# jaswon/osu-dreamer

Measured on AMD Instinct MI355X. Metric: denoiser train-steps/sec + 50-step sample latents/sec, 1/2/4/8 MI355X, higher is better.
Workload: dtype bf16

## Files before the change

### include/osu_dreamer_hip.h

```cpp
#ifndef OSU_DREAMER_HIP_H
#define OSU_DREAMER_HIP_H

#ifdef __cplusplus
extern "C" {
#endif

enum { OD_F32 = 0, OD_BF16 = 1,
       OD_F32X3 = 2,
       OD_F32X3W = 3,
       OD_F16 = 4 };
enum { OD_EPI_NONE = 0, OD_EPI_SILU = 1 };
enum { OD_ACT_NONE = 0, OD_ACT_SILU = 1 };
enum { OD_ERR_ARG = -1, OD_ERR_ALIGN = -2, OD_ERR_UNSUPPORTED = -3, OD_ERR_COMM = -4 };

int od_version(void);
const char* od_build_source_sha(void);
const char* od_error_string(int code);

int od_gemm_nt(int dtype, const void* A, int lda, const void* W, int ldw, const float* bias, void* C, int ldc,
               int M, int N, int K, int epilogue, int accumulate, void* stream);
int od_gemm_nt_qkrope(int dtype, const void* A, int lda, const void* W, int ldw, const float* bias, void* C, int ldc, int M,
                      int N, int K, const float* wq, const float* wk, const float* table, int L, int H, int hd, float eps,
                      float q_scale, void* stream);
int od_gemm_nt_qkrope_split(int dtype, const void* A, int lda, const void* W, int ldw, const float* bias, void* C, int ldc,
                            void* qk_out, int ldqk, int qk_dtype, int M, int N, int K, const float* wq, const float* wk, const float* table,
                            int L, int H, int hd, float eps, float q_scale, void* stream);
int od_gemm_tn(int dtype, const void* G, int ldg, const void* A, int lda, float* dW, int lddw, float* dbias, int M, int N,
               int K, void* stream);
int od_gemm_tn_blocks(int dtype, const void* G, int ldg, const void* A, int lda, float* dW, int lddw, float* dbias, int M, int N,
                      int K, int n_block, int n_valid, void* stream);
int od_colsum(int dtype, const void* G, int ldg, float* out, int M, int N, void* stream);
int od_pack_weight(int dtype, const float* src, int N, int K, void* dst, int Np, int Kp, int transpose,
                   const int* row_map, void* stream);

int od_linear_small(const float* x, const float* W, const float* b, float* out, float* pre, int B, int N, int K, int act,
                    void* stream);
int od_linear_small_bwd(const float* x, const float* W, const float* pre, const float* dout, float* dpre, float* dW,
                        float* db, float* dx, int accumulate_dx, int B, int N, int K, int act, void* stream);

int od_cl_to_frames(int dtype, const float* src, void* dst, int ldd, int B, int C, int L, void* stream);
int od_feed_gather(const float* store, long store_elems, const long* base, const long* cstride, const int* lens, float* out,
                   int N, int C, int Lpad, void* stream);
int od_feed_gather_quant(const void* store, long store_bytes, int elem_size, const long* base, const long* cstride, const int* lens,
                         const double* scale, const double* offset, const int* flip, float* out, int N, int C, int c0, int Ctot,
                         int Lpad, void* stream);
int od_replicate_tail(float* x, const int* lens, const int* plens, int N, int C, int Lpad, void* stream);
int od_proj_in(int dtype, const float* xt, const float* W, const float* bias, void* x, int ldx, int B, int E, int L,
               int D, void* stream);
int od_proj_in_bwd(int dtype, const float* xt, const void* dx, int ldx, float* dW, float* db, int B, int E, int L, int D,
                   void* stream);
int od_silu(int dtype, const void* x, void* y, long n, void* stream);
int od_silu_bwd(int dtype, const void* x, const void* dy, void* dx, long n, void* stream);

int od_rmsnorm_film(int dtype, const void* x, int ldx, const float* ssg, const void* cl, int ldcl, int cl_bcast,
                    void* h, int ldh, float* inv_rms, int B, int L, int C, float eps, void* stream);
int od_rmsnorm_film_bwd(int dtype, const void* x, int ldx, const float* inv_rms, const float* ssg, const void* dh,
                        int lddh, void* dres, int lddres, float* dssg, int B, int L, int C, void* stream);
int od_rmsnorm_gate_residual(int dtype, const void* x, int ldx, const void* h, int ldh, const float* ssg, void* xo,
                             int ldxo, float* inv_rms, int B, int L, int C, float eps, void* stream);
int od_rmsnorm_gate_residual_film(int dtype, const void* x, int ldx, const void* h, int ldh, const float* ssg_a, void* xo, int ldxo,
                                  float* inv_a, const float* ssg_b, const void* cl, int ldcl, int cl_bcast, void* h2, int ldh2,
                                  float* inv_b, int B, int L, int C, float eps, void* stream);
int od_rmsnorm_gate_residual_film_dwconv(int dtype, const void* x, int ldx, const void* h, int ldh, const float* ssg_a, void* xo, int ldxo,
                                         float* inv_a, const float* ssg_b, void* h2, int ldh2, float* inv_b, const float* conv_w,
                                         const float* conv_b, void* y, int ldy, int B, int L, int C, int ksize, float eps, void* stream);
int od_rmsnorm_gate_residual_bwd(int dtype, const void* h, int ldh, const float* inv_rms, const float* ssg,
                                 const void* dy, int lddy, void* dh, int lddh, float* dssg, int B, int L, int C,
                                 void* stream);

int od_rope_table(float* table, int L, int hd, void* stream);
int od_qk_norm_rope(int dtype, const void* qkv, int ldqkv, const float* wq, const float* wk, const float* table,
                    void* qk_out, int ldo, int B, int L, int H, int hd, float eps, float q_scale, void* stream);
int od_qk_norm_rope_bwd(int dtype, const void* qkv, int ldqkv, const float* wq, const float* wk, const float* table,
                        const void* dqk, int lddqk, void* dqkv, int lddqkv, float* dwq, float* dwk, int B, int L,
                        int H, int hd, float eps, float q_scale, void* stream);
int od_flash_attn_fwd(int dtype, const void* q, int ldq, const void* k, int ldk, const void* v, int ldv, void* o, int ldo,
                      float* lse, int B, int H, int L, int hd, float scale, int q_prescaled, void* stream);
int od_flash_attn_fwd_varlen(int dtype, const void* q, int ldq, const void* k, int ldk, const void* v, int ldv, void* o, int ldo,
                             float* lse, const int* lens, int B, int H, int L, int hd, float scale, int q_prescaled, void* stream);
int od_flash_attn_bwd(int dtype, const void* q, int ldq, const void* k, int ldk, const void* v, int ldv, const void* o,
                      int ldo, const void* dout, int lddo, const float* lse, float* delta, void* dq, int lddq, void* dk,
                      int lddk, void* dv, int lddv, int B, int H, int L, int hd, float scale, int q_prescaled, void* stream);
int od_attn_aux_create(void** aux_out);
int od_attn_aux_destroy(void* aux);
int od_flash_attn_bwd_aux(int dtype, const void* q, int ldq, const void* k, int ldk, const void* v, int ldv, const void* o,
                          int ldo, const void* dout, int lddo, const float* lse, float* delta, void* dq, int lddq, void* dk,
                          int lddk, void* dv, int lddv, int B, int H, int L, int hd, float scale, int q_prescaled, void* aux, void* stream);
int od_flash_attn_bwd_varlen(int dtype, const void* q, int ldq, const void* k, int ldk, const void* v, int ldv, const void* o,
                             int ldo, const void* dout, int lddo, const float* lse, float* delta, void* dq, int lddq, void* dk,
                             int lddk, void* dv, int lddv, const int* lens, int B, int H, int L, int hd, float scale, int q_prescaled,
                             void* aux, void* stream);
int od_flash_attn_bwd_fused_ws_bytes(int dtype, int B, int H, int L, long* total_out, long* zero_out);
int od_flash_attn_bwd_fused(int dtype, const void* q, int ldq, const void* k, int ldk, const void* v, int ldv, const void* o, int ldo,
                            const void* dout, int lddo, const float* lse, void* dq, int lddq, void* dk, int lddk, void* dv, int lddv,
                            int B, int H, int L, int hd, float scale, int q_prescaled, void* ws, long ws_bytes, void* stream);
int od_flash_attn_bwd_fused_status(const void* ws, int* err_out, void* stream);
int od_flash_attn_bwd_fused_err_offset(void);
int od_flash_attn_bwd_fused_passes(void);
int od_flash_attn_bwd_fused_prof(void* ws, long* out16);
int od_flash_attn_bwd_passes(void);

int od_dwconv(int dtype, const void* x, int ldx, const float* w, const float* bias, void* y, int ldy, int B, int L,
              int C, int ksize, void* stream);
int od_dwconv_varlen(int dtype, const void* x, int ldx, const float* w, const float* bias, void* y, int ldy, const int* lens,
                     int B, int L, int C, int ksize, void* stream);
int od_dwconv_bwd(int dtype, const void* x, int ldx, const float* w, const void* dy, int lddy, void* dx, int lddx,
                  float* dw, float* db, int B, int L, int C, int ksize, void* stream);
int od_dwconv_bwd_varlen(int dtype, const void* x, int ldx, const float* w, const void* dy, int lddy, void* dx, int lddx,
                         float* dw, float* db, const int* lens, int B, int L, int C, int ksize, void* stream);
int od_scale_channels(int dtype, void* x, int ldx, const float* scale, int B, int L, int C, void* stream);
int od_swiglu_rmsnorm(int dtype, const void* vg, int ldvg, void* hh, int ldhh, float* inv_rms, int M, int Hf, int Hp,
                      float eps, void* stream);
int od_swiglu_rmsnorm_bwd(int dtype, const void* vg, int ldvg, const float* inv_rms, const void* dhh, int lddhh,
                          void* dvg, int lddvg, int M, int Hf, int Hp, void* stream);

int od_final_norm_proj_out(int dtype, const void* x, int ldx, const float* W, const float* bias, float* v,
                           float* inv_rms, int B, int L, int C, int E, float eps, void* stream);
int od_final_norm_proj_out_bwd(int dtype, const void* x, int ldx, const float* inv_rms, const float* W, const float* dv,
                               void* dx, int lddx, float* dW, float* db, int B, int L, int C, int E, void* stream);
int od_uhead_fwd(const float* xt, const float* w0, const float* b0, const float* w1, const float* b1, const float* w3,
                 const float* b3, const float* w4, const float* b4, float* fsum, int B, int E, int L, int U,
                 void* stream);
int od_uhead_fwd_varlen(const float* xt, const float* w0, const float* b0, const float* w1, const float* b1, const float* w3,
                        const float* b3, const float* w4, const float* b4, float* fsum, const int* lens, int B, int E, int L,
                        int U, void* stream);
int od_uhead_bwd(const float* xt, const float* w0, const float* b0, const float* w1, const float* b1, const float* w3,
                 const float* b3, const float* w4, const float* b4, const float* dfm, float* dw0, float* db0, float* dw1,
                 float* db1, float* dw3, float* db3, float* dw4, float* db4, int B, int E, int L, int U, void* stream);
int od_uhead_bwd_varlen(const float* xt, const float* w0, const float* b0, const float* w1, const float* b1, const float* w3,
                        const float* b3, const float* w4, const float* b4, const float* dfm, float* dw0, float* db0, float* dw1,
                        float* db1, float* dw3, float* db3, float* dw4, float* db4, const int* lens, int B, int E, int L, int U,
                        void* stream);
int od_uhead_tail(const float* fsum, const float* mod, const float* w_out, const float* b_out, float* u, int B, int U,
                  int L, float u_scale, void* stream);
int od_uhead_tail_varlen(const float* fsum, const float* mod, const float* w_out, const float* b_out, float* u, const int* lens,
                         int B, int U, int L, float u_scale, void* stream);
int od_uhead_tail_bwd(const float* fsum, const float* mod, const float* w_out, const float* b_out, const float* du,
                      float* dfm, float* dmod, float* dw_out, float* db_out, int B, int U, int L, float u_scale,
                      void* stream);
int od_uhead_tail_bwd_varlen(const float* fsum, const float* mod, const float* w_out, const float* b_out, const float* du,
                             float* dfm, float* dmod, float* dw_out, float* db_out, const int* lens, int B, int U, int L,
                             float u_scale, void* stream);

int od_make_xt(const float* x0, const float* x1, const float* t, float* xt, float* dsq, int B, int E, int L, void* stream);
int od_make_xt_varlen(const float* x0, const float* x1, const float* t, float* xt, float* dsq, const int* lens, int B, int E, int L,
                      void* stream);
int od_loss_grad(const float* xt, const float* x1, const float* u, const float* v, const float* dsq, float* dv,
                 float* sums, int B, int E, int L, float c0, float osl_w, float del_w, void* stream);
int od_loss_grad_varlen(const float* xt, const float* x1, const float* u, const float* v, const float* dsq, float* dv,
                        float* sums, const int* lens, int B, int E, int L, float c0, float osl_w, float del_w, void* stream);
int od_loss_finalize(const float* sums, const float* dsq, const float* u, float* out, float* du, int B, float c0,
                     float osl_w, float del_w, void* stream);
int od_sampler_step(float* x, const float* u, const float* v, const float* eta, int B, int E, int L, void* stream);
int od_sampler_eta(const float* u, float* eta, int B, float c0, int num_steps, void* stream);
int od_sampler_eta_groups(const float* u, const int* offs, float* eta, int G, float c0, int num_steps, void* stream);
int od_sampler_step_varlen(float* x, const float* u, const float* v, const float* eta, const int* lens, const int* offs, int G,
                           int B, int E, int L, void* stream);

int od_det_clear(void);
int od_det_register(const float* base, long count, void* shadow_i64);
int od_det_enable(void* table_dev, void* stream);
int od_det_table_bytes(void);
int od_det_flush(float* dst, long count, void* stream);

int od_sqnorm(const float* g, long n, float* out, const int* status, void* stream);
int od_adamw_ema(float* p, const float* g, float* m, float* v, float* ema, long n, float lr, float beta1, float beta2,
                 float eps, float weight_decay, int step, float ema_decay, int ema_mode, const float* gnorm_sq,
                 float max_norm, const int* status, void* stream);

int od_ema_update(float* ema, const float* p, long n, float ema_decay, int ema_mode, void* stream);

int od_style_conditioning(const float* labels, const float* rff_w, const float* rff_b, const float* cond_w,
                          const float* cond_b, const float* null_labels, float* c, int B, int NL, int F, int H,
                          void* stream);
int od_rmsnorm_rows(const float* x, const float* gamma, float* y, int M, int C, float eps, void* stream);

int od_style_conditioning_bwd(const float* labels, const float* rff_w, const float* rff_b, const float* dc, float* dcond_w,
                              float* dcond_b, float* dnull_labels, int B, int NL, int F, int H, void* stream);
int od_rmsnorm_rows_bwd(const float* x, const float* gamma, const float* dy, float* dx, float* dgamma, int M, int C, float eps,
                        int accumulate_dx, void* stream);
int od_cast_rows(int src_dtype, const void* src, int dst_dtype, void* dst, long n, void* stream);

int od_spec_features_conv(int dtype, const float* audio, const float* w1, const float* b1, const float* g1, const float* w2,
                          const float* b2, const float* g2, void* out, int ldo, int B, int F, int L, float eps, void* stream);
int od_rmsnorm_affine_film(int dtype, const void* x, int ldx, const float* gamma, const float* ssg, void* y, int ldy, int B,
                           int L, int C, float eps, int act, void* stream);
int od_rmsnorm_affine_gate_residual(int dtype, const void* x, int ldx, const void* h, int ldh, const float* gamma,
                                    const float* ssg, void* xo, int ldxo, int B, int L, int C, float eps, void* stream);
int od_unet_mixer(int dtype, const void* x, int ldx, const void* p, int ldp, int p_bcast, const void* gx, int ldg,
                  const float* gamma, void* xo, int ldxo, int B, int L, int C, float eps, void* stream);
int od_unet_down(int dtype, const void* x, int ldx, const float* w, const float* bias, void* y, int ldy, int B, int Lo, int C,
                 int stride, void* stream);
int od_unet_up(int dtype, const void* x, int ldx, const float* w, const float* bias, void* y, int ldy, int B, int Li, int C,
               int stride, void* stream);
int od_chart_head(int dtype, const void* x, int ldx, const float* W, const float* bias, float* out, int B, int L, int C, int N,
                  int n_sigmoid, int rms, float eps, void* stream);
int od_attn_pool(int dtype, const void* scores, int lds, const void* values, int ldv, float* out, int B, int L, int Hh, int hd,
                 void* stream);
int od_latent_bwd_block_frames(int C);
int od_rmsnorm_affine_film_bwd(int dtype, const void* x, int ldx, const float* gamma, const float* ssg, const void* dy, int lddy, void* dx,
                               int lddx, int accumulate_dx, float* dgamma, float* dssg, float* ws, long ws_floats, int B, int L, int C,
                               float eps, int act, void* stream);
int od_rmsnorm_affine_gate_residual_bwd(int dtype, const void* h, int ldh, const float* gamma, const float* ssg, const void* dxo, int lddxo,
                                        void* dh, int lddh, float* dgamma, float* dssg, float* ws, long ws_floats, int B, int L, int C,
                                        float eps, void* stream);
int od_unet_mixer_bwd(int dtype, const void* p, int ldp, int p_bcast, const void* gx, int ldg, const float* gamma, const void* dxo,
                      int lddxo, void* dp, int lddp, void* dgx, int lddg, float* dgamma, float* ws, long ws_floats, int B, int L, int C,
                      float eps, void* stream);
int od_unet_down_bwd(int dtype, const void* x, int ldx, const float* w, const void* dy, int lddy, void* dx, int lddx, float* dw, float* db,
                     float* ws, long ws_floats, int B, int Lo, int C, int stride, void* stream);
int od_unet_up_bwd(int dtype, const void* x, int ldx, const float* w, const void* dy, int lddy, void* dx, int lddx, float* dw, float* db,
                   float* ws, long ws_floats, int B, int Li, int C, int stride, void* stream);
int od_chart_head_bwd(int dtype, const void* x, int ldx, const float* W, const float* bias, const float* dout, void* dx, int lddx,
                      float* dW, float* db, float* ws, long ws_floats, int B, int L, int C, int N, int rms, float eps, void* stream);
int od_attn_pool_bwd(int dtype, const void* scores, int lds, const void* values, int ldv, const float* dout, void* dscores, int ldds,
                     void* dvalues, int lddv, int B, int L, int Hh, int hd, void* stream);
int od_spec_features_conv_bwd(int dtype, const float* audio, const float* w1, const float* b1, const float* g1, const float* w2,
                              const float* b2, const float* g2, const void* dout, int ldo, float* dw1, float* db1, float* dg1, float* dw2,
                              float* db2, float* dg2, float* ws, long ws_floats, int B, int F, int L, float eps, void* stream);
int od_add_rows(int dtype, const void* x, void* y, long n, void* stream);
int od_proj_in_bwd_input(int dtype, const void* dx, int ldx, const float* W, float* dxt, int B, int E, int L, int D, void* stream);

int od_mmd_imq(const float* z, const float* prior, float* out, float* dz, float* ws, long ws_floats, int N, int D, void* stream);
int od_scale_by(const float* x, const float* g, float* y, long n, void* stream);
int od_latent_perturb(const float* z, long zsb, long zse, long zsl, const float* s, const float* eps_z, const float* eps_s,
                      const float* u_s, const float* repl, const float* u_span, const float* u_start, float* z_out, float* s_out,
                      void* masked, void* start_span, int B2, int E, int l, int S, float s_noise, float z_noise, float s_mask_frac,
                      float z_mask_frac, int training, void* stream);
int od_latent_perturb_bwd(const float* dz_out, const float* ds_out, const void* masked, const int* start_span, float* dz, float* ds,
                          int B2, int E, int l, int S, void* stream);
int od_latent_loss_block_frames(void);
int od_latent_loss_ws_floats(int B2, int L);
int od_latent_loss(const float* logits, const float* chart, const float* pred_labels, const float* true_labels, const void* masked,
                   const float* s_reg, float* loss_ema, void* ema_init, float* out, float* coef, float* ws, long ws_floats, int B2, int L,
                   float s_reg_weight, int training, void* stream);
int od_latent_loss_bwd(const float* logits, const float* chart, const float* pred_labels, const float* true_labels, const void* masked,
                       const float* coef, const float* g, float* dlogits, float* dlabels, float* ds_reg, int B2, int L,
                       float s_reg_weight, void* stream);

int od_mmd_imq_pairs(const float* s, const float* prior, float* out, float* ws, long ws_floats, int G, int S, void* stream);
int od_latent_loss_maps(const float* logits, const float* chart, const int* hlens, const float* pred_labels, const float* true_labels,
                        const float* s_reg, int s_reg_stride, const float* loss_ema, float* out, float* ws, long ws_floats, int G,
                        int Hmax, float s_reg_weight, void* stream);
int od_latent_eval_maps_ws_floats(int G, int Pmax);
int od_latent_eval_maps(const float* chart, const float* pred_chart, const int* plens, const float* z, const int* zlens,
                        const float* pred_labels, const float* true_labels, float* out, float* ws, long ws_floats, int G, int Pmax, int E,
                        int lmax, void* stream);

int od_spec_features_conv_varlen(int dtype, const float* audio, const float* w1, const float* b1, const float* g1, const float* w2,
                                 const float* b2, const float* g2, void* out, int ldo, const int* lens, int B, int F, int L, float eps,
                                 void* stream);
int od_rmsnorm_affine_film_varlen(int dtype, const void* x, int ldx, const float* gamma, const float* ssg, void* y, int ldy,
                                  const int* lens, int B, int L, int C, float eps, int act, void* stream);
int od_unet_mixer_varlen(int dtype, const void* x, int ldx, const void* p, int ldp, const int* prow, const void* gx, int ldg,
                         const float* gamma, void* xo, int ldxo, int B, int L, int C, float eps, void* stream);
int od_unet_down_varlen(int dtype, const void* x, int ldx, const float* w, const float* bias, void* y, int ldy, const int* lens,
                        int B, int Lo, int C, int stride, void* stream);
int od_unet_up_varlen(int dtype, const void* x, int ldx, const float* w, const float* bias, void* y, int ldy, const int* lens,
                      int B, int Li, int C, int stride, void* stream);
int od_chart_head_varlen(int dtype, const void* x, int ldx, const float* W, const float* bias, float* out, const int* lens, int B,
                         int L, int C, int N, int n_sigmoid, int rms, float eps, void* stream);
int od_attn_pool_varlen(int dtype, const void* scores, int lds, const void* values, int ldv, float* out, const int* lens, int B,
                        int L, int Hh, int hd, void* stream);

int od_comm_load(const char* path);
int od_comm_version(void);
int od_comm_unique_id(void* out, int nbytes);
int od_comm_init(void** comm_out, int nranks, int rank, const void* unique_id, int nbytes);
int od_comm_destroy(void* comm);
int od_comm_abort(void* comm);
int od_comm_count(void* comm);
int od_comm_ring_standin(float* buf, long count, int channels, int threads, int rounds, void* stream);
int od_allreduce_grads(void* comm, float* grads, long count, int average, void* stream);
int od_broadcast_f32(void* comm, float* buf, long count, int root, void* stream);

int od_graph_begin(void* stream);
int od_graph_end(void* stream, void** graph_exec_out);
int od_graph_launch(void* graph_exec, void* stream);
int od_graph_destroy(void* graph_exec);

int od_mfma_calibrate(float* scratch, int iters, double* flops_out, void* stream);

#ifdef __cplusplus
}
#endif
#endif
```

### osu_dreamer_amd/csrc/heads.hip

```cpp
#include "od_common.h"
#include "od_api_internal.h"

namespace {

constexpr int UW = 32;
constexpr int UOWN = 30;
constexpr int UWPB = 4;
constexpr int MAXU = 64, MAXE = 8;

__device__ __forceinline__ float red32(float v) {
#pragma unroll
    for (int m = 16; m >= 1; m >>= 1) v += __shfl_xor(v, m);
    return v;
}

struct UHeadW {
    const float *w0, *b0, *w1, *b1, *w3, *b3, *w4, *b4;
};

struct UHeadSmem {
    float xts[MAXE][UW + 4];
    float z0s[MAXE][UW + 2];
    float z1s[MAXU][UW + 2];
    float a1s[MAXU][UW + 2];
    float z3s[MAXU][UW + 1];
    float g4s[MAXU][UW + 1];
    float w4s[MAXU][MAXU + 1];
};

__device__ __forceinline__ void uhead_window_fwd(UHeadSmem& S, const float* __restrict__ xt, const UHeadW& P, int b, int l0,
                                                 int E, int L, int U, int Lv) {
    const int t = threadIdx.x;
    for (int idx = t; idx < E * (UW + 4); idx += 256) {
        const int e = idx / (UW + 4), ix = idx % (UW + 4);
        const int f = l0 - 3 + ix;
        S.xts[e][ix] = (f >= 0 && f < Lv) ? xt[((size_t)b * E + e) * L + f] : 0.f;
    }
    __syncthreads();
    for (int idx = t; idx < E * (UW + 2); idx += 256) {
        const int e = idx / (UW + 2), i2 = idx % (UW + 2);
        S.z0s[e][i2] = P.b0[e] + P.w0[e * 3 + 0] * S.xts[e][i2] + P.w0[e * 3 + 1] * S.xts[e][i2 + 1] + P.w0[e * 3 + 2] * S.xts[e][i2 + 2];
    }
    __syncthreads();
    for (int idx = t; idx < U * (UW + 2); idx += 256) {
        const int c = idx / (UW + 2), i2 = idx % (UW + 2);
        const int f = l0 - 2 + i2;
        float z = P.b1[c];
        for (int e = 0; e < E; e++) z += P.w1[c * E + e] * S.z0s[e][i2];
        S.z1s[c][i2] = z;
        S.a1s[c][i2] = (f >= 0 && f < Lv) ? od_silu(z) : 0.f;
    }
    __syncthreads();
    for (int idx = t; idx < U * UW; idx += 256) {
        const int c = idx / UW, i = idx % UW;
        S.z3s[c][i] = P.b3[c] + P.w3[c * 3 + 0] * S.a1s[c][i] + P.w3[c * 3 + 1] * S.a1s[c][i + 1] + P.w3[c * 3 + 2] * S.a1s[c][i + 2];
    }
    __syncthreads();
}

__device__ __forceinline__ void uhead_load_w4(UHeadSmem& S, const UHeadW& P, int U) {
    for (int idx = threadIdx.x; idx < U * U; idx += 256) S.w4s[idx / U][idx % U] = P.w4[idx];
    __syncthreads();
}

template <bool VL = false>
__global__ __launch_bounds__(256) void uhead_fwd_kernel(const float* __restrict__ xt, UHeadW P, float* __restrict__ fsum,
                                                        int E, int L, int U, int nwin, int wpb, const OdDetTable* __restrict__ det,
                                                        const int* __restrict__ lens = nullptr) {
    __shared__ UHeadSmem S;
    const int b = blockIdx.y, t = threadIdx.x;
    const int Lb = VL ? od_uniform(lens[b]) : L;
    const int i = t & 31, grp = t >> 5, cpg = U / 8;
    uhead_load_w4(S, P, U);
    float acc[MAXU / 8];
#pragma unroll
    for (int q = 0; q < MAXU / 8; q++) acc[q] = 0.f;
    for (int wi = 0; wi < wpb; wi++) {
        const int win = blockIdx.x * wpb + wi;
        if (win >= nwin) break;
        const int l0 = win * UOWN;
        if (VL && l0 >= Lb) break;
        uhead_window_fwd(S, xt, P, b, l0, E, L, U, Lb);
        const int f = l0 - 1 + i;
        const bool own = (i >= 1 && i < UW - 1 && f < Lb);
#pragma unroll
        for (int q = 0; q < MAXU / 8; q++) {
            if (q < cpg) {
                const int c = grp * cpg + q;
                float z = P.b4[c];
                for (int cc = 0; cc < U; cc++) z += S.w4s[c][cc] * S.z3s[cc][i];
                if (own) acc[q] += od_silu(z);
            }
        }
        __syncthreads();
    }
#pragma unroll
    for (int q = 0; q < MAXU / 8; q++) {
        const float s = red32(acc[q]);
        if (q < cpg && i == 0) od_red_add(det, fsum + (size_t)b * U + grp * cpg + q, s);
    }
}

struct UHeadG {
    float *dw0, *db0, *dw1, *db1, *dw3, *db3, *dw4, *db4;
};

template <bool VL>
__device__ __forceinline__ void uhead_bwd_body(const float* __restrict__ xt, const UHeadW& P, const float* __restrict__ dfm,
                                               const UHeadG& G, int E, int L, int U, int nwin, const OdDetTable* __restrict__ det,
                                               const int* __restrict__ lens) {
    __shared__ UHeadSmem S;
    __shared__ float sdw3[MAXU][3], sdb3[MAXU], sdb4[MAXU], sdw1[MAXU][MAXE], sdb1[MAXU], sdw0[MAXE][3], sdb0[MAXE];
    const int b = blockIdx.y, t = threadIdx.x;
    const int i = t & 31, grp = t >> 5, cpg = U / 8;
    const int Lb = VL ? od_uniform(lens[b]) : L;
    for (int idx = t; idx < MAXU; idx += 256) {
        sdb3[idx] = 0.f; sdb4[idx] = 0.f; sdb1[idx] = 0.f;
        for (int j = 0; j < 3; j++) sdw3[idx][j] = 0.f;
        for (int e = 0; e < MAXE; e++) sdw1[idx][e] = 0.f;
    }
    if (t < MAXE) { sdb0[t] = 0.f; for (int j = 0; j < 3; j++) sdw0[t][j] = 0.f; }
    uhead_load_w4(S, P, U);
    float adw4[16];
#pragma unroll
    for (int q = 0; q < 16; q++) adw4[q] = 0.f;
    const float invL = 1.0f / (float)Lb;

    for (int wi = 0; wi < UWPB; wi++) {
        const int win = blockIdx.x * UWPB + wi;
        if (win >= nwin) break;
        const int l0 = win * UOWN;
        if (VL && l0 >= Lb) break;
        uhead_window_fwd(S, xt, P, b, l0, E, L, U, Lb);
        const int f = l0 - 1 + i;
        const bool inr = (f >= 0 && f < Lb);
        const bool own = (i >= 1 && i < UW - 1 && f < Lb);
#pragma unroll
        for (int q = 0; q < MAXU / 8; q++) {
            if (q < cpg) {
                const int c = grp * cpg + q;
                float z = P.b4[c];
                for (int cc = 0; cc < U; cc++) z += S.w4s[c][cc] * S.z3s[cc][i];
                const float g = inr ? dfm[(size_t)b * U + c] * invL * od_silu_grad(z) : 0.f;
                S.g4s[c][i] = g;
                const float s = red32(own ? g : 0.f);
                if (i == 0) atomicAdd(&sdb4[c], s);
            }
        }
        __syncthreads();
        {
            const int iend = (Lb - (l0 - 1)) < (UW - 1) ? (Lb - (l0 - 1)) : (UW - 1);
#pragma unroll
            for (int q = 0; q < 16; q++) {
                const int o = t + 256 * q;
                if (o < U * U) {
                    const int c = o / U, cc = o % U;
                    float s = 0.f;
                    for (int ii = 1; ii < iend; ii++) s += S.g4s[c][ii] * S.z3s[cc][ii];
                    adw4[q] += s;
                }
            }
        }
        __syncthreads();
        float dz3v[MAXU / 8];
#pragma unroll
        for (int q = 0; q < MAXU / 8; q++) {
            dz3v[q] = 0.f;
            if (q < cpg) {
                const int cc = grp * cpg + q;
                float s = 0.f;
                for (int c = 0; c < U; c++) s += S.w4s[c][cc] * S.g4s[c][i];
                dz3v[q] = s;
            }
        }
        __syncthreads();
#pragma unroll
        for (int q = 0; q < MAXU / 8; q++)
            if (q < cpg) S.z3s[grp * cpg + q][i] = dz3v[q];
        __syncthreads();
#pragma unroll
        for (int q = 0; q < MAXU / 8; q++) {
            if (q < cpg) {
                const int c = grp * cpg + q;
                const float g = own ? S.z3s[c][i] : 0.f;
                float s = red32(g);
                if (i == 0) atomicAdd(&sdb3[c], s);
                for (int j = 0; j < 3; j++) {
                    s = red32(g * S.a1s[c][i + j]);
                    if (i == 0) atomicAdd(&sdw3[c][j], s);
                }
                float dz1 = 0.f;
                if (own) {
                    float da1 = 0.f;
                    for (int j = 0; j < 3; j++) da1 += P.w3[c * 3 + j] * S.z3s[c][i - j + 1];
                    dz1 = da1 * od_silu_grad(S.z1s[c][i + 1]);
                }
                S.g4s[c][i] = dz1;
                s = red32(dz1);
                if (i == 0) atomicAdd(&sdb1[c], s);
                for (int e = 0; e < E; e++) {
                    s = red32(dz1 * S.z0s[e][i + 1]);
                    if (i == 0) atomicAdd(&sdw1[c][e], s);
                }
            }
        }
        __syncthreads();
        {
            const bool ev = grp < E;
            const int e = ev ? grp : 0;
            float dz0 = 0.f;
            if (ev)
                for (int c = 0; c < U; c++) dz0 += P.w1[c * E + e] * S.g4s[c][i];
            float s = red32(dz0);
            if (ev && i == 0) atomicAdd(&sdb0[e], s);
            for (int j = 0; j < 3; j++) {
                s = red32(dz0 * S.xts[e][i + 1 + j]);
                if (ev && i == 0) atomicAdd(&sdw0[e][j], s);
            }
        }
        __syncthreads();
    }
#pragma unroll
    for (int q = 0; q < 16; q++) {
        const int o = t + 256 * q;
        if (o < U * U) od_red_add(det, G.dw4 + o, adw4[q]);
    }
    __syncthreads();
    for (int c = t; c < U; c += 256) {
        od_red_add(det, G.db4 + c, sdb4[c]);
        od_red_add(det, G.db3 + c, sdb3[c]);
        od_red_add(det, G.db1 + c, sdb1[c]);
        for (int j = 0; j < 3; j++) od_red_add(det, G.dw3 + c * 3 + j, sdw3[c][j]);
        for (int e = 0; e < E; e++) od_red_add(det, G.dw1 + c * E + e, sdw1[c][e]);
    }
    if (t < E) {
        od_red_add(det, G.db0 + t, sdb0[t]);
        for (int j = 0; j < 3; j++) od_red_add(det, G.dw0 + t * 3 + j, sdw0[t][j]);
    }
}

__global__ __launch_bounds__(256) void uhead_bwd_kernel(const float* __restrict__ xt, UHeadW P, const float* __restrict__ dfm,
                                                        UHeadG G, int E, int L, int U, int nwin, const OdDetTable* __restrict__ det) {
    uhead_bwd_body<false>(xt, P, dfm, G, E, L, U, nwin, det, nullptr);
}
__global__ __launch_bounds__(256) void uhead_bwd_varlen_kernel(const float* __restrict__ xt, UHeadW P, const float* __restrict__ dfm,
                                                               UHeadG G, int E, int L, int U, int nwin, const OdDetTable* __restrict__ det,
                                                               const int* __restrict__ lens) {
    uhead_bwd_body<true>(xt, P, dfm, G, E, L, U, nwin, det, lens);
}

template <bool VL = false>
__global__ void uhead_tail_kernel(const float* __restrict__ fsum, const float* __restrict__ mod, const float* __restrict__ w,
                                  const float* __restrict__ bo, float* __restrict__ u, int B, int U, int L, float u_scale,
                                  const int* __restrict__ lens = nullptr) {
    const int b = blockIdx.x, lane = threadIdx.x;
    const float Lf = (float)(VL ? od_uniform(lens[b]) : L);
    float s = 0.f;
    for (int c = lane; c < U; c += 64) {
        const float f = fsum[(size_t)b * U + c] / Lf;
        s += w[c] * (f * (1.f + mod[(size_t)b * 2 * U + c]) + mod[(size_t)b * 2 * U + U + c]);
    }
    s = od_wave_sum(s);
    if (lane == 0) {
        const float y = s + bo[0];
        const float sp = y > 20.f ? y : log1pf(__expf(y));
        u[b] = u_scale * sp;
    }
}
template <bool VL = false>
__global__ void uhead_tail_bwd_kernel(const float* __restrict__ fsum, const float* __restrict__ mod, const float* __restrict__ w,
                                      const float* __restrict__ bo, const float* __restrict__ du, float* __restrict__ dfm,
                                      float* __restrict__ dmod, float* __restrict__ dw, float* __restrict__ dbo,
                                      int B, int U, int L, float u_scale, const OdDetTable* __restrict__ det,
                                      const int* __restrict__ lens = nullptr) {
    const int b = blockIdx.x, lane = threadIdx.x;
    const float Lf = (float)(VL ? od_uniform(lens[b]) : L);
    float s = 0.f;
    for (int c = lane; c < U; c += 64) {
        const float f = fsum[(size_t)b * U + c] / Lf;
        s += w[c] * (f * (1.f + mod[(size_t)b * 2 * U + c]) + mod[(size_t)b * 2 * U + U + c]);
    }
    s = od_wave_sum(s);
    const float y = s + bo[0];
    const float dy = du[b] * u_scale * od_sigmoid(y);
    for (int c = lane; c < U; c += 64) {
        const float f = fsum[(size_t)b * U + c] / Lf;
        const float sc = mod[(size_t)b * 2 * U + c], sh = mod[(size_t)b * 2 * U + U + c];
        const float fm = f * (1.f + sc) + sh;
        od_red_add(det, dw + c, dy * fm);
        const float dfmv = dy * w[c];
        dfm[(size_t)b * U + c] = dfmv * (1.f + sc);
        dmod[(size_t)b * 2 * U + c] = dfmv * f;
        dmod[(size_t)b * 2 * U + U + c] = dfmv;
    }
    if (lane == 0) od_red_add(det, dbo, dy);
}

__device__ __forceinline__ float block_sum_256(float v, float* sh) {
    v = od_wave_sum(v);
    __syncthreads();
    if ((threadIdx.x & 63) == 0) sh[threadIdx.x >> 6] = v;
    __syncthreads();
    return sh[0] + sh[1] + sh[2] + sh[3];
}

template <bool VL = false>
__global__ __launch_bounds__(256) void make_xt_kernel(const float* __restrict__ x0, const float* __restrict__ x1,
                                                      const float* __restrict__ t, float* __restrict__ xt,
                                                      float* __restrict__ dsq, int EL, int L, const OdDetTable* __restrict__ det,
                                                      const int* __restrict__ lens = nullptr) {
    __shared__ float sh[4];
    const int b = blockIdx.y;
    const int Lb = VL ? od_uniform(lens[b]) : L;
    const float w = t[b];
    float acc = 0.f;
    for (int i = blockIdx.x * 256 + threadIdx.x; i < EL; i += gridDim.x * 256) {
        const size_t o = (size_t)b * EL + i;
        if (VL && (i % L) >= Lb) { xt[o] = 0.f; continue; }
        const float a = x0[o], e = x1[o];
        const float v = w < 0.5f ? a + w * (e - a) : e - (e - a) * (1.f - w);
        xt[o] = v;
        const float d = v - e;
        acc += d * d;
    }
    acc = block_sum_256(acc, sh);
    if (threadIdx.x == 0) od_red_add(det, dsq + b, acc / (float)Lb);
}

template <bool VL = false>
__global__ __launch_bounds__(256) void loss_grad_kernel(const float* __restrict__ xt, const float* __restrict__ x1,
                                                        const float* __restrict__ u, const float* __restrict__ v,
                                                        const float* __restrict__ dsq, float* __restrict__ dv,
                                                        float* __restrict__ sums, int B, int EL, int L, float c0,
                                                        float osl_w, float del_w, const OdDetTable* __restrict__ det,
                                                        const int* __restrict__ lens = nullptr) {
    __shared__ float sh[4];
    const int b = blockIdx.y;
    const int Lb = VL ? od_uniform(lens[b]) : L;
    const float ub = u[b], den = dsq[b] + c0, ut = sqrtf(den);
    const float k1 = osl_w / ((float)B * den), k2 = del_w / (float)B, invL2 = 2.f / (float)Lb;
    float s1 = 0.f, s2 = 0.f, s3 = 0.f;
    for (int i = blockIdx.x * 256 + threadIdx.x; i < EL; i += gridDim.x * 256) {
        const size_t o = (size_t)b * EL + i;
        if (VL && (i % L) >= Lb) { dv[o] = 0.f; continue; }
        const float xv = xt[o], e = x1[o], vv = v[o];
        const float r1 = xv - ub * vv - e;
        const float r2 = vv - (xv - e) / ut;
        s1 += r1 * r1; s2 += r2 * r2; s3 += r1 * (-vv);
        dv[o] = k1 * invL2 * r1 * (-ub) + k2 * invL2 * r2;
    }
    s1 = block_sum_256(s1, sh); s2 = block_sum_256(s2, sh); s3 = block_sum_256(s3, sh);
    if (threadIdx.x == 0) {
        od_red_add(det, sums + b * 3 + 0, s1 / (float)Lb);
        od_red_add(det, sums + b * 3 + 1, s2 / (float)Lb);
        od_red_add(det, sums + b * 3 + 2, s3 * invL2);
    }
}

__global__ void loss_finalize_kernel(const float* __restrict__ sums, const float* __restrict__ dsq, const float* __restrict__ u,
                                     float* __restrict__ out, float* __restrict__ du, int B, float c0, float osl_w, float del_w) {
    const int lane = threadIdx.x;
    float osl = 0.f, del = 0.f, mape = 0.f;
    for (int b = lane; b < B; b += 64) {
        const float den = dsq[b] + c0, ut = sqrtf(den);
        osl += sums[b * 3 + 0] / den;
        del += sums[b * 3 + 1];
        mape += fabsf((u[b] - ut) / ut);
        du[b] = osl_w / ((float)B * den) * sums[b * 3 + 2];
    }
    osl = od_wave_sum(osl) / (float)B; del = od_wave_sum(del) / (float)B; mape = od_wave_sum(mape) / (float)B;
    if (lane == 0) { out[0] = osl_w * osl + del_w * del; out[1] = osl; out[2] = del; out[3] = mape; }
}

__global__ __launch_bounds__(256) void sampler_step_kernel(float* __restrict__ x, const float* __restrict__ u,
                                                           const float* __restrict__ v, const float* __restrict__ eta, int EL) {
    const int b = blockIdx.y;
    const float k = eta[0] * u[b];
    for (int i = blockIdx.x * 256 + threadIdx.x; i < EL; i += gridDim.x * 256) {
        const size_t o = (size_t)b * EL + i;
        x[o] = x[o] - k * v[o];
    }
}

__global__ void sampler_eta_kernel(const float* __restrict__ u, float* __restrict__ eta, int B, float c0, int num_steps) {
    const int lane = threadIdx.x;
    float s = 0.f;
    for (int b = lane; b < B; b += 64) s += u[b];
    s = od_wave_sum(s) / (float)B;
    if (lane == 0) {
        const float r = sqrtf(c0);
        const float u0 = s > r + 1e-6f ? s : r + 1e-6f;
        eta[0] = 1.f - powf(r / u0, 1.f / (float)num_steps);
        eta[1] = s;
    }
}

__global__ void sampler_eta_groups_kernel(const float* __restrict__ u, const int* __restrict__ offs, float* __restrict__ eta, float c0,
                                          int num_steps) {
    const int g = blockIdx.x, lane = threadIdx.x;
    const int r0 = od_uniform(offs[g]), n = od_uniform(offs[g + 1]) - r0;
    float s = 0.f;
    for (int b = lane; b < n; b += 64) s += u[r0 + b];
    s = od_wave_sum(s) / (float)n;
    if (lane == 0) {
        const float r = sqrtf(c0);
        const float u0 = s > r + 1e-6f ? s : r + 1e-6f;
        eta[2 * g] = 1.f - powf(r / u0, 1.f / (float)num_steps);
        eta[2 * g + 1] = s;
    }
}

__global__ __launch_bounds__(256) void sampler_step_varlen_kernel(float* __restrict__ x, const float* __restrict__ u, const float* __restrict__ v,
                                                                  const float* __restrict__ eta, const int* __restrict__ lens,
                                                                  const int* __restrict__ offs, int G, int EL, int L) {
    const int b = blockIdx.y;
    int g = 0;
    while (g + 1 < G && od_uniform(offs[g + 1]) <= b) g++;
    const int Lb = od_uniform(lens[b]);
    const float k = eta[2 * g] * u[b];
    for (int i = blockIdx.x * 256 + threadIdx.x; i < EL; i += gridDim.x * 256) {
        const size_t o = (size_t)b * EL + i;
        x[o] = (i % L) < Lb ? x[o] - k * v[o] : 0.f;
    }
}

}

extern "C" int od_uhead_fwd(const float* xt, const float* w0, const float* b0, const float* w1, const float* b1, const float* w3,
                            const float* b3, const float* w4, const float* b4, float* fsum, int B, int E, int L, int U,
                            void* stream) {
    if (U > MAXU || U % 8 || E > MAXE) return OD_ERR_UNSUPPORTED;
    const int nwin = (L + UOWN - 1) / UOWN;
    UHeadW P{w0, b0, w1, b1, w3, b3, w4, b4};
    int wpb = (int)((long)nwin * B / 512);
    wpb = wpb < 1 ? 1 : (wpb > UWPB ? UWPB : wpb);
    OD_LAUNCH(uhead_fwd_kernel<>, dim3((nwin + wpb - 1) / wpb, B), dim3(256), 0, (hipStream_t)stream, xt, P, fsum, E, L, U, nwin, wpb, od_det_active());
    OD_CHECK_LAUNCH();
    return 0;
}

extern "C" int od_uhead_fwd_varlen(const float* xt, const float* w0, const float* b0, const float* w1, const float* b1, const float* w3,
                                   const float* b3, const float* w4, const float* b4, float* fsum, const int* lens, int B, int E, int L,
                                   int U, void* stream) {
    if (U > MAXU || U % 8 || E > MAXE) return OD_ERR_UNSUPPORTED;
    if (!lens) return OD_ERR_ARG;
    const int nwin = (L + UOWN - 1) / UOWN;
    UHeadW P{w0, b0, w1, b1, w3, b3, w4, b4};
    int wpb = (int)((long)nwin * B / 512);
    wpb = wpb < 1 ? 1 : (wpb > UWPB ? UWPB : wpb);
    OD_LAUNCH(uhead_fwd_kernel<true>, dim3((nwin + wpb - 1) / wpb, B), dim3(256), 0, (hipStream_t)stream, xt, P, fsum, E, L, U, nwin, wpb,
              od_det_active(), lens);
    OD_CHECK_LAUNCH();
    return 0;
}

extern "C" int od_uhead_bwd(const float* xt, const float* w0, const float* b0, const float* w1, const float* b1, const float* w3,
                            const float* b3, const float* w4, const float* b4, const float* dfm, float* dw0, float* db0,
                            float* dw1, float* db1, float* dw3, float* db3, float* dw4, float* db4, int B, int E, int L, int U,
                            void* stream) {
    if (U > MAXU || U % 8 || E > MAXE) return OD_ERR_UNSUPPORTED;
    const int nwin = (L + UOWN - 1) / UOWN;
    UHeadW P{w0, b0, w1, b1, w3, b3, w4, b4};
    UHeadG G{dw0, db0, dw1, db1, dw3, db3, dw4, db4};
    OD_LAUNCH(uhead_bwd_kernel, dim3((nwin + UWPB - 1) / UWPB, B), dim3(256), 0, (hipStream_t)stream, xt, P, dfm, G, E, L, U, nwin, od_det_active());
    OD_CHECK_LAUNCH();
    return 0;
}

extern "C" int od_uhead_bwd_varlen(const float* xt, const float* w0, const float* b0, const float* w1, const float* b1, const float* w3,
                                   const float* b3, const float* w4, const float* b4, const float* dfm, float* dw0, float* db0,
                                   float* dw1, float* db1, float* dw3, float* db3, float* dw4, float* db4, const int* lens, int B, int E,
                                   int L, int U, void* stream) {
    if (U > MAXU || U % 8 || E > MAXE) return OD_ERR_UNSUPPORTED;
    if (!lens) return OD_ERR_ARG;
    const int nwin = (L + UOWN - 1) / UOWN;
    UHeadW P{w0, b0, w1, b1, w3, b3, w4, b4};
    UHeadG G{dw0, db0, dw1, db1, dw3, db3, dw4, db4};
    OD_LAUNCH(uhead_bwd_varlen_kernel, dim3((nwin + UWPB - 1) / UWPB, B), dim3(256), 0, (hipStream_t)stream, xt, P, dfm, G, E, L, U, nwin,
              od_det_active(), lens);
    OD_CHECK_LAUNCH();
    return 0;
}

extern "C" int od_uhead_tail(const float* fsum, const float* mod, const float* w_out, const float* b_out, float* u, int B, int U,
                             int L, float u_scale, void* stream) {
    OD_LAUNCH(uhead_tail_kernel<>, dim3(B), dim3(64), 0, (hipStream_t)stream, fsum, mod, w_out, b_out, u, B, U, L, u_scale);
    OD_CHECK_LAUNCH();
    return 0;
}

extern "C" int od_uhead_tail_varlen(const float* fsum, const float* mod, const float* w_out, const float* b_out, float* u, const int* lens,
                                    int B, int U, int L, float u_scale, void* stream) {
    if (!lens) return OD_ERR_ARG;
    OD_LAUNCH(uhead_tail_kernel<true>, dim3(B), dim3(64), 0, (hipStream_t)stream, fsum, mod, w_out, b_out, u, B, U, L, u_scale, lens);
    OD_CHECK_LAUNCH();
    return 0;
}

extern "C" int od_uhead_tail_bwd(const float* fsum, const float* mod, const float* w_out, const float* b_out, const float* du,
                                 float* dfm, float* dmod, float* dw_out, float* db_out, int B, int U, int L, float u_scale,
                                 void* stream) {
    OD_LAUNCH(uhead_tail_bwd_kernel<>, dim3(B), dim3(64), 0, (hipStream_t)stream, fsum, mod, w_out, b_out, du, dfm, dmod, dw_out,
              db_out, B, U, L, u_scale, od_det_active());
    OD_CHECK_LAUNCH();
    return 0;
}

extern "C" int od_uhead_tail_bwd_varlen(const float* fsum, const float* mod, const float* w_out, const float* b_out, const float* du,
                                        float* dfm, float* dmod, float* dw_out, float* db_out, const int* lens, int B, int U, int L,
                                        float u_scale, void* stream) {
    if (!lens) return OD_ERR_ARG;
    OD_LAUNCH(uhead_tail_bwd_kernel<true>, dim3(B), dim3(64), 0, (hipStream_t)stream, fsum, mod, w_out, b_out, du, dfm, dmod, dw_out,
              db_out, B, U, L, u_scale, od_det_active(), lens);
    OD_CHECK_LAUNCH();
    return 0;
}

extern "C" int od_make_xt(const float* x0, const float* x1, const float* t, float* xt, float* dsq, int B, int E, int L, void* stream) {
    const int EL = E * L;
    int gx = (EL + 255) / 256; if (gx > 256) gx = 256;
    OD_LAUNCH(make_xt_kernel<>, dim3(gx, B), dim3(256), 0, (hipStream_t)stream, x0, x1, t, xt, dsq, EL, L, od_det_active());
    OD_CHECK_LAUNCH();
    return 0;
}

static inline int loss_grid_x(int EL) { const int g = (EL + 255) / 256; return g > 256 ? 256 : g; }

extern "C" int od_make_xt_varlen(const float* x0, const float* x1, const float* t, float* xt, float* dsq, const int* lens, int B, int E,
                                 int L, void* stream) {
    if (!lens) return OD_ERR_ARG;
    const int EL = E * L, gx = loss_grid_x(EL);
    OD_LAUNCH(make_xt_kernel<true>, dim3(gx, B), dim3(256), 0, (hipStream_t)stream, x0, x1, t, xt, dsq, EL, L, od_det_active(), lens);
    OD_CHECK_LAUNCH();
    return 0;
}

extern "C" int od_loss_grad(const float* xt, const float* x1, const float* u, const float* v, const float* dsq, float* dv,
                            float* sums, int B, int E, int L, float c0, float osl_w, float del_w, void* stream) {
    const int EL = E * L;
    int gx = (EL + 255) / 256; if (gx > 256) gx = 256;
    OD_LAUNCH(loss_grad_kernel<>, dim3(gx, B), dim3(256), 0, (hipStream_t)stream, xt, x1, u, v, dsq, dv, sums, B, EL, L, c0, osl_w, del_w, od_det_active());
    OD_CHECK_LAUNCH();
    return 0;
}

extern "C" int od_loss_grad_varlen(const float* xt, const float* x1, const float* u, const float* v, const float* dsq, float* dv,
                                   float* sums, const int* lens, int B, int E, int L, float c0, float osl_w, float del_w, void* stream) {
    if (!lens) return OD_ERR_ARG;
    const int EL = E * L, gx = loss_grid_x(EL);
    OD_LAUNCH(loss_grad_kernel<true>, dim3(gx, B), dim3(256), 0, (hipStream_t)stream, xt, x1, u, v, dsq, dv, sums, B, EL, L, c0, osl_w, del_w,
              od_det_active(), lens);
    OD_CHECK_LAUNCH();
    return 0;
}

extern "C" int od_loss_finalize(const float* sums, const float* dsq, const float* u, float* out, float* du, int B, float c0,
                                float osl_w, float del_w, void* stream) {
    OD_LAUNCH(loss_finalize_kernel, dim3(1), dim3(64), 0, (hipStream_t)stream, sums, dsq, u, out, du, B, c0, osl_w, del_w);
    OD_CHECK_LAUNCH();
    return 0;
}

extern "C" int od_sampler_step(float* x, const float* u, const float* v, const float* eta, int B, int E, int L, void* stream) {
    const int EL = E * L;
    int gx = (EL + 255) / 256; if (gx > 256) gx = 256;
    OD_LAUNCH(sampler_step_kernel, dim3(gx, B), dim3(256), 0, (hipStream_t)stream, x, u, v, eta, EL);
    OD_CHECK_LAUNCH();
    return 0;
}

extern "C" int od_sampler_eta(const float* u, float* eta, int B, float c0, int num_steps, void* stream) {
    OD_LAUNCH(sampler_eta_kernel, dim3(1), dim3(64), 0, (hipStream_t)stream, u, eta, B, c0, num_steps);
    OD_CHECK_LAUNCH();
    return 0;
}

extern "C" int od_sampler_eta_groups(const float* u, const int* offs, float* eta, int G, float c0, int num_steps, void* stream) {
    if (!offs || G < 1) return OD_ERR_ARG;
    OD_LAUNCH(sampler_eta_groups_kernel, dim3(G), dim3(64), 0, (hipStream_t)stream, u, offs, eta, c0, num_steps);
    OD_CHECK_LAUNCH();
    return 0;
}

extern "C" int od_sampler_step_varlen(float* x, const float* u, const float* v, const float* eta, const int* lens, const int* offs, int G,
                                      int B, int E, int L, void* stream) {
    if (!lens || !offs || G < 1) return OD_ERR_ARG;
    const int EL = E * L;
    int gx = (EL + 255) / 256; if (gx > 256) gx = 256;
    OD_LAUNCH(sampler_step_varlen_kernel, dim3(gx, B), dim3(256), 0, (hipStream_t)stream, x, u, v, eta, lens, offs, G, EL, L);
    OD_CHECK_LAUNCH();
    return 0;
}
```

### osu_dreamer_amd/csrc/misc.hip

```cpp
#include "od_common.h"
#include "od_api_internal.h"
#include <type_traits>

namespace {

template <class T>
__global__ __launch_bounds__(256) void cl_to_frames_kernel(const float* __restrict__ src, T* __restrict__ dst, int ldd, int C, int L) {
    __shared__ float tile[64][65];
    const int b = blockIdx.z, l0 = blockIdx.x * 64, c0 = blockIdx.y * 64;
    const int tx = threadIdx.x & 63, ty = threadIdx.x >> 6;
    for (int i = ty; i < 64; i += 4) {
        const int c = c0 + i, l = l0 + tx;
        tile[i][tx] = (c < C && l < L) ? src[((size_t)b * C + c) * L + l] : 0.f;
    }
    __syncthreads();
    for (int i = ty; i < 64; i += 4) {
        const int l = l0 + i, c = c0 + tx;
        if (l < L && c < C) od_t<T>::st(dst + ((size_t)b * L + l) * ldd + c, tile[tx][i]);
    }
}

constexpr int FG_SEG = 1024;
__device__ __forceinline__ bool feed_row(long store_elems, const long* __restrict__ base, const long* __restrict__ cstride,
                                         const int* __restrict__ lens, int C, int Lpad, int nseg, long items, int& n, int& c, int& l0, int& l1,
                                         long& s0, int& len, float& fill) {
    const long w = (long)blockIdx.x * 4 + od_uniform((int)(threadIdx.x >> 6));
    if (w >= items) return false;
    const long row = w / nseg;
    const int seg = (int)(w - row * nseg);
    n = (int)(row / C);
    c = (int)(row - (long)n * C);
    const long b0 = base[n], cs = cstride[n];
    len = lens[n];
    const bool sane = len >= 1 && len <= Lpad && b0 >= 0 && cs >= 0 && b0 <= store_elems && cs <= store_elems;
    s0 = sane ? b0 + (long)c * cs : 0;
    const bool ok = sane && s0 >= 0 && s0 <= store_elems - len;
    fill = ok ? 0.f : __builtin_nanf("");
    if (!ok) len = 0;
    l0 = seg * FG_SEG;
    l1 = l0 + FG_SEG < Lpad ? l0 + FG_SEG : Lpad;
    return true;
}

__global__ __launch_bounds__(256) void feed_gather_kernel(const float* __restrict__ store, long store_elems, const long* __restrict__ base,
                                                          const long* __restrict__ cstride, const int* __restrict__ lens,
                                                          float* __restrict__ out, int C, int Lpad, int nseg, long items) {
    const int lane = threadIdx.x & 63;
    int n, c, l0, l1, len;
    long s0;
    float fill;
    if (!feed_row(store_elems, base, cstride, lens, C, Lpad, nseg, items, n, c, l0, l1, s0, len, fill)) return;
    const float* src = store + s0;
    float* dst = out + ((long)n * C + c) * Lpad;
    if ((Lpad & 3) == 0 && ((((size_t)src) | ((size_t)dst)) & 15) == 0) {
        for (int l = l0 + lane * 4; l < l1; l += 256) {
            f32x4 v;
            if (l + 4 <= len) v = *(const f32x4*)(src + l);
            else {
#pragma unroll
                for (int e = 0; e < 4; e++) v[e] = l + e < len ? src[l + e] : fill;
            }
            *(f32x4*)(dst + l) = v;
        }
    } else {
        for (int l = l0 + lane; l < l1; l += 256) {
            float v[4];
#pragma unroll
            for (int e = 0; e < 4; e++) v[e] = l + 64 * e < len ? src[l + 64 * e] : fill;
#pragma unroll
            for (int e = 0; e < 4; e++)
                if (l + 64 * e < l1) dst[l + 64 * e] = v[e];
        }
    }
}

__device__ __forceinline__ float fq_value(unsigned q, double qmax, bool affine, double sc, double of, bool flip) {
#pragma clang fp contract(off)
    double v = (double)q / qmax;
    if (affine) {
        v = v * sc;
        v = v + of;
    }
    const float f = (float)v;
    return flip ? 1.0f - f : f;
}

template <int ES>
__global__ __launch_bounds__(256) void feed_gather_quant_kernel(const unsigned char* __restrict__ store, long store_bytes, const long* __restrict__ base,
                                                                const long* __restrict__ cstride, const int* __restrict__ lens,
                                                                const double* __restrict__ scale, const double* __restrict__ offset,
                                                                const int* __restrict__ flipmask, float* __restrict__ out, int C, int c0, int Ctot,
                                                                int Lpad, int nseg, long items) {
    typedef typename std::conditional<ES == 1, unsigned char, unsigned short>::type Q;
    const int lane = threadIdx.x & 63;
    int n, c, l0, l1, len;
    long s0;
    float fill;
    if (!feed_row(store_bytes / ES, base, cstride, lens, C, Lpad, nseg, items, n, c, l0, l1, s0, len, fill)) return;
    const double qmax = ES == 1 ? 255.0 : 65535.0;
    const bool affine = scale != nullptr;
    const double sc = affine ? scale[(long)n * C + c] : 1.0, of = affine ? offset[(long)n * C + c] : 0.0;
    const bool flip = flipmask != nullptr && ((flipmask[n] >> c) & 1);
    const Q* src = (const Q*)store + s0;
    float* dst = out + ((long)n * Ctot + c0 + c) * Lpad;
    if ((Lpad & 3) == 0 && (((size_t)dst) & 15) == 0 && (((size_t)store) & 3) == 0) {
        const unsigned* s32 = (const unsigned*)store;
        const long sbyte = s0 * ES;
        const int sh = 8 * (int)(sbyte & 3);
        const long last = (store_bytes >> 2) - (sh ? ES + 1 : ES);
        for (int l = l0 + lane * 4; l < l1; l += 256) {
            unsigned q[4];
            const long a = (sbyte + (long)l * ES) >> 2;
            if (l + 4 <= len && a <= last) {
                unsigned d[ES + 1];
#pragma unroll
                for (int i = 0; i < ES; i++) d[i] = s32[a + i];
                d[ES] = sh ? s32[a + ES] : 0u;
#pragma unroll
                for (int i = 0; i < ES; i++) d[i] = (unsigned)((((unsigned long)d[i + 1] << 32) | d[i]) >> sh);
#pragma unroll
                for (int e = 0; e < 4; e++) q[e] = ES == 1 ? (d[0] >> (8 * e)) & 255u : (d[e >> 1] >> (16 * (e & 1))) & 65535u;
            } else {
#pragma unroll
                for (int e = 0; e < 4; e++) q[e] = l + e < len ? (unsigned)src[l + e] : 0u;
            }
            f32x4 v;
#pragma unroll
            for (int e = 0; e < 4; e++) v[e] = l + e < len ? fq_value(q[e], qmax, affine, sc, of, flip) : fill;
            *(f32x4*)(dst + l) = v;
        }
    } else {
        for (int l = l0 + lane; l < l1; l += 256) {
            unsigned q[4];
#pragma unroll
            for (int e = 0; e < 4; e++) q[e] = l + 64 * e < len ? (unsigned)src[l + 64 * e] : 0u;
#pragma unroll
            for (int e = 0; e < 4; e++)
                if (l + 64 * e < l1) dst[l + 64 * e] = l + 64 * e < len ? fq_value(q[e], qmax, affine, sc, of, flip) : fill;
        }
    }
}

__global__ __launch_bounds__(256) void replicate_tail_kernel(float* __restrict__ x, const int* __restrict__ lens, const int* __restrict__ plens,
                                                             int C, int Lpad, long rows) {
    const int lane = threadIdx.x & 63;
    const long row = (long)blockIdx.x * 4 + od_uniform((int)(threadIdx.x >> 6));
    if (row >= rows) return;
    const int n = (int)(row / C);
    const int len = lens[n], plen = plens[n];
    float* dst = x + row * Lpad;
    if (len < 1 || plen > Lpad) {
        for (int l = lane; l < Lpad; l += 64) dst[l] = __builtin_nanf("");
        return;
    }
    if (plen <= len) return;
    const float v = dst[len - 1];
    for (int l = len + lane; l < plen; l += 64) dst[l] = v;
}

template <class T>
__global__ __launch_bounds__(256) void proj_in_kernel(const float* __restrict__ xt, const float* __restrict__ W,
                                                      const float* __restrict__ bias, T* __restrict__ x, int ldx,
                                                      int B, int E, int L, int D) {
    const int lane = threadIdx.x & 63;
    const long M = (long)B * L;
    const long nw = (long)gridDim.x * 4, w0 = (long)blockIdx.x * 4 + (threadIdx.x >> 6);
    for (int c = lane * 8; c < D; c += 512) {
        float wv[8][8], bv[8];
        od_ld8(bias + c, bv);
        if (E == 6) {
            float flat[48];
#pragma unroll
            for (int q = 0; q < 6; q++) od_ld8(W + (size_t)c * 6 + q * 8, *(float(*)[8])&flat[q * 8]);
#pragma unroll
            for (int k = 0; k < 8; k++)
#pragma unroll
                for (int e = 0; e < 8; e++) wv[k][e] = e < 6 ? flat[k * 6 + e] : 0.f;
        } else {
#pragma unroll
            for (int k = 0; k < 8; k++)
#pragma unroll
                for (int e = 0; e < 8; e++) wv[k][e] = e < E ? W[(size_t)(c + k) * E + e] : 0.f;
        }
        for (long m = w0; m < M; m += nw) {
            const int b = (int)(m / L), l = (int)(m % L);
            float xe[8];
#pragma unroll
            for (int e = 0; e < 8; e++) xe[e] = e < E ? xt[((size_t)b * E + e) * L + l] : 0.f;
            float o[8];
#pragma unroll
            for (int k = 0; k < 8; k++) {
                float s = bv[k];
#pragma unroll
                for (int e = 0; e < 8; e++) s += wv[k][e] * xe[e];
                o[k] = s;
            }
            od_st8(x + m * ldx + c, o);
        }
    }
}

template <class T>
__global__ __launch_bounds__(256) void proj_in_bwd_kernel(const float* __restrict__ xt, const T* __restrict__ dx, int ldx,
                                                          float* __restrict__ dW, float* __restrict__ db, int B, int E, int L, int D,
                                                          const OdDetTable* __restrict__ det) {
    __shared__ float red[64][73];
    const int lane = threadIdx.x & 63, wave = threadIdx.x >> 6;
    const int M = B * L;
    const int nw = gridDim.x * 4, w0 = blockIdx.x * 4 + wave;
    for (int c0 = 0; c0 < D; c0 += 512) {
        const int c = c0 + lane * 8;
        float aw[8][8], ab[8];
#pragma unroll
        for (int k = 0; k < 8; k++) {
            ab[k] = 0.f;
#pragma unroll
            for (int e = 0; e < 8; e++) aw[k][e] = 0.f;
        }
        if (c < D)
            for (int m = w0; m < M; m += nw) {
                const int b = m / L, l = m - b * L;
                float xe[8], g[8];
#pragma unroll
                for (int e = 0; e < 8; e++) xe[e] = e < E ? xt[((size_t)b * E + e) * L + l] : 0.f;
                od_ld8(dx + (size_t)m * ldx + c, g);
#pragma unroll
                for (int k = 0; k < 8; k++) {
                    ab[k] += g[k];
#pragma unroll
                    for (int e = 0; e < 8; e++) aw[k][e] += g[k] * xe[e];
                }
            }
        for (int w = 0; w < 4; w++) {
            if (wave == w) {
#pragma unroll
                for (int k = 0; k < 8; k++) {
                    red[lane][k * 9 + 8] = (w ? red[lane][k * 9 + 8] : 0.f) + ab[k];
#pragma unroll
                    for (int e = 0; e < 8; e++) red[lane][k * 9 + e] = (w ? red[lane][k * 9 + e] : 0.f) + aw[k][e];
                }
            }
            __syncthreads();
        }
        if (wave == 0 && c < D) {
#pragma unroll
            for (int k = 0; k < 8; k++) {
                od_red_add(det, db + c + k, red[lane][k * 9 + 8]);
#pragma unroll
                for (int e = 0; e < 8; e++)
                    if (e < E) od_red_add(det, dW + (size_t)(c + k) * E + e, red[lane][k * 9 + e]);
            }
        }
        __syncthreads();
    }
}

template <class T>
__global__ __launch_bounds__(256) void silu_kernel(const T* __restrict__ x, T* __restrict__ y, long n8) {
    for (long i = (long)blockIdx.x * 256 + threadIdx.x; i < n8; i += (long)gridDim.x * 256) {
        float v[8]; od_ld8(x + i * 8, v);
#pragma unroll
        for (int e = 0; e < 8; e++) v[e] = od_silu(v[e]);
        od_st8(y + i * 8, v);
    }
}
template <class T>
__global__ __launch_bounds__(256) void silu_bwd_kernel(const T* __restrict__ x, const T* __restrict__ dy, T* __restrict__ dx, long n8) {
    for (long i = (long)blockIdx.x * 256 + threadIdx.x; i < n8; i += (long)gridDim.x * 256) {
        float v[8], g[8]; od_ld8(x + i * 8, v); od_ld8(dy + i * 8, g);
#pragma unroll
        for (int e = 0; e < 8; e++) g[e] *= od_silu_grad(v[e]);
        od_st8(dx + i * 8, g);
    }
}

template <class T, int KS, int DW_RUN, bool VL = false>
__global__ __launch_bounds__(256) void dwconv_kernel(const T* __restrict__ x, int ldx, const float* __restrict__ w,
                                                     const float* __restrict__ bias, T* __restrict__ y, int ldy,
                                                     int L, int C, const int* __restrict__ lens = nullptr) {
    constexpr int R = KS / 2;
    const int cg = C / 8;
    const int b = blockIdx.y;
    const int Lb = VL ? od_uniform(lens[b]) : L;
    const long t = (long)blockIdx.x * 256 + threadIdx.x;
    const int cgi = (int)(t % cg);
    const long run = t / cg;
    const int l0 = (int)(run * DW_RUN);
    if (l0 >= L) return;
    const int c = cgi * 8;
    float wv[8][KS], bv[8];
#pragma unroll
    for (int k = 0; k < 8; k++) {
        bv[k] = bias[c + k];
#pragma unroll
        for (int j = 0; j < KS; j++) wv[k][j] = w[(size_t)(c + k) * KS + j];
    }
    float win[KS][8];
    const T* xb = x + (size_t)b * L * ldx + c;
#pragma unroll
    for (int j = 0; j < KS - 1; j++) {
        const int l = l0 - R + j;
        if (l >= 0 && l < Lb) od_ld8(xb + (size_t)l * ldx, win[j]);
        else {
#pragma unroll
            for (int k = 0; k < 8; k++) win[j][k] = 0.f;
        }
    }
    for (int i = 0; i < DW_RUN; i++) {
        const int l = l0 + i;
        if (l >= L) break;
        const int ln = l + R;
        if (ln < Lb) od_ld8(xb + (size_t)ln * ldx, win[KS - 1]);
        else {
#pragma unroll
            for (int k = 0; k < 8; k++) win[KS - 1][k] = 0.f;
        }
        float o[8];
#pragma unroll
        for (int k = 0; k < 8; k++) {
            float s = bv[k];
#pragma unroll
            for (int j = 0; j < KS; j++) s += wv[k][j] * win[j][k];
            o[k] = (VL && l >= Lb) ? 0.f : s;
        }
        od_st8(y + ((size_t)b * L + l) * ldy + c, o);
#pragma unroll
        for (int j = 0; j < KS - 1; j++)
#pragma unroll
            for (int k = 0; k < 8; k++) win[j][k] = win[j + 1][k];
    }
}

constexpr int DW_RUN_BWD = 64;
template <class T, int KS, bool VL = false>
__global__ __launch_bounds__(256) void dwconv_bwd_kernel(const T* __restrict__ x, int ldx, const float* __restrict__ w,
                                                         const T* __restrict__ dy, int lddy, T* __restrict__ dx, int lddx,
                                                         float* __restrict__ dw, float* __restrict__ db, int L, int C,
                                                         const OdDetTable* __restrict__ det, const int* __restrict__ lens = nullptr) {
    constexpr int R = KS / 2;
    __shared__ long long red[(KS <= 5 ? 1024 : 512) * (KS + 1)];
    __shared__ int s_bad;
    const int cg = C / 8;
    const int b = blockIdx.y;
    const int Lb = VL ? od_uniform(lens[b]) : L;
    const long t = (long)blockIdx.x * 256 + threadIdx.x;
    const int cgi = (int)(t % cg);
    const long run = t / cg;
    const int l0 = (int)(run * DW_RUN_BWD);
    const bool active = l0 < L;
    const int c = cgi * 8;
    for (int i = threadIdx.x; i < C * (KS + 1); i += 256) red[i] = 0;
    if (threadIdx.x == 0) s_bad = 0;
    __syncthreads();
    float wv[8][KS], adw[8][KS], adb[8];
#pragma unroll
    for (int k = 0; k < 8; k++) {
        adb[k] = 0.f;
#pragma unroll
        for (int j = 0; j < KS; j++) { wv[k][j] = w[(size_t)(c + k) * KS + j]; adw[k][j] = 0.f; }
    }
    if (active) {
        float wy[KS][8], wx[KS][8];
        const T* xb = x + (size_t)b * L * ldx + c;
        const T* yb = dy + (size_t)b * L * lddy + c;
#pragma unroll
        for (int j = 0; j < KS - 1; j++) {
            const int l = l0 - R + j;
            if (l >= 0 && l < Lb) { od_ld8(xb + (size_t)l * ldx, wx[j]); od_ld8(yb + (size_t)l * lddy, wy[j]); }
            else {
#pragma unroll
                for (int k = 0; k < 8; k++) { wx[j][k] = 0.f; wy[j][k] = 0.f; }
            }
        }
        constexpr int DW_PF = 2;
        typedef typename std::conditional<sizeof(T) == 2, u32x4, f32x4>::type row_t;
        row_t px[DW_PF][sizeof(T) == 2 ? 1 : 2], py[DW_PF][sizeof(T) == 2 ? 1 : 2];
        auto fetch = [&](int ln, int slot) {
            if (ln < Lb) {
#pragma unroll
                for (int h2 = 0; h2 < (sizeof(T) == 2 ? 1 : 2); h2++) {
                    px[slot][h2] = *(const row_t*)(xb + (size_t)ln * ldx + h2 * 4);
                    py[slot][h2] = *(const row_t*)(yb + (size_t)ln * lddy + h2 * 4);
                }
            } else {
#pragma unroll
                for (int h2 = 0; h2 < (sizeof(T) == 2 ? 1 : 2); h2++) { px[slot][h2] = (row_t)(0); py[slot][h2] = (row_t)(0); }
            }
        };
        auto unpack = [&](const row_t (&r)[sizeof(T) == 2 ? 1 : 2], float (&o8)[8]) {
            if constexpr (sizeof(T) == 2) {
#pragma unroll
                for (int i2 = 0; i2 < 4; i2++) {
                    union { uint32_t u; float f; } lo, hi;
                    lo.u = r[0][i2] << 16; hi.u = r[0][i2] & 0xffff0000u;
                    o8[2 * i2] = lo.f; o8[2 * i2 + 1] = hi.f;
                }
            } else {
#pragma unroll
                for (int i2 = 0; i2 < 4; i2++) { o8[i2] = r[0][i2]; o8[4 + i2] = r[1][i2]; }
            }
        };
#pragma unroll
        for (int pf = 0; pf < DW_PF; pf++) fetch(l0 + R + pf, pf);
        for (int i0 = 0; i0 < DW_RUN_BWD; i0 += DW_PF) {
          if (l0 + i0 >= L) break;
#pragma unroll
          for (int pf = 0; pf < DW_PF; pf++) {
            const int i = i0 + pf;
            const int l = l0 + i;
            if (l >= L) break;
            unpack(px[pf], wx[KS - 1]);
            unpack(py[pf], wy[KS - 1]);
            fetch(l + R + DW_PF, pf);
            float o[8];
#pragma unroll
            for (int k = 0; k < 8; k++) {
                float sacc = 0.f;
#pragma unroll
                for (int jj = 0; jj < KS; jj++) sacc += wv[k][jj] * wy[KS - 1 - jj][k];
                o[k] = (VL && l >= Lb) ? 0.f : sacc;
                const float gy = wy[R][k];
                adb[k] += gy;
#pragma unroll
                for (int jj = 0; jj < KS; jj++) adw[k][jj] += gy * wx[jj][k];
            }
            od_st8(dx + ((size_t)b * L + l) * lddx + c, o);
#pragma unroll
            for (int j = 0; j < KS - 1; j++)
#pragma unroll
                for (int k = 0; k < 8; k++) { wx[j][k] = wx[j + 1][k]; wy[j][k] = wy[j + 1][k]; }
          }
        }
#pragma unroll
        for (int k = 0; k < 8; k++) {
            od_lds_fix_add(&red[(c + k) * (KS + 1) + KS], adb[k], &s_bad);
#pragma unroll
            for (int j = 0; j < KS; j++) od_lds_fix_add(&red[(c + k) * (KS + 1) + j], adw[k][j], &s_bad);
        }
    }
    __syncthreads();
    for (int i = threadIdx.x; i < C * (KS + 1); i += 256) {
        const int ch = i / (KS + 1), j = i % (KS + 1);
        const float v = od_lds_unfix(red[i], s_bad);
        if (v != 0.f) {
            if (j == KS) od_red_add(det, db + ch, v); else od_red_add(det, dw + (size_t)ch * KS + j, v);
        }
    }
}

constexpr int LS_KC = 256, LS_NB = 8;
__global__ __launch_bounds__(256) void linear_small_kernel(const float* __restrict__ x, const float* __restrict__ W,
                                                           const float* __restrict__ bias, float* __restrict__ out,
                                                           float* __restrict__ pre, int B, int N, int K, int act) {
    __shared__ __attribute__((aligned(16))) float xs[32][LS_KC + 4];
    __shared__ __attribute__((aligned(16))) float ws[LS_NB][LS_KC + 4];
    const int b0 = blockIdx.y * 32, n0 = blockIdx.x * LS_NB;
    const int bl = threadIdx.x & 31, nl = threadIdx.x >> 5;
    float acc = 0.f;
    for (int k0 = 0; k0 < K; k0 += LS_KC) {
        const int kc = K - k0 < LS_KC ? K - k0 : LS_KC;
        for (int i = threadIdx.x; i < 32 * LS_KC; i += 256) {
            const int r = i / LS_KC, c = i % LS_KC;
            xs[r][c] = (b0 + r < B && c < kc) ? x[(size_t)(b0 + r) * K + k0 + c] : 0.f;
        }
        for (int i = threadIdx.x; i < LS_NB * LS_KC; i += 256) {
            const int r = i / LS_KC, c = i % LS_KC;
            ws[r][c] = (n0 + r < N && c < kc) ? W[(size_t)(n0 + r) * K + k0 + c] : 0.f;
        }
        __syncthreads();
#pragma unroll 8
        for (int c = 0; c < LS_KC; c += 4) {
            const f32x4 a = *(const f32x4*)&xs[bl][c], w = *(const f32x4*)&ws[nl][c];
            acc += a[0] * w[0]; acc += a[1] * w[1]; acc += a[2] * w[2]; acc += a[3] * w[3];
        }
        __syncthreads();
    }
    const int b = b0 + bl, n = n0 + nl;
    if (b < B && n < N) {
        const float s = acc + (bias ? bias[n] : 0.f);
        if (pre) pre[(size_t)b * N + n] = s;
        out[(size_t)b * N + n] = act == OD_ACT_SILU ? od_silu(s) : s;
    }
}
__global__ __launch_bounds__(256) void linear_small_dpre_kernel(const float* __restrict__ pre, const float* __restrict__ dout,
                                                                float* __restrict__ dpre, long n, int act) {
    const long i = (long)blockIdx.x * 256 + threadIdx.x;
    if (i >= n) return;
    dpre[i] = act == OD_ACT_SILU ? dout[i] * od_silu_grad(pre[i]) : dout[i];
}
__global__ __launch_bounds__(256) void linear_small_dw_kernel(const float* __restrict__ x, const float* __restrict__ dpre,
                                                              float* __restrict__ dW, float* __restrict__ db, int B, int N, int K) {
    const int n = blockIdx.y, k = blockIdx.x * 256 + threadIdx.x;
    if (dW && k < K) {
        float s0 = 0.f, s1 = 0.f, s2 = 0.f, s3 = 0.f;
        int b = 0;
        for (; b + 3 < B; b += 4) {
            s0 += dpre[(size_t)b * N + n] * x[(size_t)b * K + k];
            s1 += dpre[(size_t)(b + 1) * N + n] * x[(size_t)(b + 1) * K + k];
            s2 += dpre[(size_t)(b + 2) * N + n] * x[(size_t)(b + 2) * K + k];
            s3 += dpre[(size_t)(b + 3) * N + n] * x[(size_t)(b + 3) * K + k];
        }
        for (; b < B; b++) s0 += dpre[(size_t)b * N + n] * x[(size_t)b * K + k];
        dW[(size_t)n * K + k] += (s0 + s1) + (s2 + s3);
    }
    if (db && blockIdx.x == 0 && threadIdx.x == 0) {
        float s = 0.f;
        for (int b = 0; b < B; b++) s += dpre[(size_t)b * N + n];
        db[n] += s;
    }
}
constexpr int LS_NR = 32;
__global__ __launch_bounds__(256) void linear_small_dx_kernel(const float* __restrict__ W, const float* __restrict__ dpre,
                                                              float* __restrict__ dx, int B, int N, int K, const OdDetTable* __restrict__ det) {
    __shared__ __attribute__((aligned(16))) float ds[LS_NR][32];
    const int n0 = blockIdx.x * LS_NR, b0 = blockIdx.y * 32, k = blockIdx.z * 256 + threadIdx.x;
    for (int i = threadIdx.x; i < LS_NR * 32; i += 256) {
        const int bl = i / LS_NR, nl = i % LS_NR;
        ds[nl][bl] = (b0 + bl < B && n0 + nl < N) ? dpre[(size_t)(b0 + bl) * N + n0 + nl] : 0.f;
    }
    __syncthreads();
    if (k >= K) return;
    float acc[32];
#pragma unroll
    for (int i = 0; i < 32; i++) acc[i] = 0.f;
    const int nr = N - n0 < LS_NR ? N - n0 : LS_NR;
    for (int nl = 0; nl < nr; nl++) {
        const float w = W[(size_t)(n0 + nl) * K + k];
#pragma unroll
        for (int q4 = 0; q4 < 8; q4++) {
            const f32x4 d = *(const f32x4*)&ds[nl][4 * q4];
            acc[4 * q4] += d[0] * w; acc[4 * q4 + 1] += d[1] * w; acc[4 * q4 + 2] += d[2] * w; acc[4 * q4 + 3] += d[3] * w;
        }
    }
#pragma unroll
    for (int i = 0; i < 32; i++)
        if (b0 + i < B) od_red_add(det, dx + (size_t)(b0 + i) * K + k, acc[i]);
}

__global__ __launch_bounds__(256) void zero_f32_kernel(float* __restrict__ p, long n) {
    const long i = (long)blockIdx.x * 256 + threadIdx.x;
    if (i < n) p[i] = 0.f;
}

template <class T>
__global__ __launch_bounds__(256) void pack_weight_kernel(const float* __restrict__ src, int N, int K, T* __restrict__ dst,
                                                          int Np, int Kp, int transpose, const int* __restrict__ row_map) {
    const long i = (long)blockIdx.x * 256 + threadIdx.x;
    if (i >= (long)Np * Kp) return;
    int n, k;
    if (!transpose) { n = (int)(i / Kp); k = (int)(i % Kp); }
    else { k = (int)(i / Np); n = (int)(i % Np); }
    const int sn = row_map ? row_map[n] : (n < N ? n : -1);
    const float v = (sn >= 0 && k < K) ? src[(size_t)sn * K + k] : 0.f;
    od_t<T>::st(dst + i, v);
}

__global__ __launch_bounds__(256) void pack_weight_split_kernel(const float* __restrict__ src, int N, int K, bf16_t* __restrict__ dst,
                                                                int Np, int Kp, const int* __restrict__ row_map) {
    const long i = (long)blockIdx.x * 256 + threadIdx.x;
    if (i >= (long)Np * Kp) return;
    const int n = (int)(i / Kp), k = (int)(i % Kp);
    const int sn = row_map ? row_map[n] : (n < N ? n : -1);
    const float v = (sn >= 0 && k < K) ? src[(size_t)sn * K + k] : 0.f;
    const bf16_t hi = od_f2bf(v);
    const bf16_t lo = od_f2bf(v - od_bf2f(hi));
    bf16_t* slab = dst + ((size_t)n * Kp + (k & ~31)) * 2;
    slab[k & 31] = hi;
    slab[32 + (k & 31)] = lo;
}

}

#define DISPATCH_T(DT, CALL)                                       \
    do {                                                           \
        if ((DT) == OD_BF16) { typedef bf16_t T_; CALL; }          \
        else if ((DT) == OD_F32) { typedef float T_; CALL; }       \
        else return OD_ERR_ARG;                                    \
    } while (0)

extern "C" int od_cl_to_frames(int dtype, const float* src, void* dst, int ldd, int B, int C, int L, void* stream) {
    dim3 grid((L + 63) / 64, (C + 63) / 64, B);
    DISPATCH_T(dtype, OD_LAUNCH((cl_to_frames_kernel<T_>), grid, dim3(256), 0, (hipStream_t)stream, src, (T_*)dst, ldd, C, L));
    OD_CHECK_LAUNCH();
    return 0;
}

extern "C" int od_feed_gather(const float* store, long store_elems, const long* base, const long* cstride, const int* lens, float* out,
                              int N, int C, int Lpad, void* stream) {
    if (!store || !base || !cstride || !lens || !out || Lpad < 1 || N < 1 || C < 1 || store_elems < 1) return OD_ERR_ARG;
    const int nseg = (Lpad + FG_SEG - 1) / FG_SEG;
    const long items = (long)N * C * nseg, blocks = (items + 3) / 4;
    if (blocks > 0x7fffffffL) return OD_ERR_UNSUPPORTED;
    OD_LAUNCH(feed_gather_kernel, dim3((unsigned)blocks), dim3(256), 0, (hipStream_t)stream, store, store_elems, base, cstride, lens, out, C, Lpad, nseg, items);
    OD_CHECK_LAUNCH();
    return 0;
}

extern "C" int od_feed_gather_quant(const void* store, long store_bytes, int elem_size, const long* base, const long* cstride, const int* lens,
                                    const double* scale, const double* offset, const int* flip, float* out, int N, int C, int c0, int Ctot,
                                    int Lpad, void* stream) {
    if (!store || !base || !cstride || !lens || !out || Lpad < 1 || N < 1 || C < 1 || store_bytes < 1) return OD_ERR_ARG;
    if ((elem_size != 1 && elem_size != 2) || (scale == nullptr) != (offset == nullptr)) return OD_ERR_ARG;
    if (c0 < 0 || C > Ctot - c0 || (flip && C > 32)) return OD_ERR_ARG;
    const int nseg = (Lpad + FG_SEG - 1) / FG_SEG;
    const long items = (long)N * C * nseg, blocks = (items + 3) / 4;
    if (blocks > 0x7fffffffL) return OD_ERR_UNSUPPORTED;
    if (elem_size == 1)
        OD_LAUNCH(feed_gather_quant_kernel<1>, dim3((unsigned)blocks), dim3(256), 0, (hipStream_t)stream, (const unsigned char*)store, store_bytes, base,
                  cstride, lens, scale, offset, flip, out, C, c0, Ctot, Lpad, nseg, items);
    else
        OD_LAUNCH(feed_gather_quant_kernel<2>, dim3((unsigned)blocks), dim3(256), 0, (hipStream_t)stream, (const unsigned char*)store, store_bytes, base,
                  cstride, lens, scale, offset, flip, out, C, c0, Ctot, Lpad, nseg, items);
    OD_CHECK_LAUNCH();
    return 0;
}

extern "C" int od_replicate_tail(float* x, const int* lens, const int* plens, int N, int C, int Lpad, void* stream) {
    if (!x || !lens || !plens || N < 1 || C < 1 || Lpad < 1) return OD_ERR_ARG;
    const long rows = (long)N * C, blocks = (rows + 3) / 4;
    if (blocks > 0x7fffffffL) return OD_ERR_UNSUPPORTED;
    OD_LAUNCH(replicate_tail_kernel, dim3((unsigned)blocks), dim3(256), 0, (hipStream_t)stream, x, lens, plens, C, Lpad, rows);
    OD_CHECK_LAUNCH();
    return 0;
}

extern "C" int od_proj_in(int dtype, const float* xt, const float* W, const float* bias, void* x, int ldx, int B, int E, int L,
                          int D, void* stream) {
    if (E > 8) return OD_ERR_UNSUPPORTED;
    if (D % 8 || ldx % 8) return OD_ERR_ALIGN;
    const long M = (long)B * L;
    int blocks = (int)((M + 15) / 16); if (blocks > 4096) blocks = 4096;
    DISPATCH_T(dtype, OD_LAUNCH((proj_in_kernel<T_>), dim3(blocks), dim3(256), 0, (hipStream_t)stream, xt, W, bias, (T_*)x, ldx, B, E, L, D));
    OD_CHECK_LAUNCH();
    return 0;
}

extern "C" int od_proj_in_bwd(int dtype, const float* xt, const void* dx, int ldx, float* dW, float* db, int B, int E, int L, int D,
                              void* stream) {
    if (E > 8) return OD_ERR_UNSUPPORTED;
    if (D % 8 || ldx % 8) return OD_ERR_ALIGN;
    const long M = (long)B * L;
    if (M > 0x7fffffffL) return OD_ERR_UNSUPPORTED;
    int blocks = (int)((M + 63) / 64); if (blocks > 512) blocks = 512; if (blocks < 1) blocks = 1;
    DISPATCH_T(dtype, OD_LAUNCH((proj_in_bwd_kernel<T_>), dim3(blocks), dim3(256), 0, (hipStream_t)stream, xt, (const T_*)dx, ldx, dW, db, B, E, L, D, od_det_active()));
    OD_CHECK_LAUNCH();
    return 0;
}

extern "C" int od_silu(int dtype, const void* x, void* y, long n, void* stream) {
    if (n % 8) return OD_ERR_ALIGN;
    long n8 = n / 8; int blocks = (int)((n8 + 255) / 256); if (blocks > 4096) blocks = 4096; if (blocks < 1) blocks = 1;
    DISPATCH_T(dtype, OD_LAUNCH((silu_kernel<T_>), dim3(blocks), dim3(256), 0, (hipStream_t)stream, (const T_*)x, (T_*)y, n8));
    OD_CHECK_LAUNCH();
    return 0;
}
extern "C" int od_silu_bwd(int dtype, const void* x, const void* dy, void* dx, long n, void* stream) {
    if (n % 8) return OD_ERR_ALIGN;
    long n8 = n / 8; int blocks = (int)((n8 + 255) / 256); if (blocks > 4096) blocks = 4096; if (blocks < 1) blocks = 1;
    DISPATCH_T(dtype, OD_LAUNCH((silu_bwd_kernel<T_>), dim3(blocks), dim3(256), 0, (hipStream_t)stream, (const T_*)x, (const T_*)dy, (T_*)dx, n8));
    OD_CHECK_LAUNCH();
    return 0;
}

template <class T>
__global__ __launch_bounds__(256) void scale_channels_kernel(T* __restrict__ x, int ldx, const float* __restrict__ scale, long M, int L, int C) {
    const int cg = C / 8;
    const long i = (long)blockIdx.x * 256 + threadIdx.x;
    if (i >= M * cg) return;
    const long m = i / cg;
    const int c = (int)(i % cg) * 8;
    float v[8], f[8];
    od_ld8(x + m * ldx + c, v);
    od_ld8(scale + (m / L) * C + c, f);
#pragma unroll
    for (int e = 0; e < 8; e++) v[e] *= f[e];
    od_st8(x + m * ldx + c, v);
}

extern "C" int od_scale_channels(int dtype, void* x, int ldx, const float* scale, int B, int L, int C, void* stream) {
    if (C % 8 || ldx % 8) return OD_ERR_ALIGN;
    const long M = (long)B * L, n = M * (C / 8);
    if (n == 0) return 0;
    DISPATCH_T(dtype, OD_LAUNCH((scale_channels_kernel<T_>), dim3((unsigned)((n + 255) / 256)), dim3(256), 0, (hipStream_t)stream, (T_*)x, ldx, scale, M, L, C));
    OD_CHECK_LAUNCH();
    return 0;
}

extern "C" int od_dwconv(int dtype, const void* x, int ldx, const float* w, const float* bias, void* y, int ldy, int B, int L,
                         int C, int ksize, void* stream) {
    if (C % 8 || ldx % 8 || ldy % 8) return OD_ERR_ALIGN;
    if (ksize != 3 && ksize != 5 && ksize != 7 && ksize != 9) return OD_ERR_UNSUPPORTED;
#ifndef OD_DW_SMALL_THREADS
#define OD_DW_SMALL_THREADS 131072
#endif
    const bool small = (long)B * (C / 8) * ((L + 31) / 32) < OD_DW_SMALL_THREADS;
    const int run = small ? 4 : 32;
    const long threads = (long)(C / 8) * ((L + run - 1) / run);
    dim3 grid((unsigned)((threads + 255) / 256), B);
#define DW_GO(KS_, RUN_) DISPATCH_T(dtype, OD_LAUNCH((dwconv_kernel<T_, KS_, RUN_>), grid, dim3(256), 0, (hipStream_t)stream, (const T_*)x, ldx, w, bias, (T_*)y, ldy, L, C))
    if (ksize == 5) { if (small) DW_GO(5, 4); else DW_GO(5, 32); }
    else if (ksize == 3) { if (small) DW_GO(3, 4); else DW_GO(3, 32); }
    else if (ksize == 7) { if (small) DW_GO(7, 4); else DW_GO(7, 32); }
    else { if (small) DW_GO(9, 4); else DW_GO(9, 32); }
#undef DW_GO
    OD_CHECK_LAUNCH();
    return 0;
}

extern "C" int od_dwconv_varlen(int dtype, const void* x, int ldx, const float* w, const float* bias, void* y, int ldy, const int* lens,
                                int B, int L, int C, int ksize, void* stream) {
    if (C % 8 || ldx % 8 || ldy % 8) return OD_ERR_ALIGN;
    if (ksize != 3 && ksize != 5 && ksize != 7 && ksize != 9) return OD_ERR_UNSUPPORTED;
    if (!lens) return OD_ERR_ARG;
    const bool small = (long)B * (C / 8) * ((L + 31) / 32) < OD_DW_SMALL_THREADS;
    const int run = small ? 4 : 32;
    const long threads = (long)(C / 8) * ((L + run - 1) / run);
    dim3 grid((unsigned)((threads + 255) / 256), B);
#define DW_GO(KS_, RUN_) DISPATCH_T(dtype, OD_LAUNCH((dwconv_kernel<T_, KS_, RUN_, true>), grid, dim3(256), 0, (hipStream_t)stream, (const T_*)x, ldx, w, bias, (T_*)y, ldy, L, C, lens))
    if (ksize == 5) { if (small) DW_GO(5, 4); else DW_GO(5, 32); }
    else if (ksize == 3) { if (small) DW_GO(3, 4); else DW_GO(3, 32); }
    else if (ksize == 7) { if (small) DW_GO(7, 4); else DW_GO(7, 32); }
    else { if (small) DW_GO(9, 4); else DW_GO(9, 32); }
#undef DW_GO
    OD_CHECK_LAUNCH();
    return 0;
}

extern "C" int od_dwconv_bwd(int dtype, const void* x, int ldx, const float* w, const void* dy, int lddy, void* dx, int lddx,
                             float* dw, float* db, int B, int L, int C, int ksize, void* stream) {
    if (C % 8 || ldx % 8 || lddy % 8 || lddx % 8) return OD_ERR_ALIGN;
    if (C > 1024 || (ksize > 5 && C > 512)) return OD_ERR_UNSUPPORTED;
    const long threads = (long)(C / 8) * ((L + DW_RUN_BWD - 1) / DW_RUN_BWD);
    dim3 grid((unsigned)((threads + 255) / 256), B);
    if (ksize == 5) DISPATCH_T(dtype, OD_LAUNCH((dwconv_bwd_kernel<T_, 5>), grid, dim3(256), 0, (hipStream_t)stream, (const T_*)x, ldx, w, (const T_*)dy, lddy, (T_*)dx, lddx, dw, db, L, C, od_det_active()));
    else if (ksize == 3) DISPATCH_T(dtype, OD_LAUNCH((dwconv_bwd_kernel<T_, 3>), grid, dim3(256), 0, (hipStream_t)stream, (const T_*)x, ldx, w, (const T_*)dy, lddy, (T_*)dx, lddx, dw, db, L, C, od_det_active()));
    else if (ksize == 7 && C <= 512) DISPATCH_T(dtype, OD_LAUNCH((dwconv_bwd_kernel<T_, 7>), grid, dim3(256), 0, (hipStream_t)stream, (const T_*)x, ldx, w, (const T_*)dy, lddy, (T_*)dx, lddx, dw, db, L, C, od_det_active()));
    else if (ksize == 9 && C <= 512) DISPATCH_T(dtype, OD_LAUNCH((dwconv_bwd_kernel<T_, 9>), grid, dim3(256), 0, (hipStream_t)stream, (const T_*)x, ldx, w, (const T_*)dy, lddy, (T_*)dx, lddx, dw, db, L, C, od_det_active()));
    else return OD_ERR_UNSUPPORTED;
    OD_CHECK_LAUNCH();
    return 0;
}

extern "C" int od_dwconv_bwd_varlen(int dtype, const void* x, int ldx, const float* w, const void* dy, int lddy, void* dx, int lddx,
                                    float* dw, float* db, const int* lens, int B, int L, int C, int ksize, void* stream) {
    if (C % 8 || ldx % 8 || lddy % 8 || lddx % 8) return OD_ERR_ALIGN;
    if (C > 1024 || (ksize > 5 && C > 512)) return OD_ERR_UNSUPPORTED;
    if (!lens) return OD_ERR_ARG;
    const long threads = (long)(C / 8) * ((L + DW_RUN_BWD - 1) / DW_RUN_BWD);
    dim3 grid((unsigned)((threads + 255) / 256), B);
#define DWB_GO(KS_) DISPATCH_T(dtype, OD_LAUNCH((dwconv_bwd_kernel<T_, KS_, true>), grid, dim3(256), 0, (hipStream_t)stream, (const T_*)x, ldx, w, (const T_*)dy, lddy, (T_*)dx, lddx, dw, db, L, C, od_det_active(), lens))
    if (ksize == 5) DWB_GO(5);
    else if (ksize == 3) DWB_GO(3);
    else if (ksize == 7) DWB_GO(7);
    else if (ksize == 9) DWB_GO(9);
    else return OD_ERR_UNSUPPORTED;
#undef DWB_GO
    OD_CHECK_LAUNCH();
    return 0;
}

extern "C" int od_linear_small(const float* x, const float* W, const float* b, float* out, float* pre, int B, int N, int K, int act,
                               void* stream) {
    OD_LAUNCH(linear_small_kernel, dim3((N + LS_NB - 1) / LS_NB, (B + 31) / 32), dim3(256), 0, (hipStream_t)stream, x, W, b, out, pre, B, N, K, act);
    OD_CHECK_LAUNCH();
    return 0;
}

extern "C" int od_linear_small_bwd(const float* x, const float* W, const float* pre, const float* dout, float* dpre, float* dW,
                                   float* db, float* dx, int accumulate_dx, int B, int N, int K, int act, void* stream) {
    if (act != OD_ACT_NONE && !pre) return OD_ERR_ARG;
    const long n = (long)B * N;
    OD_LAUNCH(linear_small_dpre_kernel, dim3((unsigned)((n + 255) / 256)), dim3(256), 0, (hipStream_t)stream, pre, dout, dpre, n, act);
    if (dW || db)
        OD_LAUNCH(linear_small_dw_kernel, dim3((K + 255) / 256, N), dim3(256), 0, (hipStream_t)stream, x, (const float*)dpre, dW, db, B, N, K);
    if (dx) {
        if (!accumulate_dx)
            OD_LAUNCH(zero_f32_kernel, dim3((unsigned)(((long)B * K + 255) / 256)), dim3(256), 0, (hipStream_t)stream, dx, (long)B * K);
        OD_LAUNCH(linear_small_dx_kernel, dim3((N + LS_NR - 1) / LS_NR, (B + 31) / 32, (K + 255) / 256), dim3(256), 0, (hipStream_t)stream, W,
                  (const float*)dpre, dx, B, N, K, od_det_active());
    }
    OD_CHECK_LAUNCH();
    return 0;
}

extern "C" int od_pack_weight(int dtype, const float* src, int N, int K, void* dst, int Np, int Kp, int transpose,
                              const int* row_map, void* stream) {
    const long n = (long)Np * Kp;
    if (dtype == OD_F32X3W) {
        if (transpose || Kp % 32) return OD_ERR_UNSUPPORTED;
        OD_LAUNCH(pack_weight_split_kernel, dim3((unsigned)((n + 255) / 256)), dim3(256), 0, (hipStream_t)stream, src, N, K, (bf16_t*)dst, Np, Kp, row_map);
        OD_CHECK_LAUNCH();
        return 0;
    }
    DISPATCH_T(dtype, OD_LAUNCH((pack_weight_kernel<T_>), dim3((unsigned)((n + 255) / 256)), dim3(256), 0, (hipStream_t)stream, src, N, K, (T_*)dst, Np, Kp, transpose, row_map));
    OD_CHECK_LAUNCH();
    return 0;
}
```

### osu_dreamer_amd/engine.py

```python
from __future__ import annotations


import math
import os
from collections import OrderedDict
from typing import Dict, List, Optional

import torch

from . import det, ops
from ._lib import OD_ACT_NONE, OD_ACT_SILU

OD_FUSE_FILM_DWCONV_DEFAULT = "0"

FP32_EPS = float(torch.finfo(torch.float32).eps)

PLAN_CACHE_DEFAULT = 16
PLAN_CACHE_DETERMINISTIC = 2


def _ceil(x: int, m: int) -> int:
    return (x + m - 1) // m * m


class Workspace:

    def __init__(self, device):
        self.device = device
        self.t: Dict[str, torch.Tensor] = {}
        self.bytes = 0

    def get(self, name: str, shape, dtype) -> torch.Tensor:
        t = self.t.get(name)
        if t is None:
            t = torch.zeros(shape, dtype=dtype, device=self.device)
            self.t[name] = t
            self.bytes += t.numel() * t.element_size()
            if name in det.WS_NAMES:
                ctx = det.context(self.device)
                if ctx is not None:
                    ctx.register(t)
        return t


class DenoiserEngine:
    def __init__(self, model):
        self.model = model
        a = model.args
        ba = a.backbone_args
        self.E, self.A, self.S = model.emb_dim, model.a_dim, model.style_dim
        self.Cg, self.D, self.U = a.global_cond_dim, a.backbone_dim, a.u_head_dim
        self.H, self.hd, self.depth = ba.n_heads, ba.head_dim, ba.depth
        self.dh = self.H * self.hd
        self.q_scale = math.log2(math.e) / math.sqrt(self.hd)
        self.radius = ba.radius
        self.ksize = 1 + 2 * ba.radius
        self.Hf = int(self.D * ba.expand * 2 / 3)
        self.Hp = _ceil(self.Hf, 64)
        if ba.radius not in (0, 1, 2, 3, 4):
            raise NotImplementedError("depthwise kernel sizes 3, 5, 7, 9 (radius 1-4) are compiled; radius 0 is the identity")
        if not (0.0 <= ba.dropout < 1.0):
            raise ValueError(f"dropout probability has to be in [0, 1), got {ba.dropout}")
        self.dropout = float(ba.dropout)
        self._packed: Dict[str, torch.Tensor] = {}
        self._packed_key = None
        self._plan_key = None
        self.ws: Optional[Workspace] = None
        self._plans: "OrderedDict[tuple, Workspace]" = OrderedDict()
        self.plan_switches = 0
        self.plan_builds = 0
        self._rowmap = None
        self.generation = 0
        self._attn_aux = None
        self._attn_ws_cache: Dict[tuple, "ops.FusedAttnBwdWorkspace"] = {}
        self._attn_ws = None
        self.varlen = False
        self.attn_f16 = False

    def _det_flush(self, *tensors):
        ctx = det.context(self.model.arena.data.device)
        if ctx is not None:
            for t in tensors:
                ctx.flush(t)

    def _det_flush_segment(self, name: str):
        ctx = det.context(self.model.arena.data.device)
        if ctx is not None:
            s, e = self.model.arena.segments(self.depth)[name]
            ctx.flush(self.model.arena.ensure_grad()[s:e])

    def P(self, name: str) -> torch.Tensor:
        return self.model.arena.view(name)

    def G(self, name: str) -> torch.Tensor:
        return self.model.arena.grad_view(name)

    def _gemm_weights(self) -> List[str]:
        names = ["proj_audio.0"]
        for i in range(self.depth):
            p = f"net.layers.{i}."
            names += [p + "proj_cl", p + "attn.qkv_proj", p + "attn.out_proj", p + "ffn.proj_vg.1", p + "ffn.proj_o"]
        return names

    def pack_weights(self, dtype: torch.dtype, train: bool, x3: bool = False):
        dev = self.model.arena.data.device
        x3 = bool(x3 and dtype == torch.float32 and not train)
        key = (dtype, train, dev, x3)
        if self._packed_key != key:
            self._packed = {}
            self._packed_key = key
            self.generation += 1
            Hf, Hp = self.Hf, self.Hp
            rm = [-1] * (2 * Hp)
            for j in range(Hf):
                rm[j] = j
                rm[Hp + j] = Hf + j
            self._rowmap = torch.tensor(rm, dtype=torch.int32, device=dev)
        pk = self._packed
        for n in self._gemm_weights():
            w = self.P(n + ".weight")
            N, K = w.shape[0], w.shape[1]
            Np, Kp, rmap = N, K, None
            if n.endswith("ffn.proj_vg.1"):
                Np, rmap = 2 * self.Hp, self._rowmap
            if n.endswith("ffn.proj_o"):
                Kp = self.Hp
            if n not in pk:
                pk[n] = torch.empty(Np, Kp, dtype=dtype, device=dev)
                if x3 and Kp % 32 == 0:
                    pk[n] = ops.SplitWeight(pk[n])
                if train:
                    pk[n + ".T"] = torch.empty(Kp, Np, dtype=dtype, device=dev)
                if rmap is not None:
                    pk[n + ".b"] = torch.empty(Np, dtype=torch.float32, device=dev)
            ops.pack_weight(w, pk[n], row_map=rmap)
            if train:
                ops.pack_weight(w, pk[n + ".T"], transpose=True, row_map=rmap)
            if rmap is not None:
                ops.pack_weight(self.P(n + ".bias"), pk[n + ".b"].view(Np, 1), row_map=rmap)

    def W(self, name: str, T: bool = False) -> torch.Tensor:
        return self._packed[name + (".T" if T else "")]

    def plain_gemm(self, A: torch.Tensor, W: torch.Tensor, bias, C: torch.Tensor):
        ops.gemm_nt(A, W, bias, C, x3=self.x3)

    def plan(self, B: int, L: int, Ba: int, dtype: torch.dtype, train: bool, x3: bool = False, lens=None, offs=None):
        dev = self.model.arena.data.device
        assert not (x3 and train), "the f32x3 product exists for the forward kernels only"
        varlen = lens is not None
        x3 = bool(x3 and dtype == torch.float32)
        ngroups = len(offs) - 1 if offs is not None else 0
        key = (B, L, Ba, dtype, train, dev, x3, getattr(self.model, "attn_dtype", None), varlen, ngroups)
        if key != self._plan_key:
            self.plan_switches += 1
            self.ws = self._plans.get(key) if train else None
            if self.ws is None:
                self.plan_builds += 1
                self.ws = Workspace(dev)
                tab = self.ws.get("rope", (L, self.hd // 2, 2), torch.float32)
                ops.rope_table(tab, L, self.hd)
            if train:
                limit = max(1, int(os.environ.get("OD_PLAN_CACHE", PLAN_CACHE_DEFAULT)))
                if det.enabled():
                    limit = min(limit, PLAN_CACHE_DETERMINISTIC)
                self._plans[key] = self.ws
                self._plans.move_to_end(key)
                while len(self._plans) > limit:
                    self._plans.popitem(last=False)
            self._plan_key = key
            self.generation += 1
        self.varlen = varlen
        if varlen:
            lens_t = torch.as_tensor(lens).to("cpu", torch.int32)
            if lens_t.shape != (B,) or int(lens_t.min()) < 1 or int(lens_t.max()) > L:
                raise ValueError(f"lens must hold B = {B} lengths in [1, {L}]")
            self.ws.get("vl.lens", (B,), torch.int32).copy_(lens_t)
            if offs is not None:
                offs_t = torch.as_tensor(offs).to("cpu", torch.int32)
                if int(offs_t[0]) != 0 or int(offs_t[-1]) != B or bool((offs_t[1:] <= offs_t[:-1]).any()):
                    raise ValueError("offs must rise strictly from 0 to B")
                self.ws.get("vl.offs", (ngroups + 1,), torch.int32).copy_(offs_t)
        self.B, self.L, self.Ba, self.dtype, self.train, self.x3 = B, L, Ba, dtype, train, x3
        self.M, self.Ma = B * L, Ba * L
        self.attn_f16 = getattr(self.model, "attn_dtype", None) == torch.float16
        if self.attn_f16 and (dtype != torch.bfloat16 or self.hd != 64):
            if not getattr(self, "_warned_f16_fallback", False):
                import warnings
                warnings.warn(f"attn_dtype = float16 applies to compute_dtype bfloat16 with head_dim 64; this plan (dtype {dtype}, head_dim "
                              f"{self.hd}) runs its attention in {dtype}")
                self._warned_f16_fallback = True
            self.attn_f16 = False
        if varlen and train and self.attn_f16:
            raise NotImplementedError("ragged training has no half-operand attention (attn_dtype = float16 runs the fused backward, which has no "
                                      "varlen form): train ragged batches with attn_dtype = None")
        return self.ws

    def buf(self, name, shape, dtype=None):
        return self.ws.get(name, shape, self.dtype if dtype is None else dtype)

    def lbuf(self, name, i, shape, dtype=None):
        return self.buf(f"{name}.{i}" if self.train else name, shape, dtype)

    def conditioning(self, audio: torch.Tensor, style: torch.Tensor):
        B, Ba, L = self.B, self.Ba, self.L
        D, A, Cg, U = self.D, self.A, self.Cg, self.U
        f32 = torch.float32
        a_t = self.buf("a_t", (self.Ma, A))
        a_pre = self.buf("a_pre", (self.Ma, A))
        a = self.buf("a", (self.Ma, A))
        ops.cl_to_frames(audio, a_t)
        ops.gemm_nt(a_t, self.W("proj_audio.0"), self.P("proj_audio.0.bias"), a_pre, x3=self.x3)
        ops.silu(a_pre, a)
        cg, cg_pre = self.buf("cg", (B, Cg), f32), self.buf("cg_pre", (B, Cg), f32)
        ops.linear_small(style, self.P("proj_style.0.weight"), self.P("proj_style.0.bias"), cg, cg_pre, OD_ACT_SILU)
        for i in range(self.depth):
            p = f"net.layers.{i}."
            for s in ("ssg1", "ssg2"):
                ops.linear_small(cg, self.P(p + s + ".weight"), self.P(p + s + ".bias"),
                                 self.buf(f"{s}.{i}", (B, 3 * D), f32))
            if not self.train:
                ops.gemm_nt(a, self.W(p + "proj_cl"), self.P(p + "proj_cl.bias"), self.buf(f"cl.{i}", (self.Ma, D)), x3=self.x3)
        ops.linear_small(cg, self.P("u_mod.weight"), self.P("u_mod.bias"), self.buf("umod", (B, 2 * U), f32))

    def pred(self, xt: torch.Tensor, u: torch.Tensor, v: torch.Tensor):
        B, L, M, D, dh, Hp = self.B, self.L, self.M, self.D, self.dh, self.Hp
        f32 = torch.float32
        tab = self.ws.t["rope"]
        bcast = self.Ba == 1 and B > 1
        x = self.lbuf("x_in", 0, (M, D))
        ops.proj_in(xt, self.P("proj_in.weight"), self.P("proj_in.bias"), x)

        def cl_of(i):
            if not self.train:
                return self.ws.t[f"cl.{i}"]
            cl = self.buf("cl", (self.Ma, D))
            ops.gemm_nt(self.ws.t["a"], self.W(f"net.layers.{i}.proj_cl"), self.P(f"net.layers.{i}.proj_cl.bias"), cl)
            return cl

        h1 = self.lbuf("h1", 0, (M, D))
        ops.rmsnorm_film(x, self.ws.t["ssg1.0"], cl_of(0), bcast, h1, self.lbuf("inv1", 0, (M,), f32), B, L)
        for i in range(self.depth):
            p = f"net.layers.{i}."
            ssg1, ssg2 = self.ws.t[f"ssg1.{i}"], self.ws.t[f"ssg2.{i}"]
            qkv = self.lbuf("qkv", i, (M, 3 * dh))
            if self.train or self.attn_f16 or self.hd not in (32, 64) or (2 * dh) % 128:
                qk = self.lbuf("qk16" if self.attn_f16 else "qk", i, (M, 2 * dh), torch.float16 if self.attn_f16 else None)
                ops.gemm_nt_qkrope_split(h1, self.W(p + "attn.qkv_proj"), self.P(p + "attn.qkv_proj.bias"), qkv, qk,
                                         self.P(p + "attn.q_norm.weight"), self.P(p + "attn.k_norm.weight"), tab, L, self.H,
                                         self.hd, FP32_EPS, x3=self.x3, q_scale=self.q_scale)
            else:
                ops.gemm_nt_qkrope(h1, self.W(p + "attn.qkv_proj"), self.P(p + "attn.qkv_proj.bias"), qkv,
                                   self.P(p + "attn.q_norm.weight"), self.P(p + "attn.k_norm.weight"), tab, L,
                                   self.H, self.hd, FP32_EPS, x3=self.x3, q_scale=self.q_scale)
                qk = qkv
            y = self.lbuf("y", i, (M, dh))
            lse = self.lbuf("lse", i, (B, self.H, L), f32)
            if self.varlen:
                ops.flash_attn_fwd_varlen(qk[:, :dh], qk[:, dh:], self._v_of(qkv), y, lse, self.ws.t["vl.lens"], B, self.H, L, self.hd,
                                          1.0 / math.sqrt(self.hd), x3=self.x3, q_prescaled=True)
            else:
                ops.flash_attn_fwd(qk[:, :dh], qk[:, dh:], self._v_of(qkv), y, lse, B, self.H, L, self.hd,
                                   1.0 / math.sqrt(self.hd), x3=self.x3, q_prescaled=True)
            ao = self.lbuf("ao", i, (M, D))
            self.plain_gemm(y, self.W(p + "attn.out_proj"), self.P(p + "attn.out_proj.bias"), ao)
            x_mid = self.lbuf("x_mid", i, (M, D))
            h2 = self.lbuf("h2", i, (M, D))
            fuse_dw = (self.radius > 0 and not self.varlen and D <= 512 and x.data_ptr() != x_mid.data_ptr() and x.dtype in (torch.bfloat16, torch.float32)
                       and os.environ.get("OD_FUSE_FILM_DWCONV", OD_FUSE_FILM_DWCONV_DEFAULT) == "1")
            if fuse_dw:
                hdw = self.lbuf("hdw", i, (M, D))
                ops.rmsnorm_gate_residual_film_dwconv(x, ao, ssg1, x_mid, self.lbuf("inv2", i, (M,), f32), ssg2, h2 if self.train else None,
                                                      self.lbuf("inv3", i, (M,), f32),
                                                      self.P(p + "ffn.proj_vg.0.weight"), self.P(p + "ffn.proj_vg.0.bias"), hdw, B, L, self.ksize)
            else:
                ops.rmsnorm_gate_residual_film(x, ao, ssg1, x_mid, self.lbuf("inv2", i, (M,), f32), ssg2, None, False, h2,
                                               self.lbuf("inv3", i, (M,), f32), B, L)
            if fuse_dw:
                pass
            elif self.radius > 0:
                hdw = self.lbuf("hdw", i, (M, D))
                if self.varlen:
                    ops.dwconv_varlen(h2, self.P(p + "ffn.proj_vg.0.weight"), self.P(p + "ffn.proj_vg.0.bias"), hdw, self.ws.t["vl.lens"], B, L,
                                      self.ksize)
                else:
                    ops.dwconv(h2, self.P(p + "ffn.proj_vg.0.weight"), self.P(p + "ffn.proj_vg.0.bias"), hdw, B, L, self.ksize)
            else:
                hdw = h2
            vg = self.lbuf("vg", i, (M, 2 * Hp))
            ops.gemm_nt(hdw, self.W(p + "ffn.proj_vg.1"), self._packed[p + "ffn.proj_vg.1.b"], vg, x3=self.x3)
            hh = self.lbuf("hh", i, (M, Hp))
            ops.swiglu_rmsnorm(vg, hh, self.lbuf("inv4", i, (M,), f32), self.Hf, Hp)
            if self._drop_active():
                ops.scale_channels(hh, self.draw_dropout_mask(i), B, L)
            fo = self.lbuf("fo", i, (M, D))
            self.plain_gemm(hh, self.W(p + "ffn.proj_o"), self.P(p + "ffn.proj_o.bias"), fo)
            x = self.buf(f"x_in.{i + 1}", (M, D)) if self.train else self.buf(f"x_in.{(i + 1) & 1}", (M, D))
            if i + 1 < self.depth:
                h1 = self.lbuf("h1", i + 1, (M, D))
                ops.rmsnorm_gate_residual_film(x_mid, fo, ssg2, x, self.lbuf("inv5", i, (M,), f32),
                                               self.ws.t[f"ssg1.{i + 1}"], cl_of(i + 1), bcast, h1,
                                               self.lbuf("inv1", i + 1, (M,), f32), B, L)
            else:
                ops.rmsnorm_gate_residual(x_mid, fo, ssg2, x, self.lbuf("inv5", i, (M,), f32), B, L)
        self._x_last = x
        ops.final_norm_proj_out(x, self.P("proj_out.weight"), self.P("proj_out.bias"), v,
                                self.buf("invf", (M,), f32), B, L)
        fsum = self.buf("fsum", (B, self.U), f32)
        fsum.zero_()
        if self.varlen:
            ops.uhead_fwd_varlen(xt, self._uhead_w(), fsum, self.ws.t["vl.lens"], self.U)
            self._det_flush(fsum)
            ops.uhead_tail_varlen(fsum, self.ws.t["umod"], self.P("u_out.weight"), self.P("u_out.bias"), u, self.ws.t["vl.lens"], L,
                                  self.model.u_scale)
        else:
            ops.uhead_fwd(xt, self._uhead_w(), fsum, self.U)
            self._det_flush(fsum)
            ops.uhead_tail(fsum, self.ws.t["umod"], self.P("u_out.weight"), self.P("u_out.bias"), u, L, self.model.u_scale)

    def _v_of(self, qkv: torch.Tensor) -> torch.Tensor:
        v = qkv[:, 2 * self.dh:]
        return v.view(torch.float16) if self.attn_f16 else v

    def attn_bwd_passes(self) -> int:
        from . import _lib
        return int(_lib.lib().cdll.od_flash_attn_bwd_fused_passes() if self.fused_attn_bwd() else _lib.lib().cdll.od_flash_attn_bwd_passes())

    def fused_attn_bwd(self) -> bool:
        import os
        if self.dtype != torch.bfloat16 or self.hd != 64 or self.varlen:
            return False
        if self.attn_f16:
            return True
        env = os.environ.get("OD_ATTN_BWD_FUSED", "")
        if env in ("0", "1"):
            return env == "1"
        return self.L >= 2048

    def attn_bwd_launch(self, i: int, dy: torch.Tensor, delta: torch.Tensor, dqkv: torch.Tensor, core_only: bool = False):
        t, dh, p = self.ws.t, self.dh, f"net.layers.{i}."
        qk, qkv, y, lse = t[f"qk16.{i}" if self.attn_f16 else f"qk.{i}"], t[f"qkv.{i}"], t[f"y.{i}"], t[f"lse.{i}"]
        wq, wk = self.P(p + "attn.q_norm.weight"), self.P(p + "attn.k_norm.weight")
        gq, gk = self.G(p + "attn.q_norm.weight"), self.G(p + "attn.k_norm.weight")
        scale = 1.0 / math.sqrt(self.hd)
        dqk = self.buf("d.qk", (self.M, 2 * dh))
        if self.fused_attn_bwd():
            key = (self.B, self.H, self.L, qk.device, qk.dtype)
            ws = self._attn_ws_cache.get(key)
            if ws is None:
                if len(self._attn_ws_cache) >= 4:
                    self._attn_ws_cache.pop(next(iter(self._attn_ws_cache)))
                ws = self._attn_ws_cache[key] = ops.FusedAttnBwdWorkspace(self.B, self.H, self.L, qk.device, qk.dtype)
                ws.checked = False
            self._attn_ws = ws
            ops.flash_attn_bwd_fused(qk[:, :dh], qk[:, dh:], self._v_of(qkv), y, dy, lse, dqk[:, :dh], dqk[:, dh:], dqkv[:, 2 * dh:],
                                     self.B, self.H, self.L, self.hd, scale, self._attn_ws, q_prescaled=True)
        else:
            if (self._attn_aux is None or self._attn_aux.device != qk.device) and qk.is_cuda:
                if self._attn_aux is not None:
                    self._attn_aux.close()
                with torch.cuda.device(qk.device):
                    self._attn_aux = ops.AttnAux()
                self._attn_aux.device = qk.device
            if self.varlen:
                ops.flash_attn_bwd_varlen(qk[:, :dh], qk[:, dh:], qkv[:, 2 * dh:], y, dy, lse, delta, dqk[:, :dh], dqk[:, dh:],
                                          dqkv[:, 2 * dh:], self.ws.t["vl.lens"], self.B, self.H, self.L, self.hd, scale, q_prescaled=True,
                                          aux=self._attn_aux)
            else:
                ops.flash_attn_bwd(qk[:, :dh], qk[:, dh:], qkv[:, 2 * dh:], y, dy, lse, delta, dqk[:, :dh], dqk[:, dh:],
                                   dqkv[:, 2 * dh:], self.B, self.H, self.L, self.hd, scale, q_prescaled=True, aux=self._attn_aux)
        if not core_only:
            ops.qk_norm_rope_bwd(qkv, wq, wk, t["rope"], dqk, dqkv, gq, gk, self.B, self.L, self.H, self.hd, FP32_EPS, q_scale=self.q_scale)

    def _drop_active(self) -> bool:
        return self.dropout > 0.0 and self.model.training

    def _drop_mask(self, i: int) -> torch.Tensor:
        return self.ws.t[f"drop.{i}"]

    def draw_dropout_mask(self, i: int) -> torch.Tensor:
        keep = 1.0 - self.dropout
        m = self.buf(f"drop.{i}", (self.B, self.Hp), torch.float32)
        m.zero_()
        m[:, :self.Hf] = torch.empty(self.B, self.Hf, device=m.device, dtype=torch.float32).bernoulli_(keep) / keep
        return m

    def _uhead_w(self, grads=False):
        f = self.G if grads else self.P
        return [f(f"u_head.{j}.{s}") for j in (0, 1, 3, 4) for s in ("weight", "bias")]

    def backward(self, xt: torch.Tensor, style: torch.Tensor, du: torch.Tensor, dv: torch.Tensor, reducer=None):
        assert self.train
        B, L, M, D, dh, Hf, Hp, A = self.B, self.L, self.M, self.D, self.dh, self.Hf, self.Hp, self.A
        f32 = torch.float32
        dctx = det.context(self.model.arena.data.device)
        if dctx is not None:
            dctx.register(self.model.arena.ensure_grad())
        tab = self.ws.t["rope"]
        cg, a = self.ws.t["cg"], self.ws.t["a"]
        dx = self.buf("d.x", (M, D))
        dbr = self.buf("d.branch", (M, D))
        dtmp = self.buf("d.tmp", (M, D))
        dhh = self.buf("d.hh", (M, Hp))
        dvg = self.buf("d.vg", (M, 2 * Hp))
        dy = self.buf("d.y", (M, dh))
        dqkv = self.buf("d.qkv", (M, 3 * dh))
        da = self.buf("d.a", (self.Ma, A))
        delta = self.buf("d.delta", (B, self.H, L), f32)
        dcg = self.buf("d.cg", (B, self.Cg), f32)
        dssg1, dssg2 = self.buf("d.ssg1", (B, 3 * D), f32), self.buf("d.ssg2", (B, 3 * D), f32)

        ops.final_norm_proj_out_bwd(self._x_last, self.ws.t["invf"], self.P("proj_out.weight"), dv, dx,
                                    self.G("proj_out.weight"), self.G("proj_out.bias"), B, L)
        dfm, dmod = self.buf("d.fm", (B, self.U), f32), self.buf("d.mod", (B, 2 * self.U), f32)
        if self.varlen:
            lens = self.ws.t["vl.lens"]
            ops.uhead_tail_bwd_varlen(self.ws.t["fsum"], self.ws.t["umod"], self.P("u_out.weight"), self.P("u_out.bias"), du,
                                      dfm, dmod, self.G("u_out.weight"), self.G("u_out.bias"), lens, L, self.model.u_scale)
            ops.uhead_bwd_varlen(xt, self._uhead_w(), dfm, self._uhead_w(grads=True), lens, self.U)
        else:
            ops.uhead_tail_bwd(self.ws.t["fsum"], self.ws.t["umod"], self.P("u_out.weight"), self.P("u_out.bias"), du,
                               dfm, dmod, self.G("u_out.weight"), self.G("u_out.bias"), L, self.model.u_scale)
            ops.uhead_bwd(xt, self._uhead_w(), dfm, self._uhead_w(grads=True), self.U)
        ops.linear_small_bwd(cg, self.P("u_mod.weight"), None, dmod, self.buf("d.lin_pre_umod", (B, 2 * self.U), f32),
                             self.G("u_mod.weight"), self.G("u_mod.bias"), dcg, False, OD_ACT_NONE)
        self._det_flush_segment("tail")
        if reducer is not None:
            reducer.segment_done("tail")

        for i in reversed(range(self.depth)):
            p = f"net.layers.{i}."
            t = self.ws.t
            ssg1, ssg2 = t[f"ssg1.{i}"], t[f"ssg2.{i}"]
            dssg1.zero_()
            dssg2.zero_()
            ops.rmsnorm_gate_residual_bwd(t[f"fo.{i}"], t[f"inv5.{i}"], ssg2, dx, dbr, dssg2, B, L)
            ops.gemm_tn(dbr, t[f"hh.{i}"], self.G(p + "ffn.proj_o.weight"), n_cols=D, k_cols=Hf,
                        dbias=self.G(p + "ffn.proj_o.bias"))
            ops.gemm_nt(dbr, self.W(p + "ffn.proj_o", T=True), None, dhh)
            if self._drop_active():
                ops.scale_channels(dhh, self._drop_mask(i), B, L)
            ops.swiglu_rmsnorm_bwd(t[f"vg.{i}"], t[f"inv4.{i}"], dhh, dvg, Hf, Hp)
            gw, gb = self.G(p + "ffn.proj_vg.1.weight"), self.G(p + "ffn.proj_vg.1.bias")
            hdw = t[f"hdw.{i}"] if self.radius > 0 else t[f"h2.{i}"]
            ops.gemm_tn(dvg, hdw, gw, n_cols=2 * Hp, k_cols=D, dbias=gb, n_block=Hp, n_valid=Hf)
            if self.radius > 0:
                self.plain_gemm(dvg, self.W(p + "ffn.proj_vg.1", T=True), None, dtmp)
                if self.varlen:
                    ops.dwconv_bwd_varlen(t[f"h2.{i}"], self.P(p + "ffn.proj_vg.0.weight"), dtmp, dbr, self.G(p + "ffn.proj_vg.0.weight"),
                                          self.G(p + "ffn.proj_vg.0.bias"), self.ws.t["vl.lens"], B, L, self.ksize)
                else:
                    ops.dwconv_bwd(t[f"h2.{i}"], self.P(p + "ffn.proj_vg.0.weight"), dtmp, dbr,
                                   self.G(p + "ffn.proj_vg.0.weight"), self.G(p + "ffn.proj_vg.0.bias"), B, L, self.ksize)
            else:
                self.plain_gemm(dvg, self.W(p + "ffn.proj_vg.1", T=True), None, dbr)
            ops.rmsnorm_film_bwd(t[f"x_mid.{i}"], t[f"inv3.{i}"], ssg2, dbr, dx, dssg2, B, L)
            ops.rmsnorm_gate_residual_bwd(t[f"ao.{i}"], t[f"inv2.{i}"], ssg1, dx, dbr, dssg1, B, L)
            ops.gemm_tn(dbr, t[f"y.{i}"], self.G(p + "attn.out_proj.weight"), dbias=self.G(p + "attn.out_proj.bias"))
            ops.gemm_nt(dbr, self.W(p + "attn.out_proj", T=True), None, dy)
            self.attn_bwd_launch(i, dy, delta, dqkv)
            ops.gemm_tn(dqkv, t[f"h1.{i}"], self.G(p + "attn.qkv_proj.weight"), dbias=self.G(p + "attn.qkv_proj.bias"))
            self.plain_gemm(dqkv, self.W(p + "attn.qkv_proj", T=True), None, dtmp)
            ops.gemm_tn(dtmp, a, self.G(p + "proj_cl.weight"), dbias=self.G(p + "proj_cl.bias"))
            ops.gemm_nt(dtmp, self.W(p + "proj_cl", T=True), None, da, accumulate=(i != self.depth - 1))
            ops.rmsnorm_film_bwd(t[f"x_in.{i}"], t[f"inv1.{i}"], ssg1, dtmp, dx, dssg1, B, L)
            lp = self.buf("d.lin_pre_ssg", (B, 3 * D), f32)
            self._det_flush(dssg1, dssg2)
            ops.linear_small_bwd(cg, self.P(p + "ssg2.weight"), None, dssg2, lp, self.G(p + "ssg2.weight"),
                                 self.G(p + "ssg2.bias"), dcg, True, OD_ACT_NONE)
            ops.linear_small_bwd(cg, self.P(p + "ssg1.weight"), None, dssg1, lp, self.G(p + "ssg1.weight"),
                                 self.G(p + "ssg1.bias"), dcg, True, OD_ACT_NONE)
            self._det_flush_segment(f"layer{i}")
            if reducer is not None:
                reducer.segment_done(f"layer{i}")

        ops.proj_in_bwd(xt, dx, self.G("proj_in.weight"), self.G("proj_in.bias"))
        da_pre = self.buf("d.a_pre", (self.Ma, A))
        ops.silu_bwd(self.ws.t["a_pre"], da, da_pre)
        ops.gemm_tn(da_pre, self.ws.t["a_t"], self.G("proj_audio.0.weight"), dbias=self.G("proj_audio.0.bias"))
        self._det_flush(dcg)
        ops.linear_small_bwd(style, self.P("proj_style.0.weight"), self.ws.t["cg_pre"], dcg,
                             self.buf("d.lin_pre_style", (B, self.Cg), f32), self.G("proj_style.0.weight"),
                             self.G("proj_style.0.bias"), None, False, OD_ACT_SILU)
        self._det_flush_segment("head")
        if reducer is not None:
            reducer.segment_done("head")
        if self.fused_attn_bwd() and self._attn_ws is not None and not self._attn_ws.checked:
            self._attn_ws.checked = True
            self.check_attn_status()

    def attn_status_ptr(self) -> int:
        return self._attn_ws.err_ptr() if self._attn_ws is not None else 0

    def attn_status_view(self) -> torch.Tensor:
        return self._attn_ws.err_view()

    ATTN_STATUS = {1: "a launch left jobs unprocessed (an XCD ran none of its workgroups): gradients incomplete",
                   2: "a launch with another (B, H, L) than the workspace's earlier launches was refused",
                   3: "a chain wait ran out of time (the predecessor's write never came; OD_FB_CHAIN_TIMEOUT_MS): dq is NaN"}

    def check_attn_status(self):
        if self._attn_ws is None:
            return
        code = 0
        for ws in {id(w): w for w in [self._attn_ws, *self._attn_ws_cache.values()]}.values():
            code = code or ws.status()
        if code != 0:
            raise RuntimeError(f"od_flash_attn_bwd_fused status {code}: {self.ATTN_STATUS.get(code, '?')}; the optimizer steps since then "
                               "were skipped.  OD_ATTN_BWD_FUSED=0 selects the two-kernel backward.")
```

### osu_dreamer_amd/ops.py

```python
from __future__ import annotations

import os
from typing import Optional

import torch

from . import _lib
from ._lib import OD_ACT_NONE, OD_ACT_SILU, OD_BF16, OD_EPI_NONE, OD_EPI_SILU, OD_F32, OD_F32X3, OD_F32X3W


def dt_code(dtype: torch.dtype) -> int:
    if dtype == torch.float32:
        return OD_F32
    if dtype == torch.bfloat16:
        return OD_BF16
    if dtype == torch.float16:
        return _lib.OD_F16
    raise TypeError(f"unsupported compute dtype {dtype}")


class SplitWeight:

    def __init__(self, storage: torch.Tensor):
        self.t = storage


def mm_code(dtype: torch.dtype, x3: bool, w=None) -> int:
    if isinstance(w, SplitWeight):
        if not (x3 and dtype == torch.float32):
            raise ValueError("a pre-split weight can only feed the fp32-as-3-x-bf16 product")
        return OD_F32X3W
    return OD_F32X3 if (x3 and dtype == torch.float32) else dt_code(dtype)


def _w(W):
    return W.t if isinstance(W, SplitWeight) else W


def _stream(t: torch.Tensor) -> int:
    return torch.cuda.current_stream(t.device).cuda_stream if t.is_cuda else 0


def _p(t: Optional[torch.Tensor]) -> Optional[int]:
    return None if t is None else t.data_ptr()


def _ld(t: torch.Tensor) -> int:
    assert t.dim() == 2 and t.stride(1) == 1, "need a row-major 2-D view"
    return t.stride(0)


def _f32(*ts):
    for t in ts:
        assert t is None or (t.dtype == torch.float32 and t.is_contiguous()), "expected contiguous fp32"


def _i32(*ts):
    for t in ts:
        assert t.dtype == torch.int32 and t.is_contiguous(), "expected contiguous int32"


def gemm_nt(A, W, bias, C, epilogue=OD_EPI_NONE, accumulate=False, x3=False):
    code, W = mm_code(A.dtype, x3, W), _w(W)
    M, K = A.shape
    N = W.shape[0]
    assert W.shape[1] == K and tuple(C.shape) == (M, N)
    assert A.dtype == W.dtype == C.dtype
    _f32(bias)
    _lib.lib().od_gemm_nt(code, _p(A), _ld(A), _p(W), _ld(W), _p(bias), _p(C), _ld(C), M, N, K,
                          epilogue, int(accumulate), _stream(A))


def gemm_nt_qkrope(A, W, bias, C, wq, wk, table, L, H, hd, eps, x3=False, q_scale=1.0):
    code, W = mm_code(A.dtype, x3, W), _w(W)
    M, K = A.shape
    N = W.shape[0]
    assert W.shape[1] == K and tuple(C.shape) == (M, N) and A.dtype == W.dtype == C.dtype
    _f32(bias, wq, wk, table)
    _lib.lib().od_gemm_nt_qkrope(code, _p(A), _ld(A), _p(W), _ld(W), _p(bias), _p(C), _ld(C), M, N, K,
                                 _p(wq), _p(wk), _p(table), L, H, hd, eps, q_scale, _stream(A))


def gemm_nt_qkrope_split(A, W, bias, C, qk_out, wq, wk, table, L, H, hd, eps, x3=False, q_scale=1.0):
    code, W = mm_code(A.dtype, x3, W), _w(W)
    M, K = A.shape
    N = W.shape[0]
    assert W.shape[1] == K and tuple(C.shape) == (M, N) and tuple(qk_out.shape) == (M, 2 * H * hd)
    assert A.dtype == W.dtype == C.dtype
    assert qk_out.dtype == A.dtype or (qk_out.dtype == torch.float16 and A.dtype == torch.bfloat16)
    _f32(bias, wq, wk, table)
    qk_code = _lib.OD_F16 if qk_out.dtype == torch.float16 else (OD_F32 if A.dtype == torch.float32 else code)
    _lib.lib().od_gemm_nt_qkrope_split(code, _p(A), _ld(A), _p(W), _ld(W), _p(bias), _p(C), _ld(C), _p(qk_out),
                                       _ld(qk_out), qk_code, M, N, K, _p(wq), _p(wk), _p(table), L, H, hd, eps, q_scale, _stream(A))


def gemm_tn(G, A, dW, n_cols=None, k_cols=None, dbias=None, n_block=0, n_valid=0):
    M = G.shape[0]
    N = n_cols if n_cols is not None else G.shape[1]
    K = k_cols if k_cols is not None else A.shape[1]
    rows = N if not n_block else (N // n_block) * n_valid
    assert not n_block or N % n_block == 0
    assert dW.dtype == torch.float32 and dW.is_contiguous() and dW.numel() == rows * K
    _f32(dbias)
    _lib.lib().od_gemm_tn_blocks(dt_code(G.dtype), _p(G), _ld(G), _p(A), _ld(A), _p(dW), K, _p(dbias), M, N, K, n_block, n_valid, _stream(G))


def colsum(G, out, n_cols=None):
    M = G.shape[0]
    N = n_cols if n_cols is not None else G.shape[1]
    _f32(out)
    _lib.lib().od_colsum(dt_code(G.dtype), _p(G), _ld(G), _p(out), M, N, _stream(G))


def pack_weight(src, dst, transpose=False, row_map=None):
    N = src.shape[0]
    K = src.numel() // N
    _f32(src)
    code = OD_F32X3W if isinstance(dst, SplitWeight) else dt_code(_w(dst).dtype)
    dst = _w(dst)
    if transpose:
        Kp, Np = dst.shape
    else:
        Np, Kp = dst.shape
    assert dst.is_contiguous()
    _lib.lib().od_pack_weight(code, _p(src), N, K, _p(dst), Np, Kp, int(transpose), _p(row_map), _stream(src))


def linear_small(x, W, b, out, pre=None, act=OD_ACT_NONE):
    B, K = x.shape
    N = W.shape[0]
    _f32(x, W, b, out, pre)
    _lib.lib().od_linear_small(_p(x), _p(W), _p(b), _p(out), _p(pre), B, N, K, act, _stream(x))


def linear_small_bwd(x, W, pre, dout, dpre, dW, db, dx, accumulate_dx, act=OD_ACT_NONE):
    B, K = x.shape
    N = W.shape[0]
    _f32(x, W, pre, dout, dpre, dW, db, dx)
    _lib.lib().od_linear_small_bwd(_p(x), _p(W), _p(pre), _p(dout), _p(dpre), _p(dW), _p(db), _p(dx),
                                   int(accumulate_dx), B, N, K, act, _stream(x))


def cl_to_frames(src, dst):
    B, C, L = src.shape
    _f32(src)
    _lib.lib().od_cl_to_frames(dt_code(dst.dtype), _p(src), _p(dst), _ld(dst), B, C, L, _stream(src))


def _feed_rows(base, cstride, lens, N):
    assert lens.dtype == torch.int32 and lens.dim() == 1 and lens.shape[0] == N and lens.is_contiguous(), "lens must be a contiguous int32 [B]"
    for t in (base, cstride):
        assert t.dtype == torch.int64 and t.dim() == 1 and t.shape[0] == N and t.is_contiguous(), "base / cstride must be contiguous int64 [N]"


def feed_gather(store, base, cstride, lens, out):
    N, C, Lpad = out.shape
    _f32(store, out)
    _feed_rows(base, cstride, lens, N)
    assert store.device == out.device == base.device == cstride.device == lens.device, "feed_gather: every tensor on one device"
    _lib.lib().od_feed_gather(_p(store), store.numel(), _p(base), _p(cstride), _p(lens), _p(out), N, C, Lpad, _stream(out))


def feed_gather_quant(store, elem_size, base, cstride, lens, out, c0=0, channels=None, scale=None, offset=None, flip=None):
    N, Ctot, Lpad = out.shape
    C = Ctot - c0 if channels is None else channels
    _f32(out)
    _feed_rows(base, cstride, lens, N)
    assert store.dtype == torch.uint8 and store.dim() == 1 and store.is_contiguous(), "the store is a flat uint8 tensor (its bytes)"
    assert (scale is None) == (offset is None), "scale and offset come together"
    for t in (scale, offset):
        assert t is None or (t.dtype == torch.float64 and tuple(t.shape) == (N, C) and t.is_contiguous()), "scale / offset must be contiguous fp64 (N, channels)"
    if flip is not None:
        _lens(flip, N)
    assert all(t is None or t.device == out.device for t in (store, base, cstride, lens, scale, offset, flip)), "feed_gather_quant: every tensor on one device"
    _lib.lib().od_feed_gather_quant(_p(store), store.numel(), elem_size, _p(base), _p(cstride), _p(lens), _p(scale), _p(offset), _p(flip), _p(out),
                                    N, C, c0, Ctot, Lpad, _stream(out))


def replicate_tail(x, lens, plens):
    N, C, Lpad = x.shape
    _f32(x)
    _lens(lens, N)
    _lens(plens, N)
    assert x.device == lens.device == plens.device, "replicate_tail: every tensor on one device"
    _lib.lib().od_replicate_tail(_p(x), _p(lens), _p(plens), N, C, Lpad, _stream(x))


def proj_in(xt, W, bias, x):
    B, E, L = xt.shape
    D = x.shape[1]
    _f32(xt, W, bias)
    _lib.lib().od_proj_in(dt_code(x.dtype), _p(xt), _p(W), _p(bias), _p(x), _ld(x), B, E, L, D, _stream(xt))


def proj_in_bwd(xt, dx, dW, db):
    B, E, L = xt.shape
    D = dx.shape[1]
    _f32(xt, dW, db)
    _lib.lib().od_proj_in_bwd(dt_code(dx.dtype), _p(xt), _p(dx), _ld(dx), _p(dW), _p(db), B, E, L, D, _stream(xt))


def silu(x, y):
    assert x.is_contiguous() and y.is_contiguous()
    _lib.lib().od_silu(dt_code(x.dtype), _p(x), _p(y), x.numel(), _stream(x))


def silu_bwd(x, dy, dx):
    assert x.is_contiguous() and dy.is_contiguous() and dx.is_contiguous()
    _lib.lib().od_silu_bwd(dt_code(x.dtype), _p(x), _p(dy), _p(dx), x.numel(), _stream(x))


def rmsnorm_film(x, ssg, cl, cl_bcast, h, inv_rms, B, L, eps=1e-6):
    C = x.shape[1]
    _f32(ssg, inv_rms)
    _lib.lib().od_rmsnorm_film(dt_code(x.dtype), _p(x), _ld(x), _p(ssg), _p(cl), _ld(cl) if cl is not None else 0,
                               int(cl_bcast), _p(h), _ld(h), _p(inv_rms), B, L, C, eps, _stream(x))


def rmsnorm_film_bwd(x, inv_rms, ssg, dh, dres, dssg, B, L):
    C = x.shape[1]
    _f32(ssg, inv_rms, dssg)
    _lib.lib().od_rmsnorm_film_bwd(dt_code(x.dtype), _p(x), _ld(x), _p(inv_rms), _p(ssg), _p(dh), _ld(dh), _p(dres),
                                   _ld(dres), _p(dssg), B, L, C, _stream(x))


def rmsnorm_gate_residual(x, h, ssg, xo, inv_rms, B, L, eps=1e-6):
    C = x.shape[1]
    _f32(ssg, inv_rms)
    _lib.lib().od_rmsnorm_gate_residual(dt_code(x.dtype), _p(x), _ld(x), _p(h), _ld(h), _p(ssg), _p(xo), _ld(xo),
                                        _p(inv_rms), B, L, C, eps, _stream(x))


def rmsnorm_gate_residual_film(x, h, ssg_a, xo, inv_a, ssg_b, cl, cl_bcast, h2, inv_b, B, L, eps=1e-6):
    _f32(ssg_a, ssg_b, inv_a, inv_b)
    _lib.lib().od_rmsnorm_gate_residual_film(dt_code(x.dtype), _p(x), _ld(x), _p(h), _ld(h), _p(ssg_a), _p(xo), _ld(xo),
                                             _p(inv_a), _p(ssg_b), _p(cl), _ld(cl) if cl is not None else 0, int(cl_bcast),
                                             _p(h2), _ld(h2), _p(inv_b), B, L, x.shape[1], eps, _stream(x))


def rmsnorm_gate_residual_film_dwconv(x, h, ssg_a, xo, inv_a, ssg_b, h2, inv_b, conv_w, conv_b, y, B, L, ksize, eps=1e-6):
    _f32(ssg_a, ssg_b, inv_a, inv_b, conv_w, conv_b)
    assert xo.data_ptr() != x.data_ptr() and xo.data_ptr() != h.data_ptr()
    _lib.lib().od_rmsnorm_gate_residual_film_dwconv(dt_code(x.dtype), _p(x), _ld(x), _p(h), _ld(h), _p(ssg_a), _p(xo), _ld(xo), _p(inv_a),
                                                    _p(ssg_b), _p(h2), _ld(h2) if h2 is not None else 0, _p(inv_b), _p(conv_w), _p(conv_b),
                                                    _p(y), _ld(y), B, L, x.shape[1], ksize, eps, _stream(x))


def rmsnorm_gate_residual_bwd(h, inv_rms, ssg, dy, dh, dssg, B, L):
    C = h.shape[1]
    _f32(ssg, inv_rms, dssg)
    _lib.lib().od_rmsnorm_gate_residual_bwd(dt_code(h.dtype), _p(h), _ld(h), _p(inv_rms), _p(ssg), _p(dy), _ld(dy),
                                            _p(dh), _ld(dh), _p(dssg), B, L, C, _stream(h))


def rope_table(table, L, hd):
    _f32(table)
    _lib.lib().od_rope_table(_p(table), L, hd, _stream(table))


def qk_norm_rope(qkv, wq, wk, table, qk_out, B, L, H, hd, eps, q_scale=1.0):
    _f32(wq, wk, table)
    _lib.lib().od_qk_norm_rope(dt_code(qkv.dtype), _p(qkv), _ld(qkv), _p(wq), _p(wk), _p(table), _p(qk_out),
                               _ld(qk_out), B, L, H, hd, eps, q_scale, _stream(qkv))


def qk_norm_rope_bwd(qkv, wq, wk, table, dqk, dqkv, dwq, dwk, B, L, H, hd, eps, q_scale=1.0):
    _f32(wq, wk, table, dwq, dwk)
    _lib.lib().od_qk_norm_rope_bwd(dt_code(qkv.dtype), _p(qkv), _ld(qkv), _p(wq), _p(wk), _p(table), _p(dqk), _ld(dqk),
                                   _p(dqkv), _ld(dqkv), _p(dwq), _p(dwk), B, L, H, hd, eps, q_scale, _stream(qkv))


def flash_attn_fwd(q, k, v, o, lse, B, H, L, hd, scale, x3=False, q_prescaled=False):
    _f32(lse)
    assert q.dtype == k.dtype == v.dtype and (o.dtype == q.dtype or (q.dtype == torch.float16 and o.dtype == torch.bfloat16))
    _lib.lib().od_flash_attn_fwd(mm_code(q.dtype, x3), _p(q), _ld(q), _p(k), _ld(k), _p(v), _ld(v), _p(o), _ld(o), _p(lse),
                                 B, H, L, hd, scale, int(q_prescaled), _stream(q))


class AttnAux:

    def __init__(self):
        import ctypes
        self.handle = ctypes.c_void_p()
        _lib.lib().od_attn_aux_create(ctypes.byref(self.handle))

    def close(self):
        if self.handle:
            _lib.lib().od_attn_aux_destroy(self.handle)
            self.handle = None

    def __del__(self):
        try:
            self.close()
        except Exception:
            pass


def flash_attn_fwd_varlen(q, k, v, o, lse, lens, B, H, L, hd, scale, x3=False, q_prescaled=False):
    _f32(lse)
    _i32(lens)
    assert q.dtype == k.dtype == v.dtype and (o.dtype == q.dtype or (q.dtype == torch.float16 and o.dtype == torch.bfloat16))
    _lib.lib().od_flash_attn_fwd_varlen(mm_code(q.dtype, x3), _p(q), _ld(q), _p(k), _ld(k), _p(v), _ld(v), _p(o), _ld(o), _p(lse),
                                        _p(lens), B, H, L, hd, scale, int(q_prescaled), _stream(q))


def flash_attn_bwd(q, k, v, o, do, lse, delta, dq, dk, dv, B, H, L, hd, scale, q_prescaled=False, aux=None):
    _f32(lse, delta)
    _lib.lib().od_flash_attn_bwd_aux(dt_code(q.dtype), _p(q), _ld(q), _p(k), _ld(k), _p(v), _ld(v), _p(o), _ld(o), _p(do),
                                     _ld(do), _p(lse), _p(delta), _p(dq), _ld(dq), _p(dk), _ld(dk), _p(dv), _ld(dv),
                                     B, H, L, hd, scale, int(q_prescaled), aux.handle if aux is not None else None, _stream(q))


def flash_attn_bwd_varlen(q, k, v, o, do, lse, delta, dq, dk, dv, lens, B, H, L, hd, scale, q_prescaled=False, aux=None):
    _f32(lse, delta)
    _i32(lens)
    _lib.lib().od_flash_attn_bwd_varlen(dt_code(q.dtype), _p(q), _ld(q), _p(k), _ld(k), _p(v), _ld(v), _p(o), _ld(o), _p(do),
                                        _ld(do), _p(lse), _p(delta), _p(dq), _ld(dq), _p(dk), _ld(dk), _p(dv), _ld(dv), _p(lens),
                                        B, H, L, hd, scale, int(q_prescaled), aux.handle if aux is not None else None, _stream(q))


class FusedAttnBwdWorkspace:

    def __init__(self, B, H, L, device, dtype=torch.bfloat16):
        import ctypes
        total, zero = ctypes.c_long(), ctypes.c_long()
        _lib.lib().od_flash_attn_bwd_fused_ws_bytes(dt_code(dtype), B, H, L, ctypes.byref(total), ctypes.byref(zero))
        self.shape = (B, H, L)
        self.dtype = dtype
        self.bytes = total.value
        assert zero.value <= self.bytes
        self.zero_bytes = zero.value
        self.buf = torch.empty(self.bytes, dtype=torch.uint8, device=device)
        self.reset()

    def reset(self):
        self.buf[:self.zero_bytes].zero_()

    def err_ptr(self) -> int:
        return self.buf.data_ptr() + int(_lib.lib().cdll.od_flash_attn_bwd_fused_err_offset())

    def err_view(self) -> torch.Tensor:
        off = int(_lib.lib().cdll.od_flash_attn_bwd_fused_err_offset())
        return self.buf[off:off + 4].view(torch.int32)

    def status(self) -> int:
        import ctypes
        err = ctypes.c_int(-1)
        _lib.lib().od_flash_attn_bwd_fused_status(_p(self.buf), ctypes.byref(err), _stream(self.buf))
        return err.value


def flash_attn_bwd_fused(q, k, v, o, do, lse, dq, dk, dv, B, H, L, hd, scale, ws: FusedAttnBwdWorkspace, q_prescaled=False):
    _f32(lse)
    assert ws.shape == (B, H, L), (ws.shape, (B, H, L))
    assert q.dtype == k.dtype == v.dtype and o.dtype == do.dtype == dq.dtype == dk.dtype == dv.dtype == torch.bfloat16
    assert q.dtype == torch.bfloat16 or (q.dtype == torch.float16 and ws.dtype == torch.float16)
    _lib.lib().od_flash_attn_bwd_fused(dt_code(q.dtype), _p(q), _ld(q), _p(k), _ld(k), _p(v), _ld(v), _p(o), _ld(o), _p(do), _ld(do),
                                       _p(lse), _p(dq), _ld(dq), _p(dk), _ld(dk), _p(dv), _ld(dv), B, H, L, hd, scale, int(q_prescaled),
                                       _p(ws.buf), ws.bytes, _stream(q))


def dwconv(x, w, bias, y, B, L, ksize):
    C = x.shape[1]
    _f32(w, bias)
    _lib.lib().od_dwconv(dt_code(x.dtype), _p(x), _ld(x), _p(w), _p(bias), _p(y), _ld(y), B, L, C, ksize, _stream(x))


def dwconv_varlen(x, w, bias, y, lens, B, L, ksize):
    C = x.shape[1]
    _f32(w, bias)
    _i32(lens)
    _lib.lib().od_dwconv_varlen(dt_code(x.dtype), _p(x), _ld(x), _p(w), _p(bias), _p(y), _ld(y), _p(lens), B, L, C, ksize, _stream(x))


def dwconv_bwd(x, w, dy, dx, dw, db, B, L, ksize):
    C = x.shape[1]
    _f32(w, dw, db)
    _lib.lib().od_dwconv_bwd(dt_code(x.dtype), _p(x), _ld(x), _p(w), _p(dy), _ld(dy), _p(dx), _ld(dx), _p(dw), _p(db),
                             B, L, C, ksize, _stream(x))


def dwconv_bwd_varlen(x, w, dy, dx, dw, db, lens, B, L, ksize):
    C = x.shape[1]
    _f32(w, dw, db)
    _i32(lens)
    _lib.lib().od_dwconv_bwd_varlen(dt_code(x.dtype), _p(x), _ld(x), _p(w), _p(dy), _ld(dy), _p(dx), _ld(dx), _p(dw), _p(db),
                                    _p(lens), B, L, C, ksize, _stream(x))


def scale_channels(x, scale, B, L):
    _f32(scale)
    assert scale.shape == (B, x.shape[1]) and scale.is_contiguous()
    _lib.lib().od_scale_channels(dt_code(x.dtype), _p(x), _ld(x), _p(scale), B, L, x.shape[1], _stream(x))


def swiglu_rmsnorm(vg, hh, inv_rms, Hf, Hp, eps=1e-6):
    _f32(inv_rms)
    _lib.lib().od_swiglu_rmsnorm(dt_code(vg.dtype), _p(vg), _ld(vg), _p(hh), _ld(hh), _p(inv_rms), vg.shape[0], Hf, Hp,
                                 eps, _stream(vg))


def swiglu_rmsnorm_bwd(vg, inv_rms, dhh, dvg, Hf, Hp):
    _f32(inv_rms)
    _lib.lib().od_swiglu_rmsnorm_bwd(dt_code(vg.dtype), _p(vg), _ld(vg), _p(inv_rms), _p(dhh), _ld(dhh), _p(dvg),
                                     _ld(dvg), vg.shape[0], Hf, Hp, _stream(vg))


def final_norm_proj_out(x, W, bias, v, inv_rms, B, L, eps=1e-6):
    C = x.shape[1]
    E = W.shape[0]
    _f32(W, bias, v, inv_rms)
    _lib.lib().od_final_norm_proj_out(dt_code(x.dtype), _p(x), _ld(x), _p(W), _p(bias), _p(v), _p(inv_rms), B, L, C, E,
                                      eps, _stream(x))


def final_norm_proj_out_bwd(x, inv_rms, W, dv, dx, dW, db, B, L):
    C = x.shape[1]
    E = W.shape[0]
    _f32(W, dv, inv_rms, dW, db)
    _lib.lib().od_final_norm_proj_out_bwd(dt_code(x.dtype), _p(x), _ld(x), _p(inv_rms), _p(W), _p(dv), _p(dx), _ld(dx),
                                          _p(dW), _p(db), B, L, C, E, _stream(x))


def uhead_fwd(xt, w, fsum, U):
    B, E, L = xt.shape
    _f32(xt, fsum, *w)
    _lib.lib().od_uhead_fwd(_p(xt), *[_p(t) for t in w], _p(fsum), B, E, L, U, _stream(xt))


def uhead_fwd_varlen(xt, w, fsum, lens, U):
    B, E, L = xt.shape
    _f32(xt, fsum, *w)
    _i32(lens)
    _lib.lib().od_uhead_fwd_varlen(_p(xt), *[_p(t) for t in w], _p(fsum), _p(lens), B, E, L, U, _stream(xt))


def uhead_bwd(xt, w, dfm, g, U):
    B, E, L = xt.shape
    _f32(xt, dfm, *w, *g)
    _lib.lib().od_uhead_bwd(_p(xt), *[_p(t) for t in w], _p(dfm), *[_p(t) for t in g], B, E, L, U, _stream(xt))


def uhead_bwd_varlen(xt, w, dfm, g, lens, U):
    B, E, L = xt.shape
    _f32(xt, dfm, *w, *g)
    _i32(lens)
    _lib.lib().od_uhead_bwd_varlen(_p(xt), *[_p(t) for t in w], _p(dfm), *[_p(t) for t in g], _p(lens), B, E, L, U, _stream(xt))


def uhead_tail(fsum, mod, w_out, b_out, u, L, u_scale):
    B, U = fsum.shape
    _f32(fsum, mod, w_out, b_out, u)
    _lib.lib().od_uhead_tail(_p(fsum), _p(mod), _p(w_out), _p(b_out), _p(u), B, U, L, u_scale, _stream(fsum))


def uhead_tail_varlen(fsum, mod, w_out, b_out, u, lens, L, u_scale):
    B, U = fsum.shape
    _f32(fsum, mod, w_out, b_out, u)
    _i32(lens)
    _lib.lib().od_uhead_tail_varlen(_p(fsum), _p(mod), _p(w_out), _p(b_out), _p(u), _p(lens), B, U, L, u_scale, _stream(fsum))


def uhead_tail_bwd(fsum, mod, w_out, b_out, du, dfm, dmod, dw_out, db_out, L, u_scale):
    B, U = fsum.shape
    _f32(fsum, mod, w_out, b_out, du, dfm, dmod, dw_out, db_out)
    _lib.lib().od_uhead_tail_bwd(_p(fsum), _p(mod), _p(w_out), _p(b_out), _p(du), _p(dfm), _p(dmod), _p(dw_out),
                                 _p(db_out), B, U, L, u_scale, _stream(fsum))


def uhead_tail_bwd_varlen(fsum, mod, w_out, b_out, du, dfm, dmod, dw_out, db_out, lens, L, u_scale):
    B, U = fsum.shape
    _f32(fsum, mod, w_out, b_out, du, dfm, dmod, dw_out, db_out)
    _i32(lens)
    _lib.lib().od_uhead_tail_bwd_varlen(_p(fsum), _p(mod), _p(w_out), _p(b_out), _p(du), _p(dfm), _p(dmod), _p(dw_out),
                                        _p(db_out), _p(lens), B, U, L, u_scale, _stream(fsum))


def make_xt(x0, x1, t, xt, dsq):
    B, E, L = x0.shape
    _f32(x0, x1, t, xt, dsq)
    _lib.lib().od_make_xt(_p(x0), _p(x1), _p(t), _p(xt), _p(dsq), B, E, L, _stream(x0))


def make_xt_varlen(x0, x1, t, xt, dsq, lens):
    B, E, L = x0.shape
    _f32(x0, x1, t, xt, dsq)
    _i32(lens)
    _lib.lib().od_make_xt_varlen(_p(x0), _p(x1), _p(t), _p(xt), _p(dsq), _p(lens), B, E, L, _stream(x0))


def loss_grad(xt, x1, u, v, dsq, dv, sums, c0, osl_w, del_w):
    B, E, L = xt.shape
    _f32(xt, x1, u, v, dsq, dv, sums)
    _lib.lib().od_loss_grad(_p(xt), _p(x1), _p(u), _p(v), _p(dsq), _p(dv), _p(sums), B, E, L, c0, osl_w, del_w, _stream(xt))


def loss_grad_varlen(xt, x1, u, v, dsq, dv, sums, lens, c0, osl_w, del_w):
    B, E, L = xt.shape
    _f32(xt, x1, u, v, dsq, dv, sums)
    _i32(lens)
    _lib.lib().od_loss_grad_varlen(_p(xt), _p(x1), _p(u), _p(v), _p(dsq), _p(dv), _p(sums), _p(lens), B, E, L, c0, osl_w, del_w,
                                   _stream(xt))


def loss_finalize(sums, dsq, u, out, du, c0, osl_w, del_w):
    B = u.shape[0]
    _f32(sums, dsq, u, out, du)
    _lib.lib().od_loss_finalize(_p(sums), _p(dsq), _p(u), _p(out), _p(du), B, c0, osl_w, del_w, _stream(u))


def sampler_step(x, u, v, eta):
    B, E, L = x.shape
    _f32(x, u, v, eta)
    _lib.lib().od_sampler_step(_p(x), _p(u), _p(v), _p(eta), B, E, L, _stream(x))


def sampler_eta(u, eta, c0, num_steps):
    _f32(u, eta)
    _lib.lib().od_sampler_eta(_p(u), _p(eta), u.shape[0], c0, num_steps, _stream(u))


def sampler_eta_groups(u, offs, eta, c0, num_steps):
    _f32(u, eta)
    _i32(offs)
    G = offs.shape[0] - 1
    assert eta.numel() >= 2 * G
    _lib.lib().od_sampler_eta_groups(_p(u), _p(offs), _p(eta), G, c0, num_steps, _stream(u))


def sampler_step_varlen(x, u, v, eta, lens, offs):
    B, E, L = x.shape
    _f32(x, u, v, eta)
    _i32(lens, offs)
    _lib.lib().od_sampler_step_varlen(_p(x), _p(u), _p(v), _p(eta), _p(lens), _p(offs), offs.shape[0] - 1, B, E, L, _stream(x))


def sqnorm(g, out, status_ptr: int = 0):
    _f32(g, out)
    _lib.lib().od_sqnorm(_p(g), g.numel(), _p(out), status_ptr or None, _stream(g))


def adamw_ema(p, g, m, v, ema, lr, beta1, beta2, eps, weight_decay, step, ema_decay, ema_mode, gnorm_sq, max_norm, status_ptr: int = 0):
    _f32(p, g, m, v, ema, gnorm_sq)
    _lib.lib().od_adamw_ema(_p(p), _p(g), _p(m), _p(v), _p(ema), p.numel(), lr, beta1, beta2, eps, weight_decay, step,
                            ema_decay, ema_mode, _p(gnorm_sq), max_norm, status_ptr or None, _stream(p))


def ema_update(ema, p, decay, mode):
    _f32(ema, p)
    _lib.lib().od_ema_update(_p(ema), _p(p), p.numel(), decay, mode, _stream(p))


def style_conditioning(labels, rff_w, rff_b, cond_w, cond_b, null_labels, c):
    B, NL = labels.shape
    F, H = cond_w.shape[1], cond_w.shape[2]
    _f32(labels, rff_w, rff_b, cond_w, cond_b, null_labels, c)
    _lib.lib().od_style_conditioning(_p(labels), _p(rff_w), _p(rff_b), _p(cond_w), _p(cond_b), _p(null_labels), _p(c),
                                     B, NL, F, H, _stream(labels))


def rmsnorm_rows(x, gamma, y, eps):
    M, C = x.shape
    _f32(x, gamma, y)
    _lib.lib().od_rmsnorm_rows(_p(x), _p(gamma), _p(y), M, C, eps, _stream(x))


def style_conditioning_bwd(labels, rff_w, rff_b, dc, dcond_w, dcond_b, dnull_labels):
    B, NL = labels.shape
    F, H = dcond_w.shape[1], dcond_w.shape[2]
    _f32(labels, rff_w, rff_b, dc, dcond_w, dcond_b, dnull_labels)
    assert tuple(dc.shape) == (B, H) and rff_w.numel() == F and rff_b.numel() == F
    assert tuple(dcond_w.shape) == (NL, F, H) and tuple(dcond_b.shape) == (NL, H) and tuple(dnull_labels.shape) == (NL, H)
    _lib.lib().od_style_conditioning_bwd(_p(labels), _p(rff_w), _p(rff_b), _p(dc), _p(dcond_w), _p(dcond_b), _p(dnull_labels),
                                         B, NL, F, H, _stream(labels))


def rmsnorm_rows_bwd(x, gamma, dy, dx, dgamma, eps, accumulate_dx=False):
    M, C = x.shape
    _f32(x, gamma, dy, dx, dgamma)
    assert dy.shape == x.shape == dx.shape and (gamma is None or gamma.numel() == C) and (dgamma is None or dgamma.numel() == C)
    _lib.lib().od_rmsnorm_rows_bwd(_p(x), _p(gamma), _p(dy), _p(dx), _p(dgamma), M, C, eps, int(accumulate_dx), _stream(x))


def cast_rows(src, dst):
    assert src.is_contiguous() and dst.is_contiguous() and src.numel() == dst.numel()
    _lib.lib().od_cast_rows(dt_code(src.dtype), _p(src), dt_code(dst.dtype), _p(dst), src.numel(), _stream(src))


def spec_features_conv(audio, w1, b1, g1, w2, b2, g2, out, eps=1e-6):
    B, F, L = audio.shape
    _f32(audio, w1, b1, g1, w2, b2, g2)
    _lib.lib().od_spec_features_conv(dt_code(out.dtype), _p(audio), _p(w1), _p(b1), _p(g1), _p(w2), _p(b2), _p(g2),
                                     _p(out), _ld(out), B, F, L, eps, _stream(audio))


def rmsnorm_affine_film(x, gamma, ssg, y, B, L, act=OD_ACT_NONE, eps=1e-6):
    _f32(gamma, ssg)
    _lib.lib().od_rmsnorm_affine_film(dt_code(x.dtype), _p(x), _ld(x), _p(gamma), _p(ssg), _p(y), _ld(y), B, L, x.shape[1],
                                      eps, act, _stream(x))


def rmsnorm_affine_gate_residual(x, h, gamma, ssg, xo, B, L, eps=1e-6):
    _f32(gamma, ssg)
    _lib.lib().od_rmsnorm_affine_gate_residual(dt_code(x.dtype), _p(x), _ld(x), _p(h), _ld(h), _p(gamma), _p(ssg), _p(xo),
                                               _ld(xo), B, L, x.shape[1], eps, _stream(x))


def unet_mixer(x, p, p_bcast, gx, gamma, xo, B, L, eps=1e-6):
    _f32(gamma)
    _lib.lib().od_unet_mixer(dt_code(x.dtype), _p(x), _ld(x), _p(p), _ld(p), int(p_bcast), _p(gx), _ld(gx), _p(gamma),
                             _p(xo), _ld(xo), B, L, x.shape[1], eps, _stream(x))


def unet_down(x, w, bias, y, B, Lo, stride):
    _f32(w, bias)
    _lib.lib().od_unet_down(dt_code(x.dtype), _p(x), _ld(x), _p(w), _p(bias), _p(y), _ld(y), B, Lo, x.shape[1], stride,
                            _stream(x))


def unet_up(x, w, bias, y, B, Li, stride):
    _f32(w, bias)
    _lib.lib().od_unet_up(dt_code(x.dtype), _p(x), _ld(x), _p(w), _p(bias), _p(y), _ld(y), B, Li, x.shape[1], stride,
                          _stream(x))


def chart_head(x, W, bias, out, B, L, n_sigmoid, rms=False, eps=1e-6):
    _f32(W, bias, out)
    N = W.shape[0]
    _lib.lib().od_chart_head(dt_code(x.dtype), _p(x), _ld(x), _p(W), _p(bias), _p(out), B, L, x.shape[1], N, n_sigmoid,
                             int(rms), eps, _stream(x))


def attn_pool(scores, values, out, B, L, heads, hd):
    _f32(out)
    _lib.lib().od_attn_pool(dt_code(scores.dtype), _p(scores), _ld(scores), _p(values), _ld(values), _p(out), B, L, heads, hd,
                            _stream(scores))


def latent_bwd_ws_floats(kind, B, L, C, n=0):
    if kind == "spec":
        return B * -(-L // 32) * 4880
    f = _lib.lib().cdll.od_latent_bwd_block_frames(C)
    assert f > 0, "C must be a power of two in 8..512"
    per_row, flat = -(-L // f), -(-(B * L) // f)
    if kind == "film":
        return B * per_row * 3 * C
    if kind == "gate":
        return B * per_row * 2 * C
    if kind == "mixer":
        return (per_row if n else B * per_row) * C
    if kind in ("down", "up"):
        return flat * (2 * (n // 2) + 2) * C
    if kind == "head":
        return flat * n * (C + 1)
    raise ValueError(kind)


def rmsnorm_affine_film_bwd(x, gamma, ssg, dy, dx, dgamma, dssg, ws, B, L, act=OD_ACT_NONE, accumulate_dx=False, eps=1e-6):
    _f32(gamma, ssg, dgamma, dssg, ws)
    assert x.dtype == dy.dtype == dx.dtype
    _lib.lib().od_rmsnorm_affine_film_bwd(dt_code(x.dtype), _p(x), _ld(x), _p(gamma), _p(ssg), _p(dy), _ld(dy), _p(dx), _ld(dx),
                                          int(accumulate_dx), _p(dgamma), _p(dssg), _p(ws), ws.numel(), B, L, x.shape[1], eps, act,
                                          _stream(x))


def rmsnorm_affine_gate_residual_bwd(h, gamma, ssg, dxo, dh, dgamma, dssg, ws, B, L, eps=1e-6):
    _f32(gamma, ssg, dgamma, dssg, ws)
    assert h.dtype == dxo.dtype == dh.dtype
    _lib.lib().od_rmsnorm_affine_gate_residual_bwd(dt_code(h.dtype), _p(h), _ld(h), _p(gamma), _p(ssg), _p(dxo), _ld(dxo), _p(dh),
                                                   _ld(dh), _p(dgamma), _p(dssg), _p(ws), ws.numel(), B, L, h.shape[1], eps, _stream(h))


def unet_mixer_bwd(p, p_bcast, gx, gamma, dxo, dp, dgx, dgamma, ws, B, L, eps=1e-6):
    _f32(gamma, dgamma, ws)
    assert p.dtype == gx.dtype == dxo.dtype == dgx.dtype and dp.dtype == (torch.float32 if p_bcast else p.dtype)
    _lib.lib().od_unet_mixer_bwd(dt_code(p.dtype), _p(p), _ld(p), int(p_bcast), _p(gx), _ld(gx), _p(gamma), _p(dxo), _ld(dxo), _p(dp),
                                 _ld(dp), _p(dgx), _ld(dgx), _p(dgamma), _p(ws), ws.numel(), B, L, p.shape[1], eps, _stream(p))


def unet_down_bwd(x, w, dy, dx, dw, db, ws, B, Lo, stride):
    _f32(w, dw, db, ws)
    assert x.dtype == dy.dtype == dx.dtype
    _lib.lib().od_unet_down_bwd(dt_code(x.dtype), _p(x), _ld(x), _p(w), _p(dy), _ld(dy), _p(dx), _ld(dx), _p(dw), _p(db), _p(ws),
                                ws.numel(), B, Lo, x.shape[1], stride, _stream(x))


def unet_up_bwd(x, w, dy, dx, dw, db, ws, B, Li, stride):
    _f32(w, dw, db, ws)
    assert x.dtype == dy.dtype == dx.dtype
    _lib.lib().od_unet_up_bwd(dt_code(x.dtype), _p(x), _ld(x), _p(w), _p(dy), _ld(dy), _p(dx), _ld(dx), _p(dw), _p(db), _p(ws),
                              ws.numel(), B, Li, x.shape[1], stride, _stream(x))


def chart_head_bwd(x, W, bias, dout, dx, dW, db, ws, B, L, rms=False, eps=1e-6):
    _f32(W, bias, dout, dW, db, ws)
    N = W.shape[0]
    assert tuple(dout.shape) == (B, N, L) and x.dtype == dx.dtype
    _lib.lib().od_chart_head_bwd(dt_code(x.dtype), _p(x), _ld(x), _p(W), _p(bias), _p(dout), _p(dx), _ld(dx), _p(dW), _p(db), _p(ws),
                                 ws.numel(), B, L, x.shape[1], N, int(rms), eps, _stream(x))


def attn_pool_bwd(scores, values, dout, dscores, dvalues, B, L, heads, hd):
    _f32(dout)
    assert scores.dtype == values.dtype == dscores.dtype == dvalues.dtype
    _lib.lib().od_attn_pool_bwd(dt_code(scores.dtype), _p(scores), _ld(scores), _p(values), _ld(values), _p(dout), _p(dscores),
                                _ld(dscores), _p(dvalues), _ld(dvalues), B, L, heads, hd, _stream(scores))


def spec_features_conv_bwd(audio, w1, b1, g1, w2, b2, g2, dout, dw1, db1, dg1, dw2, db2, dg2, ws, eps=1e-6):
    B, F, L = audio.shape
    _f32(audio, w1, b1, g1, w2, b2, g2, dw1, db1, dg1, dw2, db2, dg2, ws)
    _lib.lib().od_spec_features_conv_bwd(dt_code(dout.dtype), _p(audio), _p(w1), _p(b1), _p(g1), _p(w2), _p(b2), _p(g2), _p(dout),
                                         _ld(dout), _p(dw1), _p(db1), _p(dg1), _p(dw2), _p(db2), _p(dg2), _p(ws), ws.numel(), B, F, L,
                                         eps, _stream(audio))


def add_rows(x, y):
    assert x.dtype == y.dtype and x.shape == y.shape and x.is_contiguous() and y.is_contiguous()
    _lib.lib().od_add_rows(dt_code(x.dtype), _p(x), _p(y), x.numel(), _stream(x))


def proj_in_bwd_input(dx, W, dxt):
    B, E, L = dxt.shape
    _f32(W, dxt)
    _lib.lib().od_proj_in_bwd_input(dt_code(dx.dtype), _p(dx), _ld(dx), _p(W), _p(dxt), B, E, L, dx.shape[1], _stream(dx))


def _lens(lens, B):
    _i32(lens)
    assert lens.dim() == 1 and lens.shape[0] == B and lens.is_contiguous(), "lens must be a contiguous int32 [B]"


def spec_features_conv_varlen(audio, w1, b1, g1, w2, b2, g2, out, lens, eps=1e-6):
    B, F, L = audio.shape
    _f32(audio, w1, b1, g1, w2, b2, g2)
    _lens(lens, B)
    _lib.lib().od_spec_features_conv_varlen(dt_code(out.dtype), _p(audio), _p(w1), _p(b1), _p(g1), _p(w2), _p(b2), _p(g2),
                                            _p(out), _ld(out), _p(lens), B, F, L, eps, _stream(audio))


def rmsnorm_affine_film_varlen(x, gamma, ssg, y, lens, B, L, act=OD_ACT_NONE, eps=1e-6):
    _f32(gamma, ssg)
    _lens(lens, B)
    _lib.lib().od_rmsnorm_affine_film_varlen(dt_code(x.dtype), _p(x), _ld(x), _p(gamma), _p(ssg), _p(y), _ld(y), _p(lens), B, L,
                                             x.shape[1], eps, act, _stream(x))


def unet_mixer_varlen(x, p, prow, gx, gamma, xo, B, L, eps=1e-6):
    _f32(gamma)
    _lens(prow, B)
    _lib.lib().od_unet_mixer_varlen(dt_code(x.dtype), _p(x), _ld(x), _p(p), _ld(p), _p(prow), _p(gx), _ld(gx), _p(gamma),
                                    _p(xo), _ld(xo), B, L, x.shape[1], eps, _stream(x))


def unet_down_varlen(x, w, bias, y, lens, B, Lo, stride):
    _f32(w, bias)
    _lens(lens, B)
    _lib.lib().od_unet_down_varlen(dt_code(x.dtype), _p(x), _ld(x), _p(w), _p(bias), _p(y), _ld(y), _p(lens), B, Lo, x.shape[1],
                                   stride, _stream(x))


def unet_up_varlen(x, w, bias, y, lens, B, Li, stride):
    _f32(w, bias)
    _lens(lens, B)
    _lib.lib().od_unet_up_varlen(dt_code(x.dtype), _p(x), _ld(x), _p(w), _p(bias), _p(y), _ld(y), _p(lens), B, Li, x.shape[1],
                                 stride, _stream(x))


def chart_head_varlen(x, W, bias, out, lens, B, L, n_sigmoid, rms=False, eps=1e-6):
    _f32(W, bias, out)
    _lens(lens, B)
    _lib.lib().od_chart_head_varlen(dt_code(x.dtype), _p(x), _ld(x), _p(W), _p(bias), _p(out), _p(lens), B, L, x.shape[1],
                                    W.shape[0], n_sigmoid, int(rms), eps, _stream(x))


def attn_pool_varlen(scores, values, out, lens, B, L, heads, hd):
    _f32(out)
    _lens(lens, B)
    _lib.lib().od_attn_pool_varlen(dt_code(scores.dtype), _p(scores), _ld(scores), _p(values), _ld(values), _p(out), _p(lens), B, L,
                                   heads, hd, _stream(scores))


def _u8(*ts):
    for t in ts:
        assert t.dtype == torch.uint8 and t.is_contiguous(), "expected contiguous uint8"


def mmd_imq(z, prior, out, dz, ws):
    N, D = z.shape
    _f32(z, prior, out, dz, ws)
    assert prior.shape == z.shape == dz.shape and out.numel() >= 4
    _lib.lib().od_mmd_imq(_p(z), _p(prior), _p(out), _p(dz), _p(ws), ws.numel(), N, D, _stream(z))


def scale_by(x, g, y):
    _f32(x, g, y)
    assert x.shape == y.shape
    _lib.lib().od_scale_by(_p(x), _p(g), _p(y), x.numel(), _stream(x))


def latent_perturb(z, s, eps_z, eps_s, u_s, repl, u_span, u_start, z_out, s_out, masked, start_span, s_noise, z_noise, s_mask_frac,
                   z_mask_frac, training):
    B2, E, l = z.shape
    S = s.shape[1]
    assert z.dtype == torch.float32
    _f32(s, eps_z, eps_s, u_s, repl, u_span, u_start, z_out, s_out)
    _u8(masked)
    _i32(start_span)
    assert tuple(z_out.shape) == (B2, E, l) and tuple(s_out.shape) == (B2, S) and masked.numel() == B2 and start_span.numel() == 2 * B2
    _lib.lib().od_latent_perturb(_p(z), z.stride(0), z.stride(1), z.stride(2), _p(s), _p(eps_z), _p(eps_s), _p(u_s), _p(repl), _p(u_span),
                                 _p(u_start), _p(z_out), _p(s_out), _p(masked), _p(start_span), B2, E, l, S, s_noise, z_noise,
                                 s_mask_frac, z_mask_frac, int(training), _stream(s))


def latent_perturb_bwd(dz_out, ds_out, masked, start_span, dz, ds):
    B2, E, l = dz_out.shape
    _f32(dz_out, ds_out, dz, ds)
    _u8(masked)
    _i32(start_span)
    _lib.lib().od_latent_perturb_bwd(_p(dz_out), _p(ds_out), _p(masked), _p(start_span), _p(dz), _p(ds), B2, E, l, ds_out.shape[1],
                                     _stream(ds))


def latent_loss_block_frames() -> int:
    return _lib.lib().cdll.od_latent_loss_block_frames()


def latent_loss_ws_floats(B2, L) -> int:
    return _lib.lib().cdll.od_latent_loss_ws_floats(B2, L)


def latent_loss(logits, chart, pred_labels, true_labels, masked, s_reg, loss_ema, ema_init, out, coef, ws, s_reg_weight, training):
    B2, C, L = logits.shape
    _f32(logits, chart, pred_labels, true_labels, s_reg, loss_ema, out, coef, ws)
    _u8(masked, ema_init)
    assert C == 9 and chart.shape == logits.shape and tuple(pred_labels.shape) == tuple(true_labels.shape) == (B2, 5)
    assert masked.numel() == B2 and loss_ema.numel() == 11 and out.numel() >= 13 and coef.numel() >= 11
    _lib.lib().od_latent_loss(_p(logits), _p(chart), _p(pred_labels), _p(true_labels), _p(masked), _p(s_reg), _p(loss_ema), _p(ema_init),
                              _p(out), _p(coef), _p(ws), ws.numel(), B2, L, s_reg_weight, int(training), _stream(logits))


def latent_loss_bwd(logits, chart, pred_labels, true_labels, masked, coef, g, dlogits, dlabels, ds_reg, s_reg_weight):
    B2, _, L = logits.shape
    _f32(logits, chart, pred_labels, true_labels, coef, g, dlogits, dlabels, ds_reg)
    _u8(masked)
    assert dlogits.shape == logits.shape and tuple(dlabels.shape) == (B2, 5)
    _lib.lib().od_latent_loss_bwd(_p(logits), _p(chart), _p(pred_labels), _p(true_labels), _p(masked), _p(coef), _p(g), _p(dlogits),
                                  _p(dlabels), _p(ds_reg), B2, L, s_reg_weight, _stream(logits))


def mmd_imq_pairs(s, prior, out, ws):
    N, S = s.shape
    _f32(s, prior, out, ws)
    assert N % 2 == 0 and prior.shape == s.shape and tuple(out.shape) == (N // 2, 4) and ws.numel() >= 3 * N
    _lib.lib().od_mmd_imq_pairs(_p(s), _p(prior), _p(out), _p(ws), ws.numel(), N // 2, S, _stream(s))


def latent_loss_maps(logits, chart, hlens, pred_labels, true_labels, s_reg, loss_ema, out, ws, s_reg_weight):
    B2, C, Hmax = logits.shape
    G = B2 // 2
    _f32(logits, chart, pred_labels, true_labels, loss_ema, out, ws)
    _lens(hlens, B2)
    assert C == 9 and B2 % 2 == 0 and chart.shape == logits.shape and tuple(pred_labels.shape) == tuple(true_labels.shape) == (B2, 5)
    assert s_reg.dtype == torch.float32 and s_reg.dim() == 1 and s_reg.shape[0] == G and (G == 1 or s_reg.stride(0) >= 1)
    assert loss_ema.numel() == 11 and tuple(out.shape) == (G, 13)
    _lib.lib().od_latent_loss_maps(_p(logits), _p(chart), _p(hlens), _p(pred_labels), _p(true_labels), _p(s_reg), max(s_reg.stride(0), 1),
                                   _p(loss_ema), _p(out), _p(ws), ws.numel(), G, Hmax, s_reg_weight, _stream(logits))


def latent_eval_maps_ws_floats(G, Pmax) -> int:
    return _lib.lib().cdll.od_latent_eval_maps_ws_floats(G, Pmax)


def latent_eval_maps(chart, pred_chart, plens, z, zlens, pred_labels, true_labels, out, ws):
    G, C, Pmax = chart.shape
    _f32(chart, pred_chart, z, pred_labels, true_labels, out, ws)
    _lens(plens, G)
    _lens(zlens, G)
    assert C == 9 and pred_chart.shape == chart.shape and z.dim() == 3 and z.shape[0] == G
    assert tuple(pred_labels.shape) == tuple(true_labels.shape) == (G, 5) and tuple(out.shape) == (G, 8)
    _lib.lib().od_latent_eval_maps(_p(chart), _p(pred_chart), _p(plens), _p(z), _p(zlens), _p(pred_labels), _p(true_labels), _p(out), _p(ws),
                                   ws.numel(), G, Pmax, z.shape[1], z.shape[2], _stream(chart))
```

Measured before the change: 3.137.

## Batch weight packing and small linears; restructure u-head kernels and proj_in backward

Replaces the per-weight pack_weight calls with one table-driven batched pack kernel, and replaces the per-layer ssg/u_mod linear_small calls with one grouped launch. This targets per-step launch and host overhead. The u-head forward stages its small weights in shared memory and computes z4 with register blocking. The u-head backward swaps the warp-reduce-plus-shared-atomics accumulation for per-thread register accumulators and adds a U=64 specialisation with a launch-bounds occupancy hint. proj_in_bwd gets a new launch shape; the larger rewrite risks correctness slips in the gradient reductions.

Result: no change. 3.153, median of 6 (+0.5%).

```diff
diff --git a/include/osu_dreamer_hip.h b/include/osu_dreamer_hip.h
--- a/include/osu_dreamer_hip.h
+++ b/include/osu_dreamer_hip.h
@@ -32,9 +32,11 @@
 int od_colsum(int dtype, const void* G, int ldg, float* out, int M, int N, void* stream);
 int od_pack_weight(int dtype, const float* src, int N, int K, void* dst, int Np, int Kp, int transpose,
                    const int* row_map, void* stream);
+int od_pack_weights(int dtype, const long* table, int n, long blocks, void* stream);
 
 int od_linear_small(const float* x, const float* W, const float* b, float* out, float* pre, int B, int N, int K, int act,
                     void* stream);
+int od_linear_small_group(const float* x, const long* descs, int n, int B, int K, void* stream);
 int od_linear_small_bwd(const float* x, const float* W, const float* pre, const float* dout, float* dpre, float* dW,
                         float* db, float* dx, int accumulate_dx, int B, int N, int K, int act, void* stream);
 
diff --git a/osu_dreamer_amd/csrc/heads.hip b/osu_dreamer_amd/csrc/heads.hip
--- a/osu_dreamer_amd/csrc/heads.hip
+++ b/osu_dreamer_amd/csrc/heads.hip
@@ -63,14 +63,42 @@
     __syncthreads();
 }
 
-template <bool VL = false>
+template <int BS = 1>
+__device__ __forceinline__ void uhead_z4(const UHeadSmem& S, const float* __restrict__ b4, int grp, int cpg, int i, int U,
+                                         float (&z)[MAXU / 8]) {
+    int c[MAXU / 8];
+#pragma unroll
+    for (int q = 0; q < MAXU / 8; q++) {
+        c[q] = grp * cpg + (q < cpg ? q : cpg - 1);
+        z[q] = b4[c[q] * BS];
+    }
+#pragma unroll 2
+    for (int cc = 0; cc < U; cc++) {
+        const float zv = S.z3s[cc][i];
+#pragma unroll
+        for (int q = 0; q < MAXU / 8; q++) z[q] += S.w4s[c[q]][cc] * zv;
+    }
+}
+
+template <bool VL = false, int CU = 0>
 __global__ __launch_bounds__(256) void uhead_fwd_kernel(const float* __restrict__ xt, UHeadW P, float* __restrict__ fsum,
-                                                        int E, int L, int U, int nwin, int wpb, const OdDetTable* __restrict__ det,
+                                                        int E, int L, int U_, int nwin, int wpb, const OdDetTable* __restrict__ det,
                                                         const int* __restrict__ lens = nullptr) {
     __shared__ UHeadSmem S;
+    const int U = CU ? CU : U_;
     const int b = blockIdx.y, t = threadIdx.x;
     const int Lb = VL ? od_uniform(lens[b]) : L;
     const int i = t & 31, grp = t >> 5, cpg = U / 8;
+    float* const lw = &S.g4s[0][0];
+    static_assert(sizeof(S.g4s) >= sizeof(float) * (MAXE * 4 + MAXU * (MAXE + 6)), "staged u-head weights");
+    float *const lw0 = lw, *const lb0 = lw0 + MAXE * 3, *const lw1 = lb0 + MAXE, *const lb1 = lw1 + MAXU * MAXE, *const lw3 = lb1 + MAXU,
+          *const lb3 = lw3 + MAXU * 3, *const lb4 = lb3 + MAXU;
+    for (int k = t; k < U * E; k += 256) lw1[k] = P.w1[k];
+    if (t < U * 3) lw3[t] = P.w3[t];
+    if (t < U) { lb1[t] = P.b1[t]; lb3[t] = P.b3[t]; lb4[t] = P.b4[t]; }
+    if (t < E * 3) lw0[t] = P.w0[t];
+    if (t < E) lb0[t] = P.b0[t];
+    P.w0 = lw0; P.b0 = lb0; P.w1 = lw1; P.b1 = lb1; P.w3 = lw3; P.b3 = lb3; P.b4 = lb4;
     uhead_load_w4(S, P, U);
     float acc[MAXU / 8];
 #pragma unroll
@@ -83,15 +111,11 @@
         uhead_window_fwd(S, xt, P, b, l0, E, L, U, Lb);
         const int f = l0 - 1 + i;
         const bool own = (i >= 1 && i < UW - 1 && f < Lb);
-#pragma unroll
-        for (int q = 0; q < MAXU / 8; q++) {
-            if (q < cpg) {
-                const int c = grp * cpg + q;
-                float z = P.b4[c];
-                for (int cc = 0; cc < U; cc++) z += S.w4s[c][cc] * S.z3s[cc][i];
-                if (own) acc[q] += od_silu(z);
-            }
-        }
+        float z[MAXU / 8];
+        uhead_z4(S, P.b4, grp, cpg, i, U, z);
+#pragma unroll
+        for (int q = 0; q < MAXU / 8; q++)
+            if (own) acc[q] += od_silu(z[q]);
         __syncthreads();
     }
 #pragma unroll
@@ -105,27 +129,35 @@
     float *dw0, *db0, *dw1, *db1, *dw3, *db3, *dw4, *db4;
 };
 
-template <bool VL>
+template <bool VL, int CU>
 __device__ __forceinline__ void uhead_bwd_body(const float* __restrict__ xt, const UHeadW& P, const float* __restrict__ dfm,
-                                               const UHeadG& G, int E, int L, int U, int nwin, const OdDetTable* __restrict__ det,
+                                               const UHeadG& G, int E, int L, int U_, int nwin, const OdDetTable* __restrict__ det,
                                                const int* __restrict__ lens) {
+    constexpr int NQ = MAXU / 8;
+    const int U = CU ? CU : U_;
     __shared__ UHeadSmem S;
-    __shared__ float sdw3[MAXU][3], sdb3[MAXU], sdb4[MAXU], sdw1[MAXU][MAXE], sdb1[MAXU], sdw0[MAXE][3], sdb0[MAXE];
+    __shared__ float sw3[MAXU * 3], sdf[MAXU];
+    static_assert(sizeof(UHeadSmem) + sizeof(float) * MAXU * 4 <= 53 * 1024, "three blocks per CU");
     const int b = blockIdx.y, t = threadIdx.x;
     const int i = t & 31, grp = t >> 5, cpg = U / 8;
     const int Lb = VL ? od_uniform(lens[b]) : L;
-    for (int idx = t; idx < MAXU; idx += 256) {
-        sdb3[idx] = 0.f; sdb4[idx] = 0.f; sdb1[idx] = 0.f;
-        for (int j = 0; j < 3; j++) sdw3[idx][j] = 0.f;
-        for (int e = 0; e < MAXE; e++) sdw1[idx][e] = 0.f;
-    }
-    if (t < MAXE) { sdb0[t] = 0.f; for (int j = 0; j < 3; j++) sdw0[t][j] = 0.f; }
+    const float invL = 1.0f / (float)Lb;
+    if (t < U) { S.w4s[t][MAXU] = P.b4[t]; sdf[t] = dfm[(size_t)b * U + t] * invL; }
+    if (t < 3 * U) sw3[t] = P.w3[t];
     uhead_load_w4(S, P, U);
-    float adw4[16];
+    int cq[NQ];
+#pragma unroll
+    for (int q = 0; q < NQ; q++) cq[q] = grp * cpg + (q < cpg ? q : cpg - 1);
+    float adw4[16], adw1[2] = {0.f, 0.f}, adw3 = 0.f;
+    float pb4[NQ], pb1[NQ], pb0 = 0.f, pw0[3] = {0.f, 0.f, 0.f};
 #pragma unroll
     for (int q = 0; q < 16; q++) adw4[q] = 0.f;
-    const float invL = 1.0f / (float)Lb;
-
+#pragma unroll
+    for (int q = 0; q < NQ; q++) { pb4[q] = 0.f; pb1[q] = 0.f; }
+    const bool dw4_shared = (256 % U) == 0;
+    const int UU = U * U, cc4 = t % U, cb4 = t / U, cs4 = 256 / U;
+
+#pragma unroll 1
     for (int wi = 0; wi < UWPB; wi++) {
         const int win = blockIdx.x * UWPB + wi;
         if (win >= nwin) break;
@@ -135,118 +167,171 @@
         const int f = l0 - 1 + i;
         const bool inr = (f >= 0 && f < Lb);
         const bool own = (i >= 1 && i < UW - 1 && f < Lb);
-#pragma unroll
-        for (int q = 0; q < MAXU / 8; q++) {
-            if (q < cpg) {
-                const int c = grp * cpg + q;
-                float z = P.b4[c];
-                for (int cc = 0; cc < U; cc++) z += S.w4s[c][cc] * S.z3s[cc][i];
-                const float g = inr ? dfm[(size_t)b * U + c] * invL * od_silu_grad(z) : 0.f;
-                S.g4s[c][i] = g;
-                const float s = red32(own ? g : 0.f);
-                if (i == 0) atomicAdd(&sdb4[c], s);
+        const int iend = (Lb - (l0 - 1)) < (UW - 1) ? (Lb - (l0 - 1)) : (UW - 1);
+        {
+            float z[NQ];
+            uhead_z4<MAXU + 1>(S, &S.w4s[0][MAXU], grp, cpg, i, U, z);
+#pragma unroll
+            for (int q = 0; q < NQ; q++) {
+                const float g = inr ? sdf[cq[q]] * od_silu_grad(z[q]) : 0.f;
+                S.g4s[cq[q]][i] = g;
+                pb4[q] += own ? g : 0.f;
             }
         }
         __syncthreads();
         {
-            const int iend = (Lb - (l0 - 1)) < (UW - 1) ? (Lb - (l0 - 1)) : (UW - 1);
-#pragma unroll
-            for (int q = 0; q < 16; q++) {
-                const int o = t + 256 * q;
-                if (o < U * U) {
-                    const int c = o / U, cc = o % U;
-                    float s = 0.f;
-                    for (int ii = 1; ii < iend; ii++) s += S.g4s[c][ii] * S.z3s[cc][ii];
-                    adw4[q] += s;
+            if (dw4_shared) {
+                float s[16];
+                int row[16];
+#pragma unroll
+                for (int q = 0; q < 16; q++) {
+                    s[q] = 0.f;
+                    row[q] = cb4 + cs4 * q < MAXU ? cb4 + cs4 * q : MAXU - 1;
+                }
+#pragma unroll 2
+                for (int ii = 1; ii < iend; ii++) {
+                    const float zv = S.z3s[cc4][ii];
+#pragma unroll
+                    for (int q = 0; q < 16; q++) s[q] += S.g4s[row[q]][ii] * zv;
+                }
+#pragma unroll
+                for (int q = 0; q < 16; q++)
+                    if (t + 256 * q < UU) adw4[q] += s[q];
+            } else {
+#pragma unroll
+                for (int q = 0; q < 16; q++) {
+                    const int o = t + 256 * q;
+                    if (o < UU) {
+                        const int c = o / U, cc = o % U;
+                        float s = 0.f;
+                        for (int ii = 1; ii < iend; ii++) s += S.g4s[c][ii] * S.z3s[cc][ii];
+                        adw4[q] += s;
+                    }
                 }
             }
         }
         __syncthreads();
-        float dz3v[MAXU / 8];
-#pragma unroll
-        for (int q = 0; q < MAXU / 8; q++) {
-            dz3v[q] = 0.f;
-            if (q < cpg) {
-                const int cc = grp * cpg + q;
+        float dz3v[NQ];
+#pragma unroll
+        for (int q = 0; q < NQ; q++) dz3v[q] = 0.f;
+#pragma unroll 2
+        for (int c = 0; c < U; c++) {
+            const float gv = S.g4s[c][i];
+#pragma unroll
+            for (int q = 0; q < NQ; q++) dz3v[q] += S.w4s[c][cq[q]] * gv;
+        }
+        __syncthreads();
+#pragma unroll
+        for (int q = 0; q < NQ; q++) S.z3s[cq[q]][i] = dz3v[q];
+        __syncthreads();
+        if (t < 3 * U) {
+            const int c = t / 3, j = t - 3 * c;
+            float s = 0.f;
+#pragma unroll 2
+            for (int ii = 1; ii < iend; ii++) s += S.z3s[c][ii] * S.a1s[c][ii + j];
+            adw3 += s;
+        } else if (t - 3 * U < U) {
+            const int c = t - 3 * U;
+            float s = 0.f;
+#pragma unroll 2
+            for (int ii = 1; ii < iend; ii++) s += S.z3s[c][ii];
+            adw3 += s;
+        }
+#pragma unroll
+        for (int q = 0; q < NQ; q++) {
+            const int c = cq[q];
+            float dz1 = 0.f;
+            if (own) {
+                float da1 = 0.f;
+                for (int j = 0; j < 3; j++) da1 += sw3[c * 3 + j] * S.z3s[c][i - j + 1];
+                dz1 = da1 * od_silu_grad(S.z1s[c][i + 1]);
+            }
+            S.g4s[c][i] = dz1;
+            pb1[q] += dz1;
+        }
+        __syncthreads();
+#pragma unroll
+        for (int k = 0; k < 2; k++) {
+            const int o = t + 256 * k;
+            if (o < U * E) {
+                const int c = o / E, e = o % E;
                 float s = 0.f;
-                for (int c = 0; c < U; c++) s += S.w4s[c][cc] * S.g4s[c][i];
-                dz3v[q] = s;
+#pragma unroll 2
+                for (int ii = 1; ii < UW - 1; ii++) s += S.g4s[c][ii] * S.z0s[e][ii + 1];
+                adw1[k] += s;
             }
         }
-        __syncthreads();
-#pragma unroll
-        for (int q = 0; q < MAXU / 8; q++)
-            if (q < cpg) S.z3s[grp * cpg + q][i] = dz3v[q];
-        __syncthreads();
-#pragma unroll
-        for (int q = 0; q < MAXU / 8; q++) {
-            if (q < cpg) {
-                const int c = grp * cpg + q;
-                const float g = own ? S.z3s[c][i] : 0.f;
-                float s = red32(g);
-                if (i == 0) atomicAdd(&sdb3[c], s);
-                for (int j = 0; j < 3; j++) {
-                    s = red32(g * S.a1s[c][i + j]);
-                    if (i == 0) atomicAdd(&sdw3[c][j], s);
-                }
-                float dz1 = 0.f;
-                if (own) {
-                    float da1 = 0.f;
-                    for (int j = 0; j < 3; j++) da1 += P.w3[c * 3 + j] * S.z3s[c][i - j + 1];
-                    dz1 = da1 * od_silu_grad(S.z1s[c][i + 1]);
-                }
-                S.g4s[c][i] = dz1;
-                s = red32(dz1);
-                if (i == 0) atomicAdd(&sdb1[c], s);
-                for (int e = 0; e < E; e++) {
-                    s = red32(dz1 * S.z0s[e][i + 1]);
-                    if (i == 0) atomicAdd(&sdw1[c][e], s);
-                }
-            }
+        if (grp < E) {
+            const int e = grp;
+            float dz0 = 0.f;
+#pragma unroll 4
+            for (int c = 0; c < U; c++) dz0 += P.w1[c * E + e] * S.g4s[c][i];
+            pb0 += dz0;
+#pragma unroll
+            for (int j = 0; j < 3; j++) pw0[j] += dz0 * S.xts[e][i + 1 + j];
         }
         __syncthreads();
-        {
-            const bool ev = grp < E;
-            const int e = ev ? grp : 0;
-            float dz0 = 0.f;
-            if (ev)
-                for (int c = 0; c < U; c++) dz0 += P.w1[c * E + e] * S.g4s[c][i];
-            float s = red32(dz0);
-            if (ev && i == 0) atomicAdd(&sdb0[e], s);
-            for (int j = 0; j < 3; j++) {
-                s = red32(dz0 * S.xts[e][i + 1 + j]);
-                if (ev && i == 0) atomicAdd(&sdw0[e][j], s);
-            }
-        }
-        __syncthreads();
-    }
+    }
+    float* const st4 = &S.w4s[0][0];
+    float (*const stc)[MAXU] = reinterpret_cast<float (*)[MAXU]>(&S.z1s[0][0]);
+    float (*const st0)[4] = reinterpret_cast<float (*)[4]>(&S.a1s[0][0]);
+    float* const st1 = &S.g4s[0][0];
+    static_assert(sizeof(S.z1s) >= 2 * MAXU * sizeof(float) && sizeof(S.a1s) >= MAXE * 4 * sizeof(float) &&
+                  sizeof(S.g4s) >= MAXU * MAXE * sizeof(float) && sizeof(S.w4s) >= MAXU * MAXU * sizeof(float), "flush staging");
 #pragma unroll
     for (int q = 0; q < 16; q++) {
         const int o = t + 256 * q;
-        if (o < U * U) od_red_add(det, G.dw4 + o, adw4[q]);
-    }
-    __syncthreads();
-    for (int c = t; c < U; c += 256) {
-        od_red_add(det, G.db4 + c, sdb4[c]);
-        od_red_add(det, G.db3 + c, sdb3[c]);
-        od_red_add(det, G.db1 + c, sdb1[c]);
-        for (int j = 0; j < 3; j++) od_red_add(det, G.dw3 + c * 3 + j, sdw3[c][j]);
-        for (int e = 0; e < E; e++) od_red_add(det, G.dw1 + c * E + e, sdw1[c][e]);
-    }
-    if (t < E) {
-        od_red_add(det, G.db0 + t, sdb0[t]);
-        for (int j = 0; j < 3; j++) od_red_add(det, G.dw0 + t * 3 + j, sdw0[t][j]);
-    }
-}
-
-__global__ __launch_bounds__(256) void uhead_bwd_kernel(const float* __restrict__ xt, UHeadW P, const float* __restrict__ dfm,
-                                                        UHeadG G, int E, int L, int U, int nwin, const OdDetTable* __restrict__ det) {
-    uhead_bwd_body<false>(xt, P, dfm, G, E, L, U, nwin, det, nullptr);
-}
-__global__ __launch_bounds__(256) void uhead_bwd_varlen_kernel(const float* __restrict__ xt, UHeadW P, const float* __restrict__ dfm,
-                                                               UHeadG G, int E, int L, int U, int nwin, const OdDetTable* __restrict__ det,
-                                                               const int* __restrict__ lens) {
-    uhead_bwd_body<true>(xt, P, dfm, G, E, L, U, nwin, det, lens);
+        if (o < UU) st4[o] = adw4[q];
+    }
+#pragma unroll
+    for (int k = 0; k < 2; k++) {
+        const int o = t + 256 * k;
+        if (o < U * E) st1[o] = adw1[k];
+    }
+#pragma unroll
+    for (int q = 0; q < NQ; q++) {
+        const int c = cq[q];
+        const float s4 = red32(pb4[q]), s1 = red32(pb1[q]);
+        if (q < cpg && i == 0) { stc[0][c] = s4; stc[1][c] = s1; }
+    }
+    {
+        const float s0 = red32(pb0), w00 = red32(pw0[0]), w01 = red32(pw0[1]), w02 = red32(pw0[2]);
+        if (grp < E && i == 0) { st0[grp][0] = s0; st0[grp][1] = w00; st0[grp][2] = w01; st0[grp][3] = w02; }
+    }
+    __syncthreads();
+#pragma unroll 1
+    for (int o = t; o < UU; o += 256) od_red_add(det, G.dw4 + o, st4[o]);
+#pragma unroll 1
+    for (int o = t; o < U * E; o += 256) od_red_add(det, G.dw1 + o, st1[o]);
+#pragma unroll 1
+    for (int o = t; o < 2 * U; o += 256) {
+        const int kind = o / U, c = o % U;
+        od_red_add(det, kind == 0 ? G.db4 + c : G.db1 + c, stc[kind][c]);
+    }
+    if (t < 4 * U) od_red_add(det, t < 3 * U ? G.dw3 + t : G.db3 + (t - 3 * U), adw3);
+    if (t < 4 * E) {
+        const int e = t >> 2, j = t & 3;
+        od_red_add(det, j == 0 ? G.db0 + e : G.dw0 + e * 3 + (j - 1), st0[e][j]);
+    }
+}
+
+__global__ __launch_bounds__(256, 2) void uhead_bwd_kernel(const float* __restrict__ xt, UHeadW P, const float* __restrict__ dfm,
+                                                           UHeadG G, int E, int L, int U, int nwin, const OdDetTable* __restrict__ det) {
+    uhead_bwd_body<false, 0>(xt, P, dfm, G, E, L, U, nwin, det, nullptr);
+}
+__global__ __launch_bounds__(256, 2) void uhead_bwd_u64_kernel(const float* __restrict__ xt, UHeadW P, const float* __restrict__ dfm,
+                                                               UHeadG G, int E, int L, int U, int nwin, const OdDetTable* __restrict__ det) {
+    uhead_bwd_body<false, 64>(xt, P, dfm, G, E, L, U, nwin, det, nullptr);
+}
+__global__ __launch_bounds__(256, 2) void uhead_bwd_varlen_kernel(const float* __restrict__ xt, UHeadW P, const float* __restrict__ dfm,
+                                                                  UHeadG G, int E, int L, int U, int nwin, const OdDetTable* __restrict__ det,
+                                                                  const int* __restrict__ lens) {
+    uhead_bwd_body<true, 0>(xt, P, dfm, G, E, L, U, nwin, det, lens);
+}
+__global__ __launch_bounds__(256, 2) void uhead_bwd_varlen_u64_kernel(const float* __restrict__ xt, UHeadW P, const float* __restrict__ dfm,
+                                                                      UHeadG G, int E, int L, int U, int nwin, const OdDetTable* __restrict__ det,
+                                                                      const int* __restrict__ lens) {
+    uhead_bwd_body<true, 64>(xt, P, dfm, G, E, L, U, nwin, det, lens);
 }
 
 template <bool VL = false>
@@ -434,7 +519,8 @@
     UHeadW P{w0, b0, w1, b1, w3, b3, w4, b4};
     int wpb = (int)((long)nwin * B / 512);
     wpb = wpb < 1 ? 1 : (wpb > UWPB ? UWPB : wpb);
-    OD_LAUNCH(uhead_fwd_kernel<>, dim3((nwin + wpb - 1) / wpb, B), dim3(256), 0, (hipStream_t)stream, xt, P, fsum, E, L, U, nwin, wpb, od_det_active());
+    if (U == 64) OD_LAUNCH((uhead_fwd_kernel<false, 64>), dim3((nwin + wpb - 1) / wpb, B), dim3(256), 0, (hipStream_t)stream, xt, P, fsum, E, L, U, nwin, wpb, od_det_active());
+    else OD_LAUNCH((uhead_fwd_kernel<false, 0>), dim3((nwin + wpb - 1) / wpb, B), dim3(256), 0, (hipStream_t)stream, xt, P, fsum, E, L, U, nwin, wpb, od_det_active());
     OD_CHECK_LAUNCH();
     return 0;
 }
@@ -448,8 +534,10 @@
     UHeadW P{w0, b0, w1, b1, w3, b3, w4, b4};
     int wpb = (int)((long)nwin * B / 512);
     wpb = wpb < 1 ? 1 : (wpb > UWPB ? UWPB : wpb);
-    OD_LAUNCH(uhead_fwd_kernel<true>, dim3((nwin + wpb - 1) / wpb, B), dim3(256), 0, (hipStream_t)stream, xt, P, fsum, E, L, U, nwin, wpb,
-              od_det_active(), lens);
+    if (U == 64) OD_LAUNCH((uhead_fwd_kernel<true, 64>), dim3((nwin + wpb - 1) / wpb, B), dim3(256), 0, (hipStream_t)stream, xt, P, fsum, E, L, U, nwin, wpb,
+                           od_det_active(), lens);
+    else OD_LAUNCH((uhead_fwd_kernel<true, 0>), dim3((nwin + wpb - 1) / wpb, B), dim3(256), 0, (hipStream_t)stream, xt, P, fsum, E, L, U, nwin, wpb,
+                   od_det_active(), lens);
     OD_CHECK_LAUNCH();
     return 0;
 }
@@ -462,7 +550,8 @@
     const int nwin = (L + UOWN - 1) / UOWN;
     UHeadW P{w0, b0, w1, b1, w3, b3, w4, b4};
     UHeadG G{dw0, db0, dw1, db1, dw3, db3, dw4, db4};
-    OD_LAUNCH(uhead_bwd_kernel, dim3((nwin + UWPB - 1) / UWPB, B), dim3(256), 0, (hipStream_t)stream, xt, P, dfm, G, E, L, U, nwin, od_det_active());
+    if (U == 64) OD_LAUNCH(uhead_bwd_u64_kernel, dim3((nwin + UWPB - 1) / UWPB, B), dim3(256), 0, (hipStream_t)stream, xt, P, dfm, G, E, L, U, nwin, od_det_active());
+    else OD_LAUNCH(uhead_bwd_kernel, dim3((nwin + UWPB - 1) / UWPB, B), dim3(256), 0, (hipStream_t)stream, xt, P, dfm, G, E, L, U, nwin, od_det_active());
     OD_CHECK_LAUNCH();
     return 0;
 }
@@ -476,8 +565,10 @@
     const int nwin = (L + UOWN - 1) / UOWN;
     UHeadW P{w0, b0, w1, b1, w3, b3, w4, b4};
     UHeadG G{dw0, db0, dw1, db1, dw3, db3, dw4, db4};
-    OD_LAUNCH(uhead_bwd_varlen_kernel, dim3((nwin + UWPB - 1) / UWPB, B), dim3(256), 0, (hipStream_t)stream, xt, P, dfm, G, E, L, U, nwin,
-              od_det_active(), lens);
+    if (U == 64) OD_LAUNCH(uhead_bwd_varlen_u64_kernel, dim3((nwin + UWPB - 1) / UWPB, B), dim3(256), 0, (hipStream_t)stream, xt, P, dfm, G, E, L, U, nwin,
+                           od_det_active(), lens);
+    else OD_LAUNCH(uhead_bwd_varlen_kernel, dim3((nwin + UWPB - 1) / UWPB, B), dim3(256), 0, (hipStream_t)stream, xt, P, dfm, G, E, L, U, nwin,
+                   od_det_active(), lens);
     OD_CHECK_LAUNCH();
     return 0;
 }
diff --git a/osu_dreamer_amd/csrc/misc.hip b/osu_dreamer_amd/csrc/misc.hip
--- a/osu_dreamer_amd/csrc/misc.hip
+++ b/osu_dreamer_amd/csrc/misc.hip
@@ -200,14 +200,26 @@
     }
 }
 
+__device__ __forceinline__ float od_lane_bcast(float v, int src) {
+#if defined(OD_EMU)
+    return __shfl(v, src);
+#else
+    return __builtin_bit_cast(float, __builtin_amdgcn_readlane(__builtin_bit_cast(int, v), src));
+#endif
+}
+
+constexpr int PIB_G = 8, PIB_W = 8;
 template <class T>
-__global__ __launch_bounds__(256) void proj_in_bwd_kernel(const float* __restrict__ xt, const T* __restrict__ dx, int ldx,
+__global__ __launch_bounds__(64 * PIB_W, 1) void proj_in_bwd_kernel(const float* __restrict__ xt, const T* __restrict__ dx, int ldx,
                                                           float* __restrict__ dW, float* __restrict__ db, int B, int E, int L, int D,
                                                           const OdDetTable* __restrict__ det) {
     __shared__ float red[64][73];
     const int lane = threadIdx.x & 63, wave = threadIdx.x >> 6;
     const int M = B * L;
-    const int nw = gridDim.x * 4, w0 = blockIdx.x * 4 + wave;
+    const int nw = gridDim.x * PIB_W, w0 = blockIdx.x * PIB_W + wave;
+    const int per = (M + nw - 1) / nw;
+    const long ms_ = (long)w0 * per;
+    const int ms = ms_ < M ? (int)ms_ : M, me = M - ms < per ? M : ms + per;
     for (int c0 = 0; c0 < D; c0 += 512) {
         const int c = c0 + lane * 8;
         float aw[8][8], ab[8];
@@ -217,21 +229,42 @@
 #pragma unroll
             for (int e = 0; e < 8; e++) aw[k][e] = 0.f;
         }
-        if (c < D)
-            for (int m = w0; m < M; m += nw) {
-                const int b = m / L, l = m - b * L;
-                float xe[8], g[8];
-#pragma unroll
-                for (int e = 0; e < 8; e++) xe[e] = e < E ? xt[((size_t)b * E + e) * L + l] : 0.f;
-                od_ld8(dx + (size_t)m * ldx + c, g);
-#pragma unroll
-                for (int k = 0; k < 8; k++) {
-                    ab[k] += g[k];
-#pragma unroll
-                    for (int e = 0; e < 8; e++) aw[k][e] += g[k] * xe[e];
+#pragma unroll 1
+        for (int m0 = ms; m0 < me; m0 += 64) {
+            const int nf = me - m0 < 64 ? me - m0 : 64;
+            float xl[8];
+            {
+                const int ml = m0 + lane, bb = ml / L, l = ml - bb * L;
+#pragma unroll
+                for (int e = 0; e < 8; e++) xl[e] = (lane < nf && e < E) ? xt[((size_t)bb * E + e) * L + l] : 0.f;
+            }
+#pragma unroll 1
+            for (int r0 = 0; r0 < nf; r0 += PIB_G) {
+                float g[PIB_G][8];
+#pragma unroll
+                for (int j = 0; j < PIB_G; j++) {
+                    if (c < D && r0 + j < nf) od_ld8(dx + (size_t)(m0 + r0 + j) * ldx + c, g[j]);
+                    else {
+#pragma unroll
+                        for (int k = 0; k < 8; k++) g[j][k] = 0.f;
+                    }
                 }
-            }
-        for (int w = 0; w < 4; w++) {
+#pragma unroll
+                for (int j = 0; j < PIB_G; j++) {
+                    const int src = r0 + j < 64 ? r0 + j : 63;
+                    float xe[8];
+#pragma unroll
+                    for (int e = 0; e < 8; e++) xe[e] = od_lane_bcast(xl[e], src);
+#pragma unroll
+                    for (int k = 0; k < 8; k++) {
+                        ab[k] += g[j][k];
+#pragma unroll
+                        for (int e = 0; e < 8; e++) aw[k][e] += g[j][k] * xe[e];
+                    }
+                }
+            }
+        }
+        for (int w = 0; w < PIB_W; w++) {
             if (wave == w) {
 #pragma unroll
                 for (int k = 0; k < 8; k++) {
@@ -243,7 +276,7 @@
             __syncthreads();
         }
         if (wave == 0 && c < D) {
-#pragma unroll
+#pragma unroll 1
             for (int k = 0; k < 8; k++) {
                 od_red_add(det, db + c + k, red[lane][k * 9 + 8]);
 #pragma unroll
@@ -449,9 +482,9 @@
 }
 
 constexpr int LS_KC = 256, LS_NB = 8;
-__global__ __launch_bounds__(256) void linear_small_kernel(const float* __restrict__ x, const float* __restrict__ W,
-                                                           const float* __restrict__ bias, float* __restrict__ out,
-                                                           float* __restrict__ pre, int B, int N, int K, int act) {
+__device__ __forceinline__ void linear_small_tile(const float* __restrict__ x, const float* __restrict__ W,
+                                                  const float* __restrict__ bias, float* __restrict__ out,
+                                                  float* __restrict__ pre, int B, int N, int K, int act) {
     __shared__ __attribute__((aligned(16))) float xs[32][LS_KC + 4];
     __shared__ __attribute__((aligned(16))) float ws[LS_NB][LS_KC + 4];
     const int b0 = blockIdx.y * 32, n0 = blockIdx.x * LS_NB;
@@ -481,6 +514,19 @@
         if (pre) pre[(size_t)b * N + n] = s;
         out[(size_t)b * N + n] = act == OD_ACT_SILU ? od_silu(s) : s;
     }
+}
+__global__ __launch_bounds__(256) void linear_small_kernel(const float* __restrict__ x, const float* __restrict__ W,
+                                                           const float* __restrict__ bias, float* __restrict__ out,
+                                                           float* __restrict__ pre, int B, int N, int K, int act) {
+    linear_small_tile(x, W, bias, out, pre, B, N, K, act);
+}
+constexpr int LS_GROUP = 24;
+struct LinearSmallDesc { const float* W; const float* bias; float* out; float* pre; int N, act; };
+struct LinearSmallGroup { LinearSmallDesc d[LS_GROUP]; };
+__global__ __launch_bounds__(256) void linear_small_group_kernel(const float* __restrict__ x, LinearSmallGroup g, int B, int K) {
+    const LinearSmallDesc& d = g.d[blockIdx.z];
+    if ((int)blockIdx.x * LS_NB >= d.N) return;
+    linear_small_tile(x, d.W, d.bias, d.out, d.pre, B, d.N, K, d.act);
 }
 __global__ __launch_bounds__(256) void linear_small_dpre_kernel(const float* __restrict__ pre, const float* __restrict__ dout,
                                                                 float* __restrict__ dpre, long n, int act) {
@@ -553,6 +599,48 @@
     const int sn = row_map ? row_map[n] : (n < N ? n : -1);
     const float v = (sn >= 0 && k < K) ? src[(size_t)sn * K + k] : 0.f;
     od_t<T>::st(dst + i, v);
+}
+
+constexpr int PW_FIELDS = 8, PW_T = 32;
+template <class T>
+__global__ __launch_bounds__(256) void pack_weights_kernel(const long* __restrict__ tab, int nd) {
+    __shared__ float tile[PW_T][PW_T + 1];
+    const long blk = blockIdx.x;
+    int lo = 0, hi = nd;
+    while (hi - lo > 1) {
+        const int mid = (lo + hi) >> 1;
+        if (tab[mid] <= blk) lo = mid; else hi = mid;
+    }
+    const long* d = tab + (nd + 1) + (long)lo * PW_FIELDS;
+    const float* __restrict__ src = (const float*)d[0];
+    T* __restrict__ dst = (T*)d[1];
+    const int* __restrict__ row_map = (const int*)d[2];
+    const int N = (int)d[3], K = (int)d[4], Np = (int)d[5], Kp = (int)d[6], transpose = (int)d[7];
+    const unsigned local = (unsigned)(blk - tab[lo]);
+    if (!transpose) {
+        const unsigned i = local * 256u + threadIdx.x;
+        if (i >= (unsigned)Np * (unsigned)Kp) return;
+        const int n = (int)(i / (unsigned)Kp), k = (int)(i % (unsigned)Kp);
+        const int sn = row_map ? row_map[n] : (n < N ? n : -1);
+        const float v = (sn >= 0 && k < K) ? src[(size_t)sn * K + k] : 0.f;
+        od_t<T>::st(dst + i, v);
+        return;
+    }
+    const int ntn = (Np + PW_T - 1) / PW_T;
+    const int n0 = (int)(local % (unsigned)ntn) * PW_T, k0 = (int)(local / (unsigned)ntn) * PW_T;
+    const int tx = threadIdx.x & 31, ty = threadIdx.x >> 5;
+#pragma unroll
+    for (int r = 0; r < PW_T; r += 8) {
+        const int n = n0 + ty + r, k = k0 + tx;
+        const int sn = n >= Np ? -1 : row_map ? row_map[n] : (n < N ? n : -1);
+        tile[ty + r][tx] = (sn >= 0 && k < K) ? src[(size_t)sn * K + k] : 0.f;
+    }
+    __syncthreads();
+#pragma unroll
+    for (int r = 0; r < PW_T; r += 8) {
+        const int k = k0 + ty + r, n = n0 + tx;
+        if (k < Kp && n < Np) od_t<T>::st(dst + (size_t)k * Np + n, tile[tx][ty + r]);
+    }
 }
 
 __global__ __launch_bounds__(256) void pack_weight_split_kernel(const float* __restrict__ src, int N, int K, bf16_t* __restrict__ dst,
@@ -641,8 +729,8 @@
     if (D % 8 || ldx % 8) return OD_ERR_ALIGN;
     const long M = (long)B * L;
     if (M > 0x7fffffffL) return OD_ERR_UNSUPPORTED;
-    int blocks = (int)((M + 63) / 64); if (blocks > 512) blocks = 512; if (blocks < 1) blocks = 1;
-    DISPATCH_T(dtype, OD_LAUNCH((proj_in_bwd_kernel<T_>), dim3(blocks), dim3(256), 0, (hipStream_t)stream, xt, (const T_*)dx, ldx, dW, db, B, E, L, D, od_det_active()));
+    int blocks = (int)((M + 127) / 128); if (blocks > 256) blocks = 256; if (blocks < 1) blocks = 1;
+    DISPATCH_T(dtype, OD_LAUNCH((proj_in_bwd_kernel<T_>), dim3(blocks), dim3(64 * PIB_W), 0, (hipStream_t)stream, xt, (const T_*)dx, ldx, dW, db, B, E, L, D, od_det_active()));
     OD_CHECK_LAUNCH();
     return 0;
 }
@@ -766,6 +854,24 @@
     return 0;
 }
 
+extern "C" int od_linear_small_group(const float* x, const long* descs, int n, int B, int K, void* stream) {
+    if (n < 0 || (n > 0 && !descs)) return OD_ERR_ARG;
+    for (int j0 = 0; j0 < n; j0 += LS_GROUP) {
+        const int cnt = n - j0 < LS_GROUP ? n - j0 : LS_GROUP;
+        LinearSmallGroup g = {};
+        int nmax = 0;
+        for (int j = 0; j < cnt; j++) {
+            const long* d = descs + (size_t)(j0 + j) * 6;
+            g.d[j] = LinearSmallDesc{(const float*)d[0], (const float*)d[1], (float*)d[2], (float*)d[3], (int)d[4], (int)d[5]};
+            if (!g.d[j].W || !g.d[j].out || g.d[j].N < 1) return OD_ERR_ARG;
+            if (g.d[j].N > nmax) nmax = g.d[j].N;
+        }
+        OD_LAUNCH(linear_small_group_kernel, dim3((nmax + LS_NB - 1) / LS_NB, (B + 31) / 32, cnt), dim3(256), 0, (hipStream_t)stream, x, g, B, K);
+    }
+    OD_CHECK_LAUNCH();
+    return 0;
+}
+
 extern "C" int od_linear_small_bwd(const float* x, const float* W, const float* pre, const float* dout, float* dpre, float* dW,
                                    float* db, float* dx, int accumulate_dx, int B, int N, int K, int act, void* stream) {
     if (act != OD_ACT_NONE && !pre) return OD_ERR_ARG;
@@ -796,3 +902,11 @@
     OD_CHECK_LAUNCH();
     return 0;
 }
+
+extern "C" int od_pack_weights(int dtype, const long* table, int n, long blocks, void* stream) {
+    if (n < 1 || !table || blocks < 1 || blocks > 0x7fffffffL) return OD_ERR_ARG;
+    if (dtype == OD_F32X3W) return OD_ERR_UNSUPPORTED;
+    DISPATCH_T(dtype, OD_LAUNCH((pack_weights_kernel<T_>), dim3((unsigned)blocks), dim3(256), 0, (hipStream_t)stream, table, n));
+    OD_CHECK_LAUNCH();
+    return 0;
+}
diff --git a/osu_dreamer_amd/engine.py b/osu_dreamer_amd/engine.py
--- a/osu_dreamer_amd/engine.py
+++ b/osu_dreamer_amd/engine.py
@@ -64,6 +64,7 @@
         self.dropout = float(ba.dropout)
         self._packed: Dict[str, torch.Tensor] = {}
         self._packed_key = None
+        self._pack_tables: Dict[torch.dtype, "ops.PackTable"] = {}
         self._plan_key = None
         self.ws: Optional[Workspace] = None
         self._plans: "OrderedDict[tuple, Workspace]" = OrderedDict()
@@ -116,7 +117,9 @@
                 rm[j] = j
                 rm[Hp + j] = Hf + j
             self._rowmap = torch.tensor(rm, dtype=torch.int32, device=dev)
+            self._pack_tables = {}
         pk = self._packed
+        items = []
         for n in self._gemm_weights():
             w = self.P(n + ".weight")
             N, K = w.shape[0], w.shape[1]
@@ -133,11 +136,21 @@
                     pk[n + ".T"] = torch.empty(Kp, Np, dtype=dtype, device=dev)
                 if rmap is not None:
                     pk[n + ".b"] = torch.empty(Np, dtype=torch.float32, device=dev)
-            ops.pack_weight(w, pk[n], row_map=rmap)
+            if isinstance(pk[n], ops.SplitWeight):
+                ops.pack_weight(w, pk[n], row_map=rmap)
+            else:
+                items.append((w, pk[n], False, rmap))
             if train:
-                ops.pack_weight(w, pk[n + ".T"], transpose=True, row_map=rmap)
+                items.append((w, pk[n + ".T"], True, rmap))
             if rmap is not None:
-                ops.pack_weight(self.P(n + ".bias"), pk[n + ".b"].view(Np, 1), row_map=rmap)
+                items.append((self.P(n + ".bias"), pk[n + ".b"].view(Np, 1), False, rmap))
+        for dt in sorted({it[1].dtype for it in items}, key=str):
+            group = [it for it in items if it[1].dtype == dt]
+            ptrs = [t.data_ptr() if t is not None else None for it in group for t in (it[0], it[1], it[3])]
+            tab = self._pack_tables.get(dt)
+            if tab is None or tab.ptrs != ptrs:
+                tab = self._pack_tables[dt] = ops.PackTable(group)
+            ops.pack_weights(tab)
 
     def W(self, name: str, T: bool = False) -> torch.Tensor:
         return self._packed[name + (".T" if T else "")]
@@ -214,14 +227,15 @@
         ops.silu(a_pre, a)
         cg, cg_pre = self.buf("cg", (B, Cg), f32), self.buf("cg_pre", (B, Cg), f32)
         ops.linear_small(style, self.P("proj_style.0.weight"), self.P("proj_style.0.bias"), cg, cg_pre, OD_ACT_SILU)
+        group = []
         for i in range(self.depth):
             p = f"net.layers.{i}."
             for s in ("ssg1", "ssg2"):
-                ops.linear_small(cg, self.P(p + s + ".weight"), self.P(p + s + ".bias"),
-                                 self.buf(f"{s}.{i}", (B, 3 * D), f32))
+                group.append((self.P(p + s + ".weight"), self.P(p + s + ".bias"), self.buf(f"{s}.{i}", (B, 3 * D), f32), None, OD_ACT_NONE))
             if not self.train:
                 ops.gemm_nt(a, self.W(p + "proj_cl"), self.P(p + "proj_cl.bias"), self.buf(f"cl.{i}", (self.Ma, D)), x3=self.x3)
-        ops.linear_small(cg, self.P("u_mod.weight"), self.P("u_mod.bias"), self.buf("umod", (B, 2 * U), f32))
+        group.append((self.P("u_mod.weight"), self.P("u_mod.bias"), self.buf("umod", (B, 2 * U), f32), None, OD_ACT_NONE))
+        ops.linear_small_group(cg, group)
 
     def pred(self, xt: torch.Tensor, u: torch.Tensor, v: torch.Tensor):
         B, L, M, D, dh, Hp = self.B, self.L, self.M, self.D, self.dh, self.Hp
diff --git a/osu_dreamer_amd/ops.py b/osu_dreamer_amd/ops.py
--- a/osu_dreamer_amd/ops.py
+++ b/osu_dreamer_amd/ops.py
@@ -1,5 +1,6 @@
 from __future__ import annotations
 
+import ctypes
 import os
 from typing import Optional
 
@@ -126,11 +127,51 @@
     _lib.lib().od_pack_weight(code, _p(src), N, K, _p(dst), Np, Kp, int(transpose), _p(row_map), _stream(src))
 
 
+class PackTable:
+
+    def __init__(self, items):
+        assert items
+        rows, starts, self.ptrs = [], [0], []
+        self.dtype = items[0][1].dtype
+        for src, dst, transpose, row_map in items:
+            N = src.shape[0]
+            K = src.numel() // N
+            _f32(src)
+            assert dst.dtype == self.dtype and dst.is_contiguous() and dst.dim() == 2
+            Kp, Np = dst.shape if transpose else dst.shape[::-1]
+            assert Np * Kp < 2 ** 31
+            if row_map is not None:
+                _i32(row_map)
+                assert row_map.numel() == Np
+            rows.append([_p(src), _p(dst), _p(row_map) or 0, N, K, Np, Kp, int(transpose)])
+            starts.append(starts[-1] + (((Np + 31) // 32) * ((Kp + 31) // 32) if transpose else (Np * Kp + 255) // 256))
+            self.ptrs += [_p(src), _p(dst), _p(row_map)]
+        self.n, self.blocks, self.device = len(items), starts[-1], items[0][0].device
+        self.table = torch.tensor(starts + [v for r in rows for v in r], dtype=torch.int64).to(self.device)
+
+
+def pack_weights(table: PackTable):
+    _lib.lib().od_pack_weights(dt_code(table.dtype), _p(table.table), table.n, table.blocks, _stream(table.table))
+
+
 def linear_small(x, W, b, out, pre=None, act=OD_ACT_NONE):
     B, K = x.shape
     N = W.shape[0]
     _f32(x, W, b, out, pre)
     _lib.lib().od_linear_small(_p(x), _p(W), _p(b), _p(out), _p(pre), B, N, K, act, _stream(x))
+
+
+def linear_small_group(x, group):
+    B, K = x.shape
+    _f32(x)
+    descs = []
+    for W, b, out, pre, act in group:
+        _f32(W, b, out, pre)
+        N = W.shape[0]
+        assert W.numel() == N * K and out.numel() == B * N and (pre is None or pre.numel() == B * N)
+        descs += [_p(W), _p(b) or 0, _p(out), _p(pre) or 0, N, act]
+    arr = (ctypes.c_long * len(descs))(*descs)
+    _lib.lib().od_linear_small_group(_p(x), ctypes.addressof(arr), len(group), B, K, _stream(x))
 
 
 def linear_small_bwd(x, W, pre, dout, dpre, dW, db, dx, accumulate_dx, act=OD_ACT_NONE):
```
